# pasqal-io/Pulser

Measured on NVIDIA H100. Metric: time-steps/s (1 ns sampling intervals of the Sequence evolved per second), higher is better.
Workload: dtype f64 (complex128)

## Files before the change

### include/pulser_b200.h

```cpp
#ifndef PULSER_B200_H
#define PULSER_B200_H

#include <stdint.h>

#ifdef __cplusplus
extern "C" {
#endif

#define PB200_OK 0
#define PB200_ERR_INVALID -1
#define PB200_ERR_CUDA -2
#define PB200_ERR_UNSUPPORTED -3
#define PB200_ERR_STATE -4

#define PB200_MAX_QUDITS 40
#define PB200_MAX_DRIVES 3

typedef struct pb200_plan pb200_plan;

typedef struct pb200_drive_desc {
    int32_t state_to;
    int32_t state_from;
    int32_t uniform;
    int32_t reserved;
} pb200_drive_desc;

typedef struct pb200_plan_desc {
    int32_t n_qudits;
    int32_t dim;
    int32_t n_times;
    int32_t interp_order;
    int32_t n_drives;
    int32_t rydberg_state;
    int32_t n_traj;
    int32_t device;
    const double* sampling_times;
    pb200_drive_desc drives[PB200_MAX_DRIVES];
} pb200_plan_desc;

typedef struct pb200_run_opts {
    int32_t max_step_samples;
    int32_t refine_window;
    double cheb_tol;
    double rough_tol;
    int32_t magnus_order;
    int32_t check_every;
    double tol;
    int32_t extrapolate;
    int32_t integrator;
} pb200_run_opts;

typedef struct pb200_run_stats {
    int64_t n_steps;
    int64_t n_exponentials;
    int64_t n_applies;
    int64_t n_launches;
    double gpu_ms;
    double max_rho;
    int64_t n_checks;
    double err_estimate;
    double mean_step_samples;
    int64_t integrator;
    int64_t n_rejected;
} pb200_run_stats;

int pb200_version(void);
const char* pb200_last_error(void);
int pb200_device_count(void);

int pb200_plan_create(pb200_plan** out, const pb200_plan_desc* desc);
int pb200_plan_destroy(pb200_plan* plan);
int pb200_plan_set_stream(pb200_plan* plan, void* cuda_stream);

int pb200_plan_set_interaction(pb200_plan* plan, int32_t traj0, int32_t count,
                               const double* U, const uint8_t* bad,
                               int32_t shared);

int pb200_plan_set_xy(pb200_plan* plan, int32_t traj0, int32_t count,
                      const double* Uxy, const uint8_t* bad, int32_t shared,
                      int32_t digit_u, int32_t digit_d);

int pb200_plan_set_slm_mask(pb200_plan* plan, const uint8_t* masked, const double* coeff);

int pb200_plan_set_drive(pb200_plan* plan, int32_t drive, int32_t traj0,
                         int32_t count, const double* coef, const double* det);

int pb200_plan_set_dissipator(pb200_plan* plan, int32_t n_pairs,
                              const double* generators);

int pb200_plan_set_collapse(pb200_plan* plan, int32_t n_ops, const double* ops,
                            uint64_t seed);
int pb200_plan_jump_counts(pb200_plan* plan, int64_t* jumps);

int pb200_state_set(pb200_plan* plan, int32_t traj0, int32_t count,
                    const double* psi, int64_t basis_index, int32_t broadcast);
int pb200_state_get(pb200_plan* plan, int32_t traj0, int32_t count, double* psi);
int pb200_state_probabilities(pb200_plan* plan, int32_t traj0, int32_t count,
                              double* probs);
int pb200_state_norm2(pb200_plan* plan, int32_t traj0, int32_t count,
                      double* norms2);
int pb200_state_occupation(pb200_plan* plan, int32_t traj0, int32_t count,
                           int32_t digit, double* occ);
int pb200_state_correlation(pb200_plan* plan, int32_t traj0, int32_t count,
                            int32_t digit, double* corr);

int pb200_state_energy(pb200_plan* plan, double t_us, double* energy, double* h2);

int pb200_state_overlap(pb200_plan* plan, int32_t traj0, int32_t count,
                        const double* phi, double* out);

typedef struct pb200_op_terms {
    int32_t n_terms;
    const double*  coeff;
    const int32_t* site_start;
    const int32_t* site;
    const int32_t* shift;
    const double*  weight;
} pb200_op_terms;
int pb200_state_expect(pb200_plan* plan, int32_t traj0, int32_t count,
                       const pb200_op_terms* op, double* out);

int pb200_state_sample(pb200_plan* plan, int32_t traj, int32_t one_digit,
                       const double* uniforms, int32_t n_shots, int64_t* out);
int pb200_state_copy(pb200_plan* dst, int32_t dst_traj, pb200_plan* src, int32_t src_traj);
int pb200_state_device_ptr(pb200_plan* plan, void** dptr);

int pb200_density_trace(pb200_plan* plan, int32_t traj0, int32_t count,
                        double* trace);
int pb200_density_occupation(pb200_plan* plan, int32_t traj0, int32_t count,
                             int32_t digit, double* occ);
int pb200_density_correlation(pb200_plan* plan, int32_t traj0, int32_t count,
                              int32_t digit, double* corr);
int pb200_density_expect(pb200_plan* plan, int32_t traj0, int32_t count,
                         const pb200_op_terms* op, double* out);
int pb200_density_energy(pb200_plan* plan, pb200_plan* ham, double t_us,
                         int32_t traj0, int32_t count, double* energy,
                         double* h2);
int pb200_density_overlap(pb200_plan* plan, int32_t traj0, int32_t count,
                          const double* phi, double* out);
int pb200_density_sample(pb200_plan* plan, int32_t traj, int32_t one_digit,
                         const double* uniforms, int32_t n_shots, int64_t* out);

int pb200_propagate(pb200_plan* plan, double t_start, double t_stop,
                    const pb200_run_opts* opts, pb200_run_stats* stats);

int pb200_apply_h(pb200_plan* plan, int32_t traj, double t_us,
                  const double* in, double* out);

int pb200_coefficients_at(pb200_plan* plan, int32_t traj, int32_t drive,
                          int32_t row, double t_us, double* out3);

int pb200_bench_apply(pb200_plan* plan, double t_us, int32_t reps,
                      double* ms_out, int64_t* launches_out);

int pb200_plan_create_shard(pb200_plan** out, const pb200_plan_desc* desc,
                            int32_t shard_bits, int32_t shard_index);
int pb200_shards_link(pb200_plan** plans, int32_t count);
int pb200_shards_propagate(pb200_plan** plans, int32_t count, double t_start,
                           double t_stop, const pb200_run_opts* opts,
                           pb200_run_stats* stats);
int pb200_shards_apply_h(pb200_plan** plans, int32_t count, double t_us,
                         const double* in, double* out);
int pb200_shards_energy(pb200_plan** plans, int32_t count, double t_us,
                        double* energy, double* h2);
int pb200_shards_expect(pb200_plan** plans, int32_t count,
                        const pb200_op_terms* op, double* out);

int pb200_host_interpolate(const double* x, const double* y, int32_t n,
                           int32_t order, const double* tq, int32_t nq,
                           double* out);
int pb200_host_moments(const double* x, const double* y, int32_t n,
                       int32_t order, double a, double b, double* out4);
int pb200_host_taylor_fit(const double* x, const double* y, int32_t n,
                          int32_t order, double a, double h, int32_t p,
                          double* coeffs, double* resid);
int pb200_host_taylor_separable(const double* coef, const double* det,
                                int32_t n_traj, int32_t n_qudits,
                                int32_t n_times, int32_t* separable,
                                double* a_out, double* c_out, double* m_out);
int pb200_host_taylor_shapes(const double* coef, const double* det,
                             int32_t n_traj, int32_t n_qudits, int32_t n_times,
                             int32_t max_shapes, int32_t* n_shapes,
                             double* a_out, double* c_out, double* m_out);
int pb200_host_taylor_order(double h, const double* m, int32_t p, double tol,
                            int32_t* order_out, double* tail_out);
int pb200_host_chebyshev(double rho, double tol, double* out, int32_t cap,
                         int32_t* count);

#ifdef __cplusplus
}
#endif
#endif
```

### pulser_b200/_lib.py

```python
from __future__ import annotations

import ctypes as C
import os

_HERE = os.path.dirname(os.path.abspath(__file__))
LIB_PATH = os.path.join(_HERE, "libpulser_b200.so")

PB200_MAX_DRIVES = 3


class DriveDesc(C.Structure):
    _fields_ = [
        ("state_to", C.c_int32),
        ("state_from", C.c_int32),
        ("uniform", C.c_int32),
        ("reserved", C.c_int32),
    ]


class PlanDesc(C.Structure):
    _fields_ = [
        ("n_qudits", C.c_int32),
        ("dim", C.c_int32),
        ("n_times", C.c_int32),
        ("interp_order", C.c_int32),
        ("n_drives", C.c_int32),
        ("rydberg_state", C.c_int32),
        ("n_traj", C.c_int32),
        ("device", C.c_int32),
        ("sampling_times", C.POINTER(C.c_double)),
        ("drives", DriveDesc * PB200_MAX_DRIVES),
    ]


class RunOpts(C.Structure):
    _fields_ = [
        ("max_step_samples", C.c_int32),
        ("refine_window", C.c_int32),
        ("cheb_tol", C.c_double),
        ("rough_tol", C.c_double),
        ("magnus_order", C.c_int32),
        ("check_every", C.c_int32),
        ("tol", C.c_double),
        ("extrapolate", C.c_int32),
        ("integrator", C.c_int32),
    ]


class RunStats(C.Structure):
    _fields_ = [
        ("n_steps", C.c_int64),
        ("n_exponentials", C.c_int64),
        ("n_applies", C.c_int64),
        ("n_launches", C.c_int64),
        ("gpu_ms", C.c_double),
        ("max_rho", C.c_double),
        ("n_checks", C.c_int64),
        ("err_estimate", C.c_double),
        ("mean_step_samples", C.c_double),
        ("integrator", C.c_int64),
        ("n_rejected", C.c_int64),
    ]


class OpTermsDesc(C.Structure):

    _fields_ = [
        ("n_terms", C.c_int32),
        ("coeff", C.POINTER(C.c_double)),
        ("site_start", C.POINTER(C.c_int32)),
        ("site", C.POINTER(C.c_int32)),
        ("shift", C.POINTER(C.c_int32)),
        ("weight", C.POINTER(C.c_double)),
    ]


class LibraryMissing(ImportError):
    pass


def _load() -> C.CDLL:
    if not os.path.exists(LIB_PATH):
        raise LibraryMissing(
            f"{LIB_PATH} not found: build it with "
            "`python -m pulser_b200.build` (nvcc, sm_90a). "
            "pulser_b200 has no CPU fallback."
        )
    lib = C.CDLL(LIB_PATH)
    dp = C.POINTER(C.c_double)
    vp = C.c_void_p
    sig = {
        "pb200_version": (C.c_int, []),
        "pb200_last_error": (C.c_char_p, []),
        "pb200_device_count": (C.c_int, []),
        "pb200_plan_create": (C.c_int, [C.POINTER(vp), C.POINTER(PlanDesc)]),
        "pb200_plan_destroy": (C.c_int, [vp]),
        "pb200_plan_set_stream": (C.c_int, [vp, vp]),
        "pb200_plan_set_interaction": (
            C.c_int, [vp, C.c_int32, C.c_int32, dp, C.POINTER(C.c_uint8), C.c_int32]),
        "pb200_plan_set_xy": (
            C.c_int, [vp, C.c_int32, C.c_int32, dp, C.POINTER(C.c_uint8), C.c_int32, C.c_int32, C.c_int32]),
        "pb200_plan_set_slm_mask": (C.c_int, [vp, C.POINTER(C.c_uint8), dp]),
        "pb200_plan_set_drive": (C.c_int, [vp, C.c_int32, C.c_int32, C.c_int32, dp, dp]),
        "pb200_plan_set_dissipator": (C.c_int, [vp, C.c_int32, dp]),
        "pb200_plan_set_collapse": (C.c_int, [vp, C.c_int32, dp, C.c_uint64]),
        "pb200_plan_jump_counts": (C.c_int, [vp, C.POINTER(C.c_int64)]),
        "pb200_state_set": (C.c_int, [vp, C.c_int32, C.c_int32, dp, C.c_int64, C.c_int32]),
        "pb200_state_get": (C.c_int, [vp, C.c_int32, C.c_int32, dp]),
        "pb200_state_probabilities": (C.c_int, [vp, C.c_int32, C.c_int32, dp]),
        "pb200_state_norm2": (C.c_int, [vp, C.c_int32, C.c_int32, dp]),
        "pb200_state_occupation": (C.c_int, [vp, C.c_int32, C.c_int32, C.c_int32, dp]),
        "pb200_state_correlation": (C.c_int, [vp, C.c_int32, C.c_int32, C.c_int32, dp]),
        "pb200_state_energy": (C.c_int, [vp, C.c_double, dp, dp]),
        "pb200_state_overlap": (C.c_int, [vp, C.c_int32, C.c_int32, dp, dp]),
        "pb200_state_expect": (C.c_int, [vp, C.c_int32, C.c_int32, C.POINTER(OpTermsDesc), dp]),
        "pb200_state_sample": (
            C.c_int, [vp, C.c_int32, C.c_int32, dp, C.c_int32, C.POINTER(C.c_int64)]),
        "pb200_state_copy": (C.c_int, [vp, C.c_int32, vp, C.c_int32]),
        "pb200_state_device_ptr": (C.c_int, [vp, C.POINTER(vp)]),
        "pb200_density_trace": (C.c_int, [vp, C.c_int32, C.c_int32, dp]),
        "pb200_density_occupation": (C.c_int, [vp, C.c_int32, C.c_int32, C.c_int32, dp]),
        "pb200_density_correlation": (C.c_int, [vp, C.c_int32, C.c_int32, C.c_int32, dp]),
        "pb200_density_expect": (C.c_int, [vp, C.c_int32, C.c_int32, C.POINTER(OpTermsDesc), dp]),
        "pb200_density_energy": (C.c_int, [vp, vp, C.c_double, C.c_int32, C.c_int32, dp, dp]),
        "pb200_density_overlap": (C.c_int, [vp, C.c_int32, C.c_int32, dp, dp]),
        "pb200_density_sample": (
            C.c_int, [vp, C.c_int32, C.c_int32, dp, C.c_int32, C.POINTER(C.c_int64)]),
        "pb200_propagate": (
            C.c_int, [vp, C.c_double, C.c_double, C.POINTER(RunOpts), C.POINTER(RunStats)]),
        "pb200_apply_h": (C.c_int, [vp, C.c_int32, C.c_double, dp, dp]),
        "pb200_coefficients_at": (
            C.c_int, [vp, C.c_int32, C.c_int32, C.c_int32, C.c_double, dp]),
        "pb200_bench_apply": (
            C.c_int, [vp, C.c_double, C.c_int32, dp, C.POINTER(C.c_int64)]),
        "pb200_plan_create_shard": (C.c_int, [C.POINTER(vp), C.POINTER(PlanDesc), C.c_int32, C.c_int32]),
        "pb200_shards_link": (C.c_int, [C.POINTER(vp), C.c_int32]),
        "pb200_shards_propagate": (
            C.c_int, [C.POINTER(vp), C.c_int32, C.c_double, C.c_double, C.POINTER(RunOpts), C.POINTER(RunStats)]),
        "pb200_shards_apply_h": (C.c_int, [C.POINTER(vp), C.c_int32, C.c_double, dp, dp]),
        "pb200_shards_energy": (C.c_int, [C.POINTER(vp), C.c_int32, C.c_double, dp, dp]),
        "pb200_shards_expect": (C.c_int, [C.POINTER(vp), C.c_int32, C.POINTER(OpTermsDesc), dp]),
        "pb200_host_interpolate": (
            C.c_int, [dp, dp, C.c_int32, C.c_int32, dp, C.c_int32, dp]),
        "pb200_host_moments": (
            C.c_int, [dp, dp, C.c_int32, C.c_int32, C.c_double, C.c_double, dp]),
        "pb200_host_chebyshev": (
            C.c_int, [C.c_double, C.c_double, dp, C.c_int32, C.POINTER(C.c_int32)]),
        "pb200_host_taylor_fit": (
            C.c_int, [dp, dp, C.c_int32, C.c_int32, C.c_double, C.c_double, C.c_int32, dp, dp]),
        "pb200_host_taylor_separable": (
            C.c_int, [dp, dp, C.c_int32, C.c_int32, C.c_int32, C.POINTER(C.c_int32), dp, dp, dp]),
        "pb200_host_taylor_shapes": (
            C.c_int, [dp, dp, C.c_int32, C.c_int32, C.c_int32, C.c_int32, C.POINTER(C.c_int32), dp, dp, dp]),
        "pb200_host_taylor_order": (
            C.c_int, [C.c_double, dp, C.c_int32, C.c_double, C.POINTER(C.c_int32), dp]),
    }
    for name, (res, args) in sig.items():
        fn = getattr(lib, name)
        fn.restype = res
        fn.argtypes = args
    return lib


EXPORTED_SYMBOLS = [
    "pb200_version", "pb200_last_error", "pb200_device_count",
    "pb200_plan_create", "pb200_plan_destroy", "pb200_plan_set_stream",
    "pb200_plan_set_interaction", "pb200_plan_set_xy", "pb200_plan_set_slm_mask", "pb200_plan_set_drive", "pb200_plan_set_dissipator", "pb200_plan_set_collapse",
    "pb200_plan_jump_counts", "pb200_state_set",
    "pb200_state_get", "pb200_state_probabilities", "pb200_state_norm2",
    "pb200_state_occupation", "pb200_state_correlation", "pb200_state_energy", "pb200_state_overlap", "pb200_state_expect", "pb200_state_sample", "pb200_state_copy", "pb200_state_device_ptr", "pb200_propagate", "pb200_apply_h",
    "pb200_coefficients_at", "pb200_bench_apply", "pb200_host_interpolate",
    "pb200_host_moments", "pb200_host_chebyshev", "pb200_host_taylor_fit", "pb200_host_taylor_order", "pb200_host_taylor_separable",
    "pb200_host_taylor_shapes",
    "pb200_plan_create_shard", "pb200_shards_link", "pb200_shards_propagate", "pb200_shards_apply_h", "pb200_shards_energy",
    "pb200_shards_expect",
    "pb200_density_trace", "pb200_density_occupation", "pb200_density_correlation", "pb200_density_expect",
    "pb200_density_energy", "pb200_density_overlap", "pb200_density_sample",
]

lib = _load()


class PB200Error(RuntimeError):
    def __init__(self, code: int, msg: str):
        super().__init__(f"pulser_b200 error {code}: {msg}")
        self.code = code


def check(code: int) -> None:
    if code != 0:
        raise PB200Error(code, lib.pb200_last_error().decode("utf-8", "replace"))
```

### pulser_b200/csrc/kernels.cuh

```cuda
#pragma once
#include <cuda_runtime.h>
#include <stdint.h>
#include <type_traits>

namespace pb200 {

struct c2 { double x, y; };

__host__ __device__ inline c2 cmul(c2 a, c2 b) { return {a.x * b.x - a.y * b.y, a.x * b.y + a.y * b.x}; }
__host__ __device__ inline c2 cadd(c2 a, c2 b) { return {a.x + b.x, a.y + b.y}; }

struct PassGeom {
    int n_bits;
    int lo_bits;
    int hi_shift;
    int hi_bits;
    uint32_t tile_flip_mask;
    unsigned long long extra_mask;
    int first_pass;
};

struct StageCoef {
    c2 c_psi, c_b2, c_g;
};

struct UniformDrive {
    c2 g;
    double theta;
    double w;
    double gamma;
    int to_bit;
    int from_count_is_popc;
};

__host__ __device__ inline int d2_table_stride(int n) { return 3 * n + 2; }

__device__ __forceinline__ uint32_t smem_u32(const void* p) {
    return static_cast<uint32_t>(__cvta_generic_to_shared(p));
}
__device__ __forceinline__ void mbar_init(uint64_t* bar, uint32_t count) {
    asm volatile("mbarrier.init.shared::cta.b64 [%0], %1;" ::"r"(smem_u32(bar)), "r"(count));
    asm volatile("fence.mbarrier_init.release.cluster;" ::: "memory");
    asm volatile("fence.proxy.async.shared::cta;" ::: "memory");
}
__device__ __forceinline__ void mbar_arrive_expect_tx(uint64_t* bar, uint32_t bytes) {
    asm volatile("mbarrier.arrive.expect_tx.shared::cta.b64 _, [%0], %1;" ::"r"(smem_u32(bar)), "r"(bytes)
                 : "memory");
}
__device__ __forceinline__ void mbar_wait(uint64_t* bar, uint32_t parity) {
    asm volatile(
        "{\n\t"
        ".reg .pred p;\n\t"
        "WAIT_%=:\n\t"
        "mbarrier.try_wait.parity.shared::cta.b64 p, [%0], %1;\n\t"
        "@p bra DONE_%=;\n\t"
        "bra WAIT_%=;\n\t"
        "DONE_%=:\n\t"
        "}\n" ::"r"(smem_u32(bar)),
        "r"(parity)
        : "memory");
}
__device__ __forceinline__ void tma_load_1d(void* smem_dst, const void* gmem_src, uint32_t bytes, uint64_t* bar) {
    asm volatile(
        "cp.async.bulk.shared::cluster.global.mbarrier::complete_tx::bytes [%0], [%1], %2, [%3];" ::"r"(
            smem_u32(smem_dst)),
        "l"(gmem_src), "r"(bytes), "r"(smem_u32(bar))
        : "memory");
}

__device__ __forceinline__ c2 ld_stream(const c2* p) {
    double2 r = __ldcs(reinterpret_cast<const double2*>(p));
    return {r.x, r.y};
}
__device__ __forceinline__ void st_c2(c2* p, c2 v) {
    *reinterpret_cast<double2*>(p) = make_double2(v.x, v.y);
}
__device__ __forceinline__ void st_c2_evict_last(c2* p, c2 v) {
    uint64_t pol;
    asm("createpolicy.fractional.L2::evict_last.b64 %0, 1.0;" : "=l"(pol));
    asm volatile("st.global.L2::cache_hint.v2.f64 [%0], {%1, %2}, %3;" ::"l"(p), "d"(v.x), "d"(v.y), "l"(pol) : "memory");
}

struct LanczosFuse {
    const c2* vj;
    const c2* vjm1;
    c2* vout;
    const double* acc_prev;
    const double* beta_prev;
    double* alpha_out;
    double* beta_out;
    double* acc_clear;
};

struct LanczosCoef { double alpha, beta, inv, beta_prev; };

__device__ __forceinline__ LanczosCoef lanczos_coef(const LanczosFuse& lz, long long traj) {
    LanczosCoef c;
    c.alpha = lz.acc_prev[2 * traj];
    const double ww = lz.acc_prev[2 * traj + 1];
    const double b2 = ww - c.alpha * c.alpha;
    c.beta = (b2 > 1e-28 * fmax(ww, 1e-300)) ? sqrt(b2) : 0.0;
    c.inv = c.beta > 0.0 ? 1.0 / c.beta : 0.0;
    c.beta_prev = lz.beta_prev ? lz.beta_prev[traj] : 0.0;
    return c;
}

struct StageArgs {
    const c2* v;
    const c2* psi;
    const c2* b2;
    c2* out;
    const double* dint;
    long long dint_stride;
    long long D;
    PassGeom geo;
    StageCoef coef;
    UniformDrive u;
    const double* table;
    int to_bit;
    int from_is_one;
    const double* beta_dev;
    double* dot_acc;
    LanczosFuse lz;
    const c2* w_in;
    c2* w_out;
    long long w_plane;
};

struct StageArgs2 {
    StageArgs a[2];
    int n_traj;
};

template <bool UNIFORM, bool REAL_G>
__global__ void __launch_bounds__(256) stage_d2_kernel(StageArgs a) {
    extern __shared__ __align__(128) unsigned char smem_raw[];
    c2* tile = reinterpret_cast<c2*>(smem_raw);
    __shared__ __align__(8) uint64_t mbar;

    const PassGeom g = a.geo;
    const int tbits = g.lo_bits + g.hi_bits;
    const int tsize = 1 << tbits;
    const long long traj = blockIdx.y;
    const long long tile_id = blockIdx.x;
    const int mid_bits = g.hi_shift - g.lo_bits;
    const long long mid = tile_id & ((1LL << mid_bits) - 1);
    const long long top = tile_id >> mid_bits;
    const long long base = (mid << g.lo_bits) | (top << (g.hi_shift + g.hi_bits));
    const long long voff = traj * a.D;
    const c2* vsrc = a.v + voff;

    double* tab = reinterpret_cast<double*>(tile + tsize);
    if (!UNIFORM) {
        const int stride = d2_table_stride(g.n_bits);
        const double* src = a.table + traj * stride;
        for (int i = threadIdx.x; i < stride; i += blockDim.x) tab[i] = src[i];
    }

    if (threadIdx.x == 0) mbar_init(&mbar, 1);
    __syncthreads();
    if (threadIdx.x == 0) mbar_arrive_expect_tx(&mbar, (uint32_t)tsize * 16u);
    {
        const int rows = 1 << g.hi_bits;
        const uint32_t row_bytes = (uint32_t)(16u << g.lo_bits);
        for (int r = threadIdx.x; r < rows; r += blockDim.x)
            tma_load_1d(tile + ((size_t)r << g.lo_bits), vsrc + base + ((long long)r << g.hi_shift), row_bytes, &mbar);
    }
    mbar_wait(&mbar, 0);

    const long long lomask = (1LL << g.lo_bits) - 1;
    double w, gamma, theta_u;
    c2 gu;
    if (UNIFORM) {
        w = a.u.w; gamma = a.u.gamma; theta_u = a.u.theta; gu = a.u.g;
    } else {
        w = tab[3 * g.n_bits]; gamma = tab[3 * g.n_bits + 1]; theta_u = 0.0; gu = {0.0, 0.0};
    }
    const int to_bit = a.to_bit;

    for (int t = threadIdx.x; t < tsize; t += blockDim.x) {
        const long long idx = base | (t & lomask) | ((long long)(t >> g.lo_bits) << g.hi_shift);
        const c2 vo = tile[t];
        double pr = 0.0, pi = 0.0, qr = 0.0, qi = 0.0;
#pragma unroll 1
        for (uint32_t m = g.tile_flip_mask; m; m &= m - 1) {
            const int j = __ffs(m) - 1;
            const c2 pv = tile[t ^ (1 << j)];
            const int bit = (t >> j) & 1;
            if (UNIFORM) {
                pr += pv.x; pi += pv.y;
                if (!REAL_G) {
                    const double s = (bit == to_bit) ? 1.0 : -1.0;
                    qr = fma(s, pv.x, qr); qi = fma(s, pv.y, qi);
                }
            } else {
                const int p = (j < g.lo_bits) ? j : (j - g.lo_bits + g.hi_shift);
                const double gx = tab[2 * p];
                const double gy = (bit == to_bit) ? tab[2 * p + 1] : -tab[2 * p + 1];
                pr = fma(gx, pv.x, pr); pr = fma(-gy, pv.y, pr);
                pi = fma(gx, pv.y, pi); pi = fma(gy, pv.x, pi);
            }
        }
#pragma unroll 1
        for (unsigned long long m = g.extra_mask; m; m &= m - 1) {
            const int p = __ffsll((long long)m) - 1;
            const double2 raw = __ldg(reinterpret_cast<const double2*>(vsrc + (idx ^ (1LL << p))));
            const c2 pv = {raw.x, raw.y};
            const int bit = (int)((idx >> p) & 1);
            if (UNIFORM) {
                pr += pv.x; pi += pv.y;
                if (!REAL_G) {
                    const double s = (bit == to_bit) ? 1.0 : -1.0;
                    qr = fma(s, pv.x, qr); qi = fma(s, pv.y, qi);
                }
            } else {
                const double gx = tab[2 * p];
                const double gy = (bit == to_bit) ? tab[2 * p + 1] : -tab[2 * p + 1];
                pr = fma(gx, pv.x, pr); pr = fma(-gy, pv.y, pr);
                pi = fma(gx, pv.y, pi); pi = fma(gy, pv.x, pi);
            }
        }
        c2 drive;
        if (UNIFORM) {
            drive.x = gu.x * pr; drive.y = gu.x * pi;
            if (!REAL_G) { drive.x = fma(-gu.y, qi, drive.x); drive.y = fma(gu.y, qr, drive.y); }
        } else {
            drive = {pr, pi};
        }
        c2 res;
        if (g.first_pass) {
            double diag = -gamma;
            if (a.dint) diag = fma(w, __ldcs(a.dint + traj * a.dint_stride + idx), diag);
            if (UNIFORM) {
                const int ones = __popcll((unsigned long long)idx);
                const int cnt = a.from_is_one ? ones : (g.n_bits - ones);
                diag = fma(-theta_u, (double)cnt, diag);
            } else {
                double acc = 0.0;
                for (int p = 0; p < g.n_bits; ++p) {
                    const int bit = (int)((idx >> p) & 1);
                    acc += (bit == a.from_is_one) ? tab[2 * g.n_bits + p] : 0.0;
                }
                diag -= acc;
            }
            c2 gv = {fma(diag, vo.x, drive.x), fma(diag, vo.y, drive.y)};
            res = cmul(a.coef.c_g, gv);
            if (a.psi) res = cadd(res, cmul(a.coef.c_psi, ld_stream(a.psi + voff + idx)));
            if (a.b2) res = cadd(res, cmul(a.beta_dev ? c2{-a.beta_dev[traj], 0.0} : a.coef.c_b2, ld_stream(a.b2 + voff + idx)));
        } else {
            res = cadd(ld_stream(a.out + voff + idx), cmul(a.coef.c_g, drive));
        }
        st_c2(a.out + voff + idx, res);
    }
}

__device__ __forceinline__ c2 ld_own(const c2* p) {
    double2 r = __ldcs(reinterpret_cast<const double2*>(p));
    return {r.x, r.y};
}

__device__ __forceinline__ void taylor_signed_add(double gx, double gy, double sg, double x, double y, double& pr, double& pi,
                                                  double& qr, double& qi) {
    const double zx = fma(gx, x, -gy * y), zy = fma(gx, y, gy * x);
    pr += zx; pi += zy;
    qr = fma(sg, zx, qr); qi = fma(sg, zy, qi);
}

template <bool UNIFORM, bool REAL_G, int TBITS, int RB, bool SIGNED = false>
__device__ __forceinline__ void rb_tile_gather(const PassGeom& g, const c2* tile, const double* __restrict__ tab, int tid,
                                               int to_bit, int jstart, bool skip_smem, const c2 (&v)[1 << RB],
                                               double (&pr)[1 << RB], double (&pi)[1 << RB], double (&qr)[1 << RB],
                                               double (&qi)[1 << RB]) {
    static_assert(!SIGNED || !UNIFORM, "signed sums of the per-bit table gather");
    constexpr int R = 1 << RB;
    constexpr int NT = 1 << (TBITS - RB);
#pragma unroll
    for (int q = 0; q < RB; ++q) {
        const int j = TBITS - RB + q;
        double gx = 0.0, gyt = 0.0;
        if (!UNIFORM) {
            const int p = (j < g.lo_bits) ? j : (j - g.lo_bits + g.hi_shift);
            gx = tab[2 * p]; gyt = tab[2 * p + 1];
        }
#pragma unroll
        for (int r = 0; r < R; ++r) {
            const c2 pv = v[r ^ (1 << q)];
            const int bit = (r >> q) & 1;
            if (UNIFORM) {
                pr[r] += pv.x; pi[r] += pv.y;
                if (!REAL_G) {
                    if (bit == to_bit) { qr[r] += pv.x; qi[r] += pv.y; } else { qr[r] -= pv.x; qi[r] -= pv.y; }
                }
            } else if constexpr (SIGNED) {
                const double gy = (bit == to_bit) ? gyt : -gyt;
                taylor_signed_add(gx, gy, bit == to_bit ? 1.0 : -1.0, pv.x, pv.y, pr[r], pi[r], qr[r], qi[r]);
            } else {
                const double gy = (bit == to_bit) ? gyt : -gyt;
                pr[r] = fma(gx, pv.x, pr[r]); pr[r] = fma(-gy, pv.y, pr[r]);
                pi[r] = fma(gx, pv.y, pi[r]); pi[r] = fma(gy, pv.x, pi[r]);
            }
        }
    }
#pragma unroll
    for (int j = 0; j < TBITS - RB; ++j) {
        if (j >= jstart && !skip_smem) {
            const int bit = (tid >> j) & 1;
            const int ptid = tid ^ (1 << j);
            double gx = 0.0, gy = 0.0;
            if (!UNIFORM) {
                const int p = (j < g.lo_bits) ? j : (j - g.lo_bits + g.hi_shift);
                gx = tab[2 * p];
                gy = (bit == to_bit) ? tab[2 * p + 1] : -tab[2 * p + 1];
            }
            const double sg = (bit == to_bit) ? 1.0 : -1.0;
#pragma unroll
            for (int r = 0; r < R; ++r) {
                const c2 pv = tile[ptid + r * NT];
                if (UNIFORM) {
                    pr[r] += pv.x; pi[r] += pv.y;
                    if (!REAL_G) { qr[r] = fma(sg, pv.x, qr[r]); qi[r] = fma(sg, pv.y, qi[r]); }
                } else if constexpr (SIGNED) {
                    taylor_signed_add(gx, gy, sg, pv.x, pv.y, pr[r], pi[r], qr[r], qi[r]);
                } else {
                    pr[r] = fma(gx, pv.x, pr[r]); pr[r] = fma(-gy, pv.y, pr[r]);
                    pi[r] = fma(gx, pv.y, pi[r]); pi[r] = fma(gy, pv.x, pi[r]);
                }
            }
        }
    }
}

template <bool UNIFORM, bool REAL_G, int TBITS, int RB>
__device__ __forceinline__ void rb_tile_compute(const StageArgs& a, const PassGeom& g, const c2* tile,
                                                const double* __restrict__ tab, long long base, long long traj,
                                                int tid, uint64_t* tile_bar) {
    constexpr int R = 1 << RB;
    constexpr int NT = 1 << (TBITS - RB);
    const long long voff = traj * a.D;
    const c2* vsrc = a.v + voff;
    const long long lomask = (1LL << g.lo_bits) - 1;
    const int to_bit = a.to_bit;
    const int jstart = __ffs(g.tile_flip_mask) - 1;

    c2 v[R];
    double pr[R], pi[R], qr[R], qi[R];
    long long idx[R];
#pragma unroll
    for (int r = 0; r < R; ++r) {
        const int t = tid + r * NT;
        idx[r] = base | (t & lomask) | ((long long)(t >> g.lo_bits) << g.hi_shift);
        pr[r] = 0.0; pi[r] = 0.0; qr[r] = 0.0; qi[r] = 0.0;
    }
    for (unsigned long long m = g.extra_mask; m; m &= m - 1) {
        const int p = __ffsll((long long)m) - 1;
        double gx = 0.0, gyt = 0.0;
        if (!UNIFORM) { gx = tab[2 * p]; gyt = tab[2 * p + 1]; }
        const int bit = (int)((base >> p) & 1);
        const double sg = (bit == to_bit) ? 1.0 : -1.0;
        const double gy = (bit == to_bit) ? gyt : -gyt;
        double2 raw[R];
#pragma unroll
        for (int r = 0; r < R; ++r) raw[r] = __ldg(reinterpret_cast<const double2*>(vsrc + (idx[r] ^ (1LL << p))));
#pragma unroll
        for (int r = 0; r < R; ++r) {
            if (UNIFORM) {
                pr[r] += raw[r].x; pi[r] += raw[r].y;
                if (!REAL_G) { qr[r] = fma(sg, raw[r].x, qr[r]); qi[r] = fma(sg, raw[r].y, qi[r]); }
            } else {
                pr[r] = fma(gx, raw[r].x, pr[r]); pr[r] = fma(-gy, raw[r].y, pr[r]);
                pi[r] = fma(gx, raw[r].y, pi[r]); pi[r] = fma(gy, raw[r].x, pi[r]);
            }
        }
    }
    if (tile_bar) mbar_wait(tile_bar, 0);
#pragma unroll
    for (int r = 0; r < R; ++r) v[r] = tile[tid + r * NT];
    rb_tile_gather<UNIFORM, REAL_G, TBITS, RB>(g, tile, tab, tid, to_bit, jstart, false, v, pr, pi, qr, qi);
    double w = 0.0, gamma = 0.0, th_common = 0.0;
    double th_r[R];
    if (g.first_pass) {
        if (UNIFORM) { w = a.u.w; gamma = a.u.gamma; }
        else {
            w = tab[3 * g.n_bits]; gamma = tab[3 * g.n_bits + 1];
            const long long fixed = base | (tid & lomask) | ((long long)(tid >> g.lo_bits) << g.hi_shift);
            for (int p = 0; p < g.n_bits; ++p) {
                const int bit = (int)((fixed >> p) & 1);
                th_common += (bit == a.from_is_one) ? tab[2 * g.n_bits + p] : 0.0;
            }
#pragma unroll
            for (int r = 0; r < R; ++r) {
                double acc = 0.0;
#pragma unroll
                for (int q = 0; q < RB; ++q) {
                    const int j = TBITS - RB + q;
                    const int p = (j < g.lo_bits) ? j : (j - g.lo_bits + g.hi_shift);
                    const double th = tab[2 * g.n_bits + p];
                    const int bit = (r >> q) & 1;
                    acc += ((bit == a.from_is_one) ? th : 0.0) - ((0 == a.from_is_one) ? th : 0.0);
                }
                th_r[r] = acc;
            }
        }
    }
#pragma unroll
    for (int r = 0; r < R; ++r) {
        if (UNIFORM) {
            const double dx = a.u.g.x * pr[r], dy = a.u.g.x * pi[r];
            if (!REAL_G) { pr[r] = fma(-a.u.g.y, qi[r], dx); pi[r] = fma(a.u.g.y, qr[r], dy); }
            else { pr[r] = dx; pi[r] = dy; }
        }
    }
    constexpr int H = (R >= 4) ? R / 2 : R;
    const c2 cb2 = a.beta_dev ? c2{-a.beta_dev[traj], 0.0} : a.coef.c_b2;
    const bool fuse = a.lz.vj != nullptr;
    LanczosCoef lc{0.0, 0.0, 0.0, 0.0};
    if (fuse) lc = lanczos_coef(a.lz, traj);
    double dot0 = 0.0, dot1 = 0.0;
    if (g.first_pass) {
        const double* dsrc = a.dint ? a.dint + traj * a.dint_stride : nullptr;
#pragma unroll
        for (int h0 = 0; h0 < R; h0 += H) {
            double dv[H];
            c2 pv[H], bv[H];
#pragma unroll
            for (int r = 0; r < H; ++r) {
                dv[r] = dsrc ? __ldcs(dsrc + idx[h0 + r]) : 0.0;
                if (fuse) {
                    pv[r] = ld_own(a.lz.vj + voff + idx[h0 + r]);
                    bv[r] = (a.lz.vjm1 && lc.beta_prev != 0.0) ? ld_own(a.lz.vjm1 + voff + idx[h0 + r]) : c2{0.0, 0.0};
                } else {
                    pv[r] = a.psi ? ld_own(a.psi + voff + idx[h0 + r]) : c2{0.0, 0.0};
                    bv[r] = a.b2 ? ld_own(a.b2 + voff + idx[h0 + r]) : c2{0.0, 0.0};
                }
            }
#pragma unroll
            for (int r = 0; r < H; ++r) {
                const int rr = h0 + r;
                double diag = fma(w, dv[r], -gamma);
                if (UNIFORM) {
                    const int ones = __popcll((unsigned long long)idx[rr]);
                    const int cnt = a.from_is_one ? ones : (g.n_bits - ones);
                    diag = fma(-a.u.theta, (double)cnt, diag);
                } else {
                    diag -= th_common + th_r[rr];
                }
                const c2 gv = {fma(diag, v[rr].x, pr[rr]), fma(diag, v[rr].y, pi[rr])};
                c2 res, lhs;
                if (fuse) {
                    const c2 vn = {(v[rr].x - lc.alpha * pv[r].x) * lc.inv, (v[rr].y - lc.alpha * pv[r].y) * lc.inv};
                    const double ai = lc.alpha * lc.inv, abi = ai * lc.beta_prev;
                    res.x = fma(lc.inv, gv.x, -fma(ai, v[rr].x, fma(abi, bv[r].x, lc.beta * pv[r].x)));
                    res.y = fma(lc.inv, gv.y, -fma(ai, v[rr].y, fma(abi, bv[r].y, lc.beta * pv[r].y)));
                    st_c2(a.lz.vout + voff + idx[rr], vn);
                    lhs = vn;
                } else {
                    res = cmul(a.coef.c_g, gv);
                    res = cadd(res, cmul(a.coef.c_psi, pv[r]));
                    res = cadd(res, cmul(cb2, bv[r]));
                    lhs = v[rr];
                }
                dot0 = fma(lhs.x, res.x, dot0); dot0 = fma(lhs.y, res.y, dot0);
                dot1 = fma(res.x, res.x, dot1); dot1 = fma(res.y, res.y, dot1);
                st_c2(a.out + voff + idx[rr], res);
            }
        }
    } else {
#pragma unroll
        for (int h0 = 0; h0 < R; h0 += H) {
            c2 ov[H];
#pragma unroll
            for (int r = 0; r < H; ++r) ov[r] = ld_own(a.out + voff + idx[h0 + r]);
#pragma unroll
            for (int r = 0; r < H; ++r) {
                const int rr = h0 + r;
                const c2 res = cadd(ov[r], cmul(a.coef.c_g, c2{pr[rr], pi[rr]}));
                dot0 = fma(v[rr].x, res.x, dot0); dot0 = fma(v[rr].y, res.y, dot0);
                dot1 = fma(res.x, res.x, dot1); dot1 = fma(res.y, res.y, dot1);
                st_c2(a.out + voff + idx[rr], res);
            }
        }
    }
    if (a.dot_acc) {
        for (int o = 16; o > 0; o >>= 1) {
            dot0 += __shfl_xor_sync(0xffffffffu, dot0, o);
            dot1 += __shfl_xor_sync(0xffffffffu, dot1, o);
        }
        __shared__ double dred[2][NT / 32 > 0 ? NT / 32 : 1];
        if ((tid & 31) == 0) { dred[0][tid >> 5] = dot0; dred[1][tid >> 5] = dot1; }
        __syncthreads();
        if (tid == 0) {
            double s0 = 0.0, s1 = 0.0;
#pragma unroll
            for (int i = 0; i < NT / 32; ++i) { s0 += dred[0][i]; s1 += dred[1][i]; }
            atomicAdd(a.dot_acc + 2 * traj, s0);
            atomicAdd(a.dot_acc + 2 * traj + 1, s1);
        }
    }
    if (fuse && blockIdx.x == 0 && tid == 0) {
        a.lz.alpha_out[traj] = lc.alpha;
        a.lz.beta_out[traj] = lc.beta;
        a.lz.acc_clear[2 * traj] = 0.0;
        a.lz.acc_clear[2 * traj + 1] = 0.0;
    }
}

__device__ __forceinline__ long long tile_base_of(const PassGeom& g, long long tile_id) {
    const int mid_bits = g.hi_shift - g.lo_bits;
    const long long mid = tile_id & ((1LL << mid_bits) - 1);
    const long long top = tile_id >> mid_bits;
    return (mid << g.lo_bits) | (top << (g.hi_shift + g.hi_bits));
}

__device__ __forceinline__ void pdl_wait() { asm volatile("griddepcontrol.wait;" ::: "memory"); }
__device__ __forceinline__ void pdl_launch_dependents() { asm volatile("griddepcontrol.launch_dependents;" ::: "memory"); }

template <bool UNIFORM, bool REAL_G, int TBITS, int RB>
__global__ void __launch_bounds__(1 << (TBITS - RB), (65536 / ((1 << (TBITS - RB)) * (RB >= 3 ? 128 : 64))))
stage_d2_rb_kernel(const __grid_constant__ StageArgs2 m) {
    constexpr int NT = 1 << (TBITS - RB);
    constexpr int TSIZE = 1 << TBITS;
    extern __shared__ __align__(128) unsigned char smem_raw[];
    c2* tile = reinterpret_cast<c2*>(smem_raw);
    __shared__ __align__(8) uint64_t mbar;

    const int chain = blockIdx.y / m.n_traj;
    const StageArgs& a = m.a[chain];
    const PassGeom g = a.geo;
    const int tid = threadIdx.x;
    const long long traj = blockIdx.y - chain * m.n_traj;
    const long long base = tile_base_of(g, blockIdx.x);
    const c2* vsrc = a.v + traj * a.D;

    if (tid == 0) mbar_init(&mbar, 1);
    __syncthreads();
    pdl_wait();
    pdl_launch_dependents();
    if (tid == 0) mbar_arrive_expect_tx(&mbar, (uint32_t)TSIZE * 16u);
    const int rows = 1 << g.hi_bits;
    const uint32_t row_bytes = (uint32_t)(16u << g.lo_bits);
    for (int r = tid; r < rows; r += NT)
        tma_load_1d(tile + ((size_t)r << g.lo_bits), vsrc + base + ((long long)r << g.hi_shift), row_bytes, &mbar);
    double* tab = reinterpret_cast<double*>(tile + TSIZE);
    if (!UNIFORM) {
        const int stride = d2_table_stride(g.n_bits);
        const double* src = a.table + traj * stride;
        for (int i = tid; i < stride; i += NT) tab[i] = src[i];
        __syncthreads();
    }
    rb_tile_compute<UNIFORM, REAL_G, TBITS, RB>(a, g, tile, tab, base, traj, tid, &mbar);
}

template <bool REAL_G, int TBITS, int RB>
__global__ void __launch_bounds__(1 << (TBITS - RB), 2) stage_d2_fwd_kernel(const __grid_constant__ StageArgs2 m) {
    constexpr int R = 1 << RB;
    constexpr int NT = 1 << (TBITS - RB);
    constexpr int TSIZE = 1 << TBITS;
    extern __shared__ __align__(128) unsigned char smem_raw[];
    c2* tile = reinterpret_cast<c2*>(smem_raw);
    c2* rtile = tile + TSIZE;
    __shared__ __align__(8) uint64_t mbar;

    const int chain = blockIdx.y / m.n_traj;
    const StageArgs& a = m.a[chain];
    const PassGeom g = a.geo;
    const int tid = threadIdx.x;
    const long long traj = blockIdx.y - chain * m.n_traj;
    const long long base = tile_base_of(g, blockIdx.x);
    const long long voff = traj * a.D;
    const c2* vsrc = a.v + voff;

    if (tid == 0) mbar_init(&mbar, 1);
    __syncthreads();
    pdl_wait();
    pdl_launch_dependents();
    if (tid == 0) mbar_arrive_expect_tx(&mbar, (uint32_t)TSIZE * 16u);
    {
        const int rows = 1 << g.hi_bits;
        const uint32_t row_bytes = (uint32_t)(16u << g.lo_bits);
        for (int r = tid; r < rows; r += NT)
            tma_load_1d(tile + ((size_t)r << g.lo_bits), vsrc + base + ((long long)r << g.hi_shift), row_bytes, &mbar);
    }
    const long long lomask = (1LL << g.lo_bits) - 1;
    const long long fixed = base | (tid & lomask) | ((long long)(tid >> g.lo_bits) << g.hi_shift);
    int pq[RB];
#pragma unroll
    for (int q = 0; q < RB; ++q) {
        const int j = TBITS - RB + q;
        pq[q] = (j < g.lo_bits) ? j : (j - g.lo_bits + g.hi_shift);
    }
    auto idx_of = [&](int r) {
        long long o = fixed;
#pragma unroll
        for (int q = 0; q < RB; ++q) o |= (long long)((r >> q) & 1) << pq[q];
        return o;
    };
    double pr[R], pi[R], qr[R], qi[R];
    c2 part[R];
    double dg[R];
    {
        const double* dsrc = a.dint ? a.dint + traj * a.dint_stride : nullptr;
#pragma unroll
        for (int r = 0; r < R; ++r) {
            const long long ix = idx_of(r);
            c2 w0 = {0.0, 0.0}, w1 = {0.0, 0.0}, ps = {0.0, 0.0}, bb = {0.0, 0.0};
            if (a.w_in) { w0 = ld_own(a.w_in + voff + ix); if (!REAL_G) w1 = ld_own(a.w_in + a.w_plane + voff + ix); }
            if (a.psi) ps = ld_own(a.psi + voff + ix);
            if (a.b2) bb = ld_own(a.b2 + voff + ix);
            const double dv = dsrc ? __ldcs(dsrc + ix) : 0.0;
            pr[r] = w0.x; pi[r] = w0.y; qr[r] = w1.x; qi[r] = w1.y;
            part[r] = cadd(cmul(a.coef.c_psi, ps), cmul(a.coef.c_b2, bb));
            const int ones = __popcll((unsigned long long)ix);
            const int cnt = a.from_is_one ? ones : (g.n_bits - ones);
            dg[r] = fma(-a.u.theta, (double)cnt, fma(a.u.w, dv, -a.u.gamma));
        }
    }
    const int to_bit = a.to_bit;
    for (unsigned long long em = g.extra_mask; em; em &= em - 1) {
        const int p = __ffsll((long long)em) - 1;
        const double sg = (((base >> p) & 1) == to_bit) ? 1.0 : -1.0;
        double2 raw[R];
#pragma unroll
        for (int r = 0; r < R; ++r) raw[r] = __ldg(reinterpret_cast<const double2*>(vsrc + (idx_of(r) ^ (1LL << p))));
#pragma unroll
        for (int r = 0; r < R; ++r) {
            pr[r] += raw[r].x; pi[r] += raw[r].y;
            if (!REAL_G) { qr[r] = fma(sg, raw[r].x, qr[r]); qi[r] = fma(sg, raw[r].y, qi[r]); }
        }
    }
    mbar_wait(&mbar, 0);
    const int jstart = __ffs(g.tile_flip_mask) - 1;
    c2 v[R];
#pragma unroll
    for (int r = 0; r < R; ++r) v[r] = tile[tid + r * NT];
    rb_tile_gather<true, REAL_G, TBITS, RB>(g, tile, nullptr, tid, to_bit, jstart, false, v, pr, pi, qr, qi);
#pragma unroll
    for (int r = 0; r < R; ++r) {
        double dx = a.u.g.x * pr[r], dy = a.u.g.x * pi[r];
        if (!REAL_G) { dx = fma(-a.u.g.y, qi[r], dx); dy = fma(a.u.g.y, qr[r], dy); }
        const c2 gv = {fma(dg[r], v[r].x, dx), fma(dg[r], v[r].y, dy)};
        const c2 res = cadd(part[r], cmul(a.coef.c_g, gv));
        st_c2(a.out + voff + idx_of(r), res);
        v[r] = res;
    }
    if (a.w_out) {
#pragma unroll
        for (int r = 0; r < R; ++r) {
            rtile[tid + r * NT] = v[r];
            pr[r] = 0.0; pi[r] = 0.0; qr[r] = 0.0; qi[r] = 0.0;
        }
        __syncthreads();
        rb_tile_gather<true, REAL_G, TBITS, RB>(g, rtile, nullptr, tid, to_bit, jstart, false, v, pr, pi, qr, qi);
#pragma unroll
        for (int r = 0; r < R; ++r) {
            const long long ix = idx_of(r);
            st_c2(a.w_out + voff + ix, c2{pr[r], pi[r]});
            if (!REAL_G) st_c2(a.w_out + a.w_plane + voff + ix, c2{qr[r], qi[r]});
        }
    }
}

#define PB200_TAYLOR_PMAX 8
#define PB200_MAX_SHARD_BITS 3
#define PB200_TAYLOR_SMAX 4
__host__ __device__ inline int taylor_table_stride(int n, int s) { return 2 * n + s * n; }
struct TaylorArgs {
    const c2* v;
    c2* out;
    c2* g_out;
    c2* acc;
    const double* dint;
    long long dint_stride;
    const double* cpl;
    long long cpl_stride;
    int ryd_bit;
    long long D;
    PassGeom geo;
    c2 unit;
    const double* table;
    int tab_shapes;
    int to_bit, from_is_one;
    double th0, gam0, om0;
    double m0[PB200_TAYLOR_SMAX];
    c2 scale;
    int nh;
    const c2* hchi[PB200_TAYLOR_PMAX];
    const c2* hg[PB200_TAYLOR_PMAX];
    double hth[PB200_TAYLOR_PMAX], hgam[PB200_TAYLOR_PMAX], hom[PB200_TAYLOR_PMAX];
    double hm[PB200_TAYLOR_SMAX][PB200_TAYLOR_PMAX];
    int acc_read;
    int acc_add_v;
    int acc_add_h;
    int acc_on;
    c2 acc_mul;
    const c2* peer[PB200_MAX_SHARD_BITS];
    int shard_bits, shard;
    c2* g2_out;
    double om0i;
    const c2* hg2[PB200_TAYLOR_PMAX];
    double homi[PB200_TAYLOR_PMAX];
    c2 dw[4], df[4];
    int n_pair;
    int diss_flip;
};

template <int R, int H = (R >= 4) ? R / 2 : R, bool SHARD = false, bool CPLX = false, bool DISS = false, class Off,
          class Dint>
__device__ __forceinline__ void taylor_epilogue(const TaylorArgs& a, const long long (&idx)[R], c2 (&v)[R],
                                                const double (&gx)[R], const double (&gy)[R], const Off& off,
                                                long long voff, const Dint& dint,
                                                const double* qx = nullptr, const double* qy = nullptr,
                                                const double* ex = nullptr, const double* ey = nullptr) {
    constexpr bool SHAPES = !std::is_array<Off>::value;
    const int nb = a.geo.n_bits;
    const int ones_hi = SHARD ? __popc(a.shard) : 0;
#pragma unroll
    for (int h0 = 0; h0 < R; h0 += H) {
        double sx[H], sy[H], cn[H];
        {
            double dv[H];
#pragma unroll
            for (int r = 0; r < H; ++r) dv[r] = dint(h0 + r);
#pragma unroll
            for (int r = 0; r < H; ++r) {
                const int ones = __popcll((unsigned long long)idx[h0 + r]) + ones_hi;
                cn[r] = (double)(a.from_is_one ? ones : (nb - ones));
                double diag;
                if constexpr (SHAPES) diag = fma(-a.th0, cn[r], dv[r] - a.gam0 - off(h0 + r, 0));
                else diag = fma(-a.th0, cn[r], fma(-a.m0[0], off[h0 + r], dv[r] - a.gam0));
                sx[r] = fma(diag, v[h0 + r].x, a.om0 * gx[h0 + r]);
                sy[r] = fma(diag, v[h0 + r].y, a.om0 * gy[h0 + r]);
                if constexpr (CPLX) { sx[r] = fma(a.om0i, qx[h0 + r], sx[r]); sy[r] = fma(a.om0i, qy[h0 + r], sy[r]); }
                if constexpr (DISS) { sx[r] += ex[h0 + r]; sy[r] += ey[h0 + r]; }
            }
        }
        for (int j = 0; j < a.nh; ++j) {
            if (a.hchi[j]) {
                c2 c[H];
#pragma unroll
                for (int r = 0; r < H; ++r) c[r] = ld_own(a.hchi[j] + voff + idx[h0 + r]);
#pragma unroll
                for (int r = 0; r < H; ++r) {
                    double d;
                    if constexpr (SHAPES) d = -fma(a.hth[j], cn[r], a.hgam[j] + off(h0 + r, j + 1));
                    else d = -fma(a.hth[j], cn[r], fma(a.hm[0][j], off[h0 + r], a.hgam[j]));
                    sx[r] = fma(d, c[r].x, sx[r]); sy[r] = fma(d, c[r].y, sy[r]);
                    if (j == 0 && a.acc_add_h) v[h0 + r] = cadd(v[h0 + r], c[r]);
                }
            }
            if (a.hg[j]) {
                c2 c[H];
#pragma unroll
                for (int r = 0; r < H; ++r) c[r] = ld_own(a.hg[j] + voff + idx[h0 + r]);
#pragma unroll
                for (int r = 0; r < H; ++r) { sx[r] = fma(a.hom[j], c[r].x, sx[r]); sy[r] = fma(a.hom[j], c[r].y, sy[r]); }
            }
            if constexpr (CPLX) {
                if (a.hg2[j]) {
                    c2 c[H];
#pragma unroll
                    for (int r = 0; r < H; ++r) c[r] = ld_own(a.hg2[j] + voff + idx[h0 + r]);
#pragma unroll
                    for (int r = 0; r < H; ++r) { sx[r] = fma(a.homi[j], c[r].x, sx[r]); sy[r] = fma(a.homi[j], c[r].y, sy[r]); }
                }
            }
        }
        c2 res[H];
#pragma unroll
        for (int r = 0; r < H; ++r) {
            res[r] = {a.scale.x * sx[r] - a.scale.y * sy[r], a.scale.x * sy[r] + a.scale.y * sx[r]};
            st_c2_evict_last(a.out + voff + idx[h0 + r], res[r]);
            if (a.g_out) st_c2(a.g_out + voff + idx[h0 + r], c2{gx[h0 + r], gy[h0 + r]});
            if constexpr (CPLX) { if (a.g2_out) st_c2(a.g2_out + voff + idx[h0 + r], c2{qx[h0 + r], qy[h0 + r]}); }
        }
        if (a.acc_on) {
            c2 ac[H];
#pragma unroll
            for (int r = 0; r < H; ++r) ac[r] = a.acc_read ? ld_own(a.acc + voff + idx[h0 + r]) : c2{0.0, 0.0};
#pragma unroll
            for (int r = 0; r < H; ++r) {
                c2 s = cadd(ac[r], res[r]);
                if (a.acc_add_v) s = cadd(s, v[h0 + r]);
                st_c2(a.acc + voff + idx[h0 + r], cmul(a.acc_mul, s));
            }
        }
    }
}

__device__ __forceinline__ c2 taylor_diss_diag(const TaylorArgs& a, long long s, c2 v) {
    const unsigned long long c = (unsigned long long)s & ((1ULL << a.n_pair) - 1), r = (unsigned long long)s >> a.n_pair;
    const double nr = (double)__popcll(r), nc = (double)__popcll(c), nrc = (double)__popcll(r & c);
    const double wx = fma(a.dw[3].x, nrc, fma(a.dw[2].x, nc, fma(a.dw[1].x, nr, a.dw[0].x)));
    const double wy = fma(a.dw[3].y, nrc, fma(a.dw[2].y, nc, fma(a.dw[1].y, nr, a.dw[0].y)));
    return {wx * v.x - wy * v.y, wx * v.y + wy * v.x};
}

__device__ __forceinline__ void taylor_diss_flip(const TaylorArgs& a, long long s, int pr, int pc, double2 pv, double& dx,
                                                 double& dy) {
    const c2 f = a.df[(int)((((s >> pr) & 1) << 1) | ((s >> pc) & 1))];
    dx = fma(f.x, pv.x, dx); dx = fma(-f.y, pv.y, dx);
    dy = fma(f.x, pv.y, dy); dy = fma(f.y, pv.x, dy);
}

__host__ __device__ constexpr int taylor_dint_doubles(int tbits, int rb) {
    return tbits * tbits + tbits + 1 + (1 << rb) + (rb + 1) * (1 << (tbits - rb));
}

template <int TBITS, int RB>
__device__ __forceinline__ void taylor_dint_setup(const TaylorArgs& a, long long traj, unsigned long long hi, int tid,
                                                  double* dsm) {
    constexpr int NT = 1 << (TBITS - RB), L0 = TBITS - RB;
    const int nb = a.geo.n_bits;
    double* Ws = dsm + taylor_dint_doubles(TBITS, RB);
    const double* Wq = a.cpl + traj * a.cpl_stride;
    for (int i = tid; i < nb * nb; i += NT) Ws[i] = __ldg(Wq + i);
    __syncthreads();
    auto W = [&](int p, int q) { return Ws[(nb - 1 - p) * nb + (nb - 1 - q)]; };
    const unsigned long long flip = a.ryd_bit ? 0ULL : ~0ULL;
    const unsigned long long nmask = nb >= 64 ? ~0ULL : (1ULL << nb) - 1;
    const unsigned long long hs = (hi ^ flip) & nmask & ~((1ULL << TBITS) - 1);
    double* wt = dsm;
    double* wj = wt + TBITS * TBITS;
    double* hh = wj + TBITS;
    double* ts = hh + 1;
    double* xt = ts + (1 << RB);
    for (int i = tid; i < TBITS * TBITS; i += NT) wt[i] = W(i / TBITS, i % TBITS);
    if (tid < TBITS) {
        double s = 0.0;
        for (unsigned long long m = hs; m; m &= m - 1) s += W(__ffsll((long long)m) - 1, tid);
        wj[tid] = s;
    } else if (tid >= 32 && tid < 32 + (1 << RB)) {
        const int m = tid - 32;
        const unsigned ms = ((unsigned)m ^ (unsigned)flip) & ((1u << RB) - 1);
        double s = 0.0;
        for (int q = 0; q < RB; ++q) {
            if (!((ms >> q) & 1)) continue;
            for (unsigned long long h = hs; h; h &= h - 1) s += W(L0 + q, __ffsll((long long)h) - 1);
            for (int q2 = q + 1; q2 < RB; ++q2) if ((ms >> q2) & 1) s += W(L0 + q, L0 + q2);
        }
        ts[m] = s;
    } else if (tid >= 64 && tid < 96) {
        double s = 0.0;
        for (int p = TBITS + (tid - 64); p < nb; p += 32) {
            if (!((hs >> p) & 1)) continue;
            for (unsigned long long h = hs & ~((2ULL << p) - 1); h; h &= h - 1) s += W(p, __ffsll((long long)h) - 1);
        }
#pragma unroll
        for (int o = 16; o; o >>= 1) s += __shfl_xor_sync(0xffffffffu, s, o);
        if (tid == 64) hh[0] = s;
    }
    __syncthreads();
    const unsigned tb = ((unsigned)tid ^ (unsigned)flip) & (NT - 1);
    double ct = hh[0];
    double y[RB];
#pragma unroll
    for (int q = 0; q < RB; ++q) y[q] = 0.0;
#pragma unroll 1
    for (int i = 0; i < L0; ++i) {
        const bool bi = (tb >> i) & 1;
        ct += bi ? wj[i] : 0.0;
        for (int j = i + 1; j < L0; ++j) ct += (bi && ((tb >> j) & 1)) ? wt[i * TBITS + j] : 0.0;
#pragma unroll
        for (int q = 0; q < RB; ++q) y[q] += bi ? wt[i * TBITS + L0 + q] : 0.0;
    }
#pragma unroll
    for (int q = 0; q < RB; ++q) {
        if (!a.ryd_bit) { ct += y[q]; y[q] = -y[q]; }
        xt[(q + 1) * NT + tid] = y[q];
    }
    xt[tid] = ct;
}

template <bool UNIFORM, bool REAL_G, int TBITS, int RB, bool SHARD = false, int NS = (UNIFORM ? 0 : 1), bool CPLX = false,
          bool DISS = false>
__global__ void __launch_bounds__(1 << (TBITS - RB),
                                  (CPLX || DISS) ? 1 : (65536 / ((1 << (TBITS - RB)) * (RB >= 3 ? 128 : 64))))
stage_d2_taylor_kernel(const __grid_constant__ TaylorArgs a) {
    static_assert(RB >= 3, "chunks of 8 amplitudes per thread");
    static_assert(UNIFORM || !SHARD, "shards carry one state with a uniform drive");
    static_assert(NS == (UNIFORM ? 0 : 1) || NS == PB200_TAYLOR_SMAX, "one-shape table, or PB200_TAYLOR_SMAX shapes");
    static_assert(!CPLX || !REAL_G, "a complex drive gathers through the per-bit table");
    static_assert(!DISS || (!UNIFORM && !SHARD && !CPLX), "a density matrix runs the batch gather, one device, one phase");
    constexpr bool SHAPES = NS == PB200_TAYLOR_SMAX;
    constexpr int NT = 1 << (TBITS - RB);
    constexpr int TSIZE = 1 << TBITS;
    constexpr int RC = 8;
    constexpr int CB = RB - 3;
    constexpr int STB = TBITS - CB;
    constexpr bool TAB = !(UNIFORM && REAL_G);
    extern __shared__ __align__(128) unsigned char smem_raw[];
    c2* tile = reinterpret_cast<c2*>(smem_raw);
    __shared__ __align__(8) uint64_t mbar;
    const PassGeom& g = a.geo;
    const int tid = threadIdx.x;
    const long long traj = UNIFORM ? 0 : (long long)blockIdx.y;
    const long long voff = traj * a.D;
    const long long base = (long long)blockIdx.x << TBITS;
    const c2* vsrc = a.v + voff;

    if (tid == 0) mbar_init(&mbar, 1);
    __syncthreads();
    double* dsm = reinterpret_cast<double*>(tile + TSIZE);
    const double* ts = dsm + TBITS * TBITS + TBITS + 1;
    const double* xt = ts + (1 << RB);
    double* tab = dsm + taylor_dint_doubles(TBITS, RB) + g.n_bits * g.n_bits;
    if (a.cpl)
        taylor_dint_setup<TBITS, RB>(
            a, traj, (unsigned long long)base | (SHARD ? (unsigned long long)a.shard << (g.n_bits - a.shard_bits) : 0ULL),
            tid, dsm);
    pdl_wait();
    pdl_launch_dependents();
    if (tid == 0) {
        mbar_arrive_expect_tx(&mbar, (uint32_t)TSIZE * 16u);
        tma_load_1d(tile, vsrc + base, (uint32_t)TSIZE * 16u, &mbar);
    }
    double* bl = tab + (SHAPES ? taylor_table_stride(g.n_bits, NS) : 0);
    double* at = bl + ((PB200_TAYLOR_PMAX + 1) << RB);
    auto shape_coef = [&](int J, int s) { return J == 0 ? a.m0[s] : a.hm[s][J - 1]; };
    if (TAB || SHAPES) {
        if (UNIFORM && !SHAPES) {
            for (int i = tid; i < 2 * g.n_bits; i += NT) tab[i] = (i & 1) ? a.unit.y : a.unit.x;
        } else {
            const int stride = SHAPES ? taylor_table_stride(g.n_bits, NS) : d2_table_stride(g.n_bits);
            const double* src = a.table + traj * stride;
            for (int i = tid; i < stride; i += NT) tab[i] = src[i];
            if (SHAPES) {
                for (int i = tid; i < ((a.nh + 1) << RB); i += NT) {
                    const int J = i >> RB;
                    double acc = 0.0;
                    for (int s = 0; s < NS; ++s) {
                        const double* w = src + 2 * g.n_bits + s * g.n_bits + (TBITS - RB);
                        double l = 0.0;
                        for (int q = 0; q < RB; ++q) {
                            const int bit = (i >> q) & 1;
                            l += ((bit == a.from_is_one) ? w[q] : 0.0) - ((0 == a.from_is_one) ? w[q] : 0.0);
                        }
                        acc = fma(shape_coef(J, s), l, acc);
                    }
                    bl[i] = acc;
                }
            }
        }
        __syncthreads();
    }
    const int to_bit = a.to_bit;
    const int nb = g.n_bits;
    double common = 0.0;
    if (!UNIFORM && !SHAPES) {
        for (int p = 0; p < nb; ++p) {
            const int bit = (int)(((base + tid) >> p) & 1);
            common += (bit == a.from_is_one) ? tab[2 * nb + p] : 0.0;
        }
    }
    if (SHAPES) {
        double cs[NS > 0 ? NS : 1];
#pragma unroll
        for (int s = 0; s < NS; ++s) cs[s] = 0.0;
        for (int p = 0; p < nb; ++p) {
            int bit = (int)(((base + tid) >> p) & 1);
            if (SHARD && p >= nb - a.shard_bits) bit = (a.shard >> (p - (nb - a.shard_bits))) & 1;
            if (bit == a.from_is_one) {
#pragma unroll
                for (int s = 0; s < NS; ++s) cs[s] += tab[2 * nb + s * nb + p];
            }
        }
        for (int J = 0; J <= a.nh; ++J) {
            double acc = 0.0;
#pragma unroll
            for (int s = 0; s < NS; ++s) acc = fma(shape_coef(J, s), cs[s], acc);
            at[J * NT + tid] = acc;
        }
    }
#pragma unroll 1
    for (int c = 0; c < (1 << CB); ++c) {
        const long long i0 = base + tid + c * RC * NT;
        double pr[RC], pi[RC];
        double dr[RC], di[RC];
#pragma unroll
        for (int r = 0; r < RC; ++r) { pr[r] = 0.0; pi[r] = 0.0; dr[r] = 0.0; di[r] = 0.0; }
        for (unsigned long long m = g.extra_mask; m; m &= m - 1) {
            const int p = __ffsll((long long)m) - 1;
            const int bit = (int)((base >> p) & 1);
            double gx = 0.0, gy = 0.0;
            if (TAB) { gx = tab[2 * p]; gy = (bit == to_bit) ? tab[2 * p + 1] : -tab[2 * p + 1]; }
            const c2* src = vsrc + (i0 ^ (1LL << p));
            double2 raw[RC];
#pragma unroll
            for (int r = 0; r < RC; ++r) raw[r] = __ldg(reinterpret_cast<const double2*>(src + r * NT));
#pragma unroll
            for (int r = 0; r < RC; ++r) {
                if constexpr (CPLX) {
                    taylor_signed_add(gx, gy, bit == to_bit ? 1.0 : -1.0, raw[r].x, raw[r].y, pr[r], pi[r], dr[r], di[r]);
                } else if (!TAB) {
                    pr[r] += raw[r].x; pi[r] += raw[r].y;
                } else {
                    pr[r] = fma(gx, raw[r].x, pr[r]); pr[r] = fma(-gy, raw[r].y, pr[r]);
                    pi[r] = fma(gx, raw[r].y, pi[r]); pi[r] = fma(gy, raw[r].x, pi[r]);
                }
            }
        }
        if (SHARD) {
            for (int q = 0; q < a.shard_bits; ++q) {
                const int bit = (a.shard >> q) & 1;
                double gx = 0.0, gy = 0.0;
                if (TAB) {
                    const int p = nb - a.shard_bits + q;
                    gx = tab[2 * p]; gy = (bit == to_bit) ? tab[2 * p + 1] : -tab[2 * p + 1];
                }
                const c2* src = a.peer[q] + i0;
                double2 raw[RC];
#pragma unroll
                for (int r = 0; r < RC; ++r) raw[r] = *reinterpret_cast<const double2*>(src + r * NT);
#pragma unroll
                for (int r = 0; r < RC; ++r) {
                    if constexpr (CPLX) {
                        taylor_signed_add(gx, gy, bit == to_bit ? 1.0 : -1.0, raw[r].x, raw[r].y, pr[r], pi[r], dr[r], di[r]);
                    } else if (!TAB) {
                        pr[r] += raw[r].x; pi[r] += raw[r].y;
                    } else {
                        pr[r] = fma(gx, raw[r].x, pr[r]); pr[r] = fma(-gy, raw[r].y, pr[r]);
                        pi[r] = fma(gx, raw[r].y, pi[r]); pi[r] = fma(gy, raw[r].x, pi[r]);
                    }
                }
            }
        }
        if (c == 0) mbar_wait(&mbar, 0);
        auto dint = [&](int r) {
            if (!a.cpl) return 0.0;
            const int m = c * RC + r;
            double d = ts[m] + xt[tid];
#pragma unroll
            for (int q = 0; q < RB; ++q)
                if ((m >> q) & 1) d += xt[(q + 1) * NT + tid];
            return d;
        };
        const c2* sub = tile + (c << STB);
        c2 v[RC];
        double qd[RC];
#pragma unroll
        for (int r = 0; r < RC; ++r) v[r] = sub[tid + r * NT];
        if constexpr (CPLX) rb_tile_gather<false, false, STB, 3, true>(g, sub, tab, tid, to_bit, 0, false, v, pr, pi, dr, di);
        else rb_tile_gather<!TAB, !TAB, STB, 3>(g, sub, tab, tid, to_bit, 0, false, v, pr, pi, qd, qd);
#pragma unroll
        for (int q = 0; q < CB; ++q) {
            const int p = STB + q;
            const int bit = (c >> q) & 1;
            double gx = 0.0, gy = 0.0;
            if (TAB) { gx = tab[2 * p]; gy = (bit == to_bit) ? tab[2 * p + 1] : -tab[2 * p + 1]; }
            const c2* other = tile + ((c ^ (1 << q)) << STB);
#pragma unroll
            for (int r = 0; r < RC; ++r) {
                const c2 pv = other[tid + r * NT];
                if constexpr (CPLX) {
                    taylor_signed_add(gx, gy, bit == to_bit ? 1.0 : -1.0, pv.x, pv.y, pr[r], pi[r], dr[r], di[r]);
                } else if (!TAB) {
                    pr[r] += pv.x; pi[r] += pv.y;
                } else {
                    pr[r] = fma(gx, pv.x, pr[r]); pr[r] = fma(-gy, pv.y, pr[r]);
                    pi[r] = fma(gx, pv.y, pi[r]); pi[r] = fma(gy, pv.x, pi[r]);
                }
            }
        }
        double off[RC];
        long long idx[RC];
#pragma unroll
        for (int r = 0; r < RC; ++r) {
            idx[r] = i0 + r * NT;
            if (!TAB) { pr[r] *= a.unit.x; pi[r] *= a.unit.x; }
            double acc = common;
            if (!UNIFORM && !SHAPES) {
#pragma unroll
                for (int q = 0; q < RB; ++q) {
                    const double th = tab[2 * nb + TBITS - RB + q];
                    const int bit = ((c * RC + r) >> q) & 1;
                    acc += ((bit == a.from_is_one) ? th : 0.0) - ((0 == a.from_is_one) ? th : 0.0);
                }
            }
            off[r] = acc;
        }
        double ex[RC], ey[RC];
        if constexpr (DISS) {
            double dx[RC], dy[RC];
#pragma unroll
            for (int r = 0; r < RC; ++r) {
                const c2 w = taylor_diss_diag(a, idx[r], v[r]);
                dx[r] = w.x; dy[r] = w.y;
            }
            if (a.diss_flip) {
                const int tpos = tid + (c << STB);
                for (int pc = 0; pc < a.n_pair; ++pc) {
                    const int pr = pc + a.n_pair;
                    const long long mask = (1LL << pr) | (1LL << pc);
                    double2 pv[RC];
                    if (pr < TBITS) {
#pragma unroll
                        for (int r = 0; r < RC; ++r) {
                            const c2 t = tile[(tpos + r * NT) ^ (int)mask];
                            pv[r] = make_double2(t.x, t.y);
                        }
                    } else {
#pragma unroll
                        for (int r = 0; r < RC; ++r) pv[r] = __ldg(reinterpret_cast<const double2*>(vsrc + (idx[r] ^ mask)));
                    }
#pragma unroll
                    for (int r = 0; r < RC; ++r) taylor_diss_flip(a, idx[r], pr, pc, pv[r], dx[r], dy[r]);
                }
            }
#pragma unroll
            for (int r = 0; r < RC; ++r) { ex[r] = -dy[r]; ey[r] = dx[r]; }
        }
        if constexpr (CPLX) {
            double qx[RC], qy[RC];
#pragma unroll
            for (int r = 0; r < RC; ++r) { qx[r] = -di[r]; qy[r] = dr[r]; }
            if constexpr (SHAPES) {
                const double* lc = bl + c * RC;
                const double* lt = at + tid;
                taylor_epilogue<RC, RC / 4, SHARD, true>(
                    a, idx, v, pr, pi, [&](int r, int J) { return lt[J * NT] + lc[(J << RB) + r]; }, voff, dint, qx, qy);
            } else {
                taylor_epilogue<RC, RC / 4, SHARD, true>(a, idx, v, pr, pi, off, voff, dint, qx, qy);
            }
        } else if constexpr (SHAPES) {
            const double* lc = bl + c * RC;
            const double* lt = at + tid;
            taylor_epilogue<RC, RC / 4, SHARD, false, DISS>(
                a, idx, v, pr, pi, [&](int r, int J) { return lt[J * NT] + lc[(J << RB) + r]; }, voff, dint, nullptr,
                nullptr, ex, ey);
        } else {
            taylor_epilogue<RC, UNIFORM ? RC / 2 : RC / 4, SHARD, false, DISS>(a, idx, v, pr, pi, off, voff, dint, nullptr,
                                                                             nullptr, ex, ey);
        }
    }
}

template <bool CPLX = false, bool DISS = false>
__global__ void __launch_bounds__(256) stage_d2_taylor_small_kernel(const __grid_constant__ TaylorArgs a) {
    const long long s = (long long)blockIdx.x * blockDim.x + threadIdx.x;
    if (s >= a.D) return;
    const int nb = a.geo.n_bits;
    const long long traj = blockIdx.y;
    const long long voff = traj * a.D;
    const int ns = a.tab_shapes ? a.tab_shapes : 1;
    const double* tab = a.table ? a.table + traj * (a.tab_shapes ? taylor_table_stride(nb, ns) : d2_table_stride(nb)) : nullptr;
    double gxs = 0.0, gys = 0.0, offv[PB200_TAYLOR_SMAX];
    double q2x = 0.0, q2y = 0.0;
#pragma unroll
    for (int q = 0; q < PB200_TAYLOR_SMAX; ++q) offv[q] = 0.0;
    if (tab) {
        double dx = 0.0, dy = 0.0;
        for (int p = 0; p < nb; ++p) {
            const double2 raw = __ldg(reinterpret_cast<const double2*>(a.v + voff + (s ^ (1LL << p))));
            const int bit = (int)((s >> p) & 1);
            const double gx = tab[2 * p], gy = (bit == a.to_bit) ? tab[2 * p + 1] : -tab[2 * p + 1];
            if constexpr (CPLX) {
                taylor_signed_add(gx, gy, bit == a.to_bit ? 1.0 : -1.0, raw.x, raw.y, gxs, gys, dx, dy);
            } else {
                gxs = fma(gx, raw.x, gxs); gxs = fma(-gy, raw.y, gxs);
                gys = fma(gx, raw.y, gys); gys = fma(gy, raw.x, gys);
            }
            if (bit == a.from_is_one) {
#pragma unroll
                for (int q = 0; q < PB200_TAYLOR_SMAX; ++q)
                    if (q < ns) offv[q] += tab[2 * nb + q * nb + p];
            }
        }
        q2x = -dy; q2y = dx;
    } else {
        double pr = 0.0, pi = 0.0, qr = 0.0, qi = 0.0;
        for (int p = 0; p < nb; ++p) {
            const double2 raw = __ldg(reinterpret_cast<const double2*>(a.v + voff + (s ^ (1LL << p))));
            const double sg = ((int)((s >> p) & 1) == a.to_bit) ? 1.0 : -1.0;
            pr += raw.x; pi += raw.y; qr = fma(sg, raw.x, qr); qi = fma(sg, raw.y, qi);
        }
        gxs = fma(-a.unit.y, qi, a.unit.x * pr);
        gys = fma(a.unit.y, qr, a.unit.x * pi);
        q2x = -fma(a.unit.x, qi, a.unit.y * pr);
        q2y = fma(a.unit.x, qr, -a.unit.y * pi);
    }
    const long long idx[1] = {s};
    const double2 own = __ldg(reinterpret_cast<const double2*>(a.v + voff + s));
    c2 v[1] = {{own.x, own.y}};
    const double gx[1] = {gxs}, gy[1] = {gys}, offv1[1] = {offv[0]};
    const double qx[1] = {q2x}, qy[1] = {q2y};
    double ex[1] = {0.0}, ey[1] = {0.0};
    if constexpr (DISS) {
        const c2 w = taylor_diss_diag(a, s, v[0]);
        double dx = w.x, dy = w.y;
        if (a.diss_flip) {
            for (int pc = 0; pc < a.n_pair; ++pc) {
                const int pr = pc + a.n_pair;
                const double2 pv = __ldg(reinterpret_cast<const double2*>(a.v + voff + (s ^ (1LL << pr) ^ (1LL << pc))));
                taylor_diss_flip(a, s, pr, pc, pv, dx, dy);
            }
        }
        ex[0] = -dy; ey[0] = dx;
    }
    auto local = [&](int, int J) {
        double acc = 0.0;
#pragma unroll
        for (int q = 0; q < PB200_TAYLOR_SMAX; ++q) acc = fma(J == 0 ? a.m0[q] : a.hm[q][J - 1], offv[q], acc);
        return acc;
    };
    const double* dsrc = a.dint ? a.dint + traj * a.dint_stride : nullptr;
    auto dint = [&](int) { return dsrc ? __ldcs(dsrc + s) : 0.0; };
    if (a.tab_shapes) taylor_epilogue<1, 1, false, CPLX, DISS>(a, idx, v, gx, gy, local, voff, dint, qx, qy, ex, ey);
    else taylor_epilogue<1, 1, false, CPLX, DISS>(a, idx, v, gx, gy, offv1, voff, dint, qx, qy, ex, ey);
}

__host__ __device__ inline int gen_table_stride(int n, int n_drives) { return n_drives * 3 * n + 3; }

#define PB200_TILED_MAX_HIGH 40
#define PB200_MAX_DRIVES_K 3
struct GenArgs {
    const c2* v; const c2* psi; const c2* b2; c2* out;
    const double* dint; long long dint_stride; long long D;
    int n, dim, n_drives;
    int to[3], from[3];
    StageCoef coef;
    const double* table;
    const double* beta_dev;
    const double* xy; long long xy_stride; int xy_u, xy_d;
    unsigned long long slm_mask; const double* dint2;
    double* dot_acc;
    LanczosFuse lz;
};

__global__ void __launch_bounds__(256) stage_generic_kernel(GenArgs a) {
    extern __shared__ __align__(16) unsigned char smem_raw[];
    double* tab = reinterpret_cast<double*>(smem_raw);
    const int stride = gen_table_stride(a.n, a.n_drives);
    const long long traj = blockIdx.y;
    for (int i = threadIdx.x; i < stride; i += blockDim.x) tab[i] = a.table[traj * stride + i];
    __syncthreads();
    double* xys = tab + stride;
    if (a.xy) {
        const double wx = tab[stride - 2], wxc = tab[stride - 3];
        for (int i = threadIdx.x; i < a.n * a.n; i += blockDim.x) {
            const int qi = i / a.n, qj = i - qi * a.n;
            const bool touched = ((a.slm_mask >> qi) | (a.slm_mask >> qj)) & 1ULL;
            xys[i] = a.xy[traj * a.xy_stride + i] * (touched ? wxc : wx);
        }
        __syncthreads();
    }
    const double w = tab[stride - 2], gamma = tab[stride - 1];
    const long long voff = traj * a.D;
    for (long long idx = blockIdx.x * (long long)blockDim.x + threadIdx.x; idx < a.D;
         idx += (long long)gridDim.x * blockDim.x) {
        const c2 vo = a.v[voff + idx];
        double diag = -gamma;
        if (a.dint) diag = fma(w, a.dint[traj * a.dint_stride + idx], diag);
        if (a.dint2) diag = fma(tab[stride - 3], a.dint2[traj * a.dint_stride + idx], diag);
        double rr = 0.0, ri = 0.0;
        long long rem = idx, st = 1;
        for (int k = a.n - 1; k >= 0; --k) {
            const int digit = (int)(rem % a.dim);
            rem /= a.dim;
            for (int q = 0; q < a.n_drives; ++q) {
                const double* gq = tab + q * 3 * a.n;
                if (digit == a.to[q]) {
                    const c2 pv = a.v[voff + idx + (long long)(a.from[q] - a.to[q]) * st];
                    const double gx = gq[2 * k], gy = gq[2 * k + 1];
                    rr = fma(gx, pv.x, rr); rr = fma(-gy, pv.y, rr);
                    ri = fma(gx, pv.y, ri); ri = fma(gy, pv.x, ri);
                } else if (digit == a.from[q]) {
                    const c2 pv = a.v[voff + idx + (long long)(a.to[q] - a.from[q]) * st];
                    const double gx = gq[2 * k], gy = -gq[2 * k + 1];
                    rr = fma(gx, pv.x, rr); rr = fma(-gy, pv.y, rr);
                    ri = fma(gx, pv.y, ri); ri = fma(gy, pv.x, ri);
                    diag -= gq[2 * a.n + k];
                }
            }
            st *= a.dim;
        }
        if (a.xy) {
            signed char dg[40];
            long long sts[40];
            long long r2 = idx, s2 = 1;
            for (int k = a.n - 1; k >= 0; --k) { dg[k] = (signed char)(r2 % a.dim); r2 /= a.dim; sts[k] = s2; s2 *= a.dim; }
            for (int i = 0; i < a.n; ++i) {
                if (dg[i] != a.xy_u && dg[i] != a.xy_d) continue;
                for (int j = i + 1; j < a.n; ++j) {
                    if ((dg[i] == a.xy_u && dg[j] == a.xy_d) || (dg[i] == a.xy_d && dg[j] == a.xy_u)) {
                        const double u = xys[i * a.n + j];
                        if (u == 0.0) continue;
                        const long long pidx2 = idx + (long long)(dg[j] - dg[i]) * sts[i] + (long long)(dg[i] - dg[j]) * sts[j];
                        const c2 pv = a.v[voff + pidx2];
                        rr = fma(u, pv.x, rr); ri = fma(u, pv.y, ri);
                    }
                }
            }
        }
        c2 gv = {fma(diag, vo.x, rr), fma(diag, vo.y, ri)};
        c2 res = cmul(a.coef.c_g, gv);
        if (a.psi) res = cadd(res, cmul(a.coef.c_psi, a.psi[voff + idx]));
        if (a.b2) res = cadd(res, cmul(a.beta_dev ? c2{-a.beta_dev[traj], 0.0} : a.coef.c_b2, a.b2[voff + idx]));
        st_c2(a.out + voff + idx, res);
    }
}

struct TileExtra { long long off; double gx, gy; };

__host__ __device__ constexpr int ipow_c(int b, int e) { return e <= 0 ? 1 : b * ipow_c(b, e - 1); }

template <int DIM, int K, int RBD>
__global__ void __launch_bounds__(256, 2) stage_multilevel_rb_kernel(GenArgs a) {
    constexpr int R = ipow_c(DIM, RBD);
    extern __shared__ __align__(128) unsigned char smem_raw[];
    __shared__ __align__(8) uint64_t mbar;
    __shared__ TileExtra extra[PB200_MAX_DRIVES_K * PB200_TILED_MAX_HIGH];
    __shared__ int n_extra;
    __shared__ double diag_high;

    const int tid = threadIdx.x;
    const long long traj = blockIdx.y;
    const int n = a.n;
    const int kk = n < K ? n : K;
    int nt_act = 1;
    for (int j = 0; j < kk - RBD; ++j) nt_act *= DIM;
    const int tsz = nt_act * R;
    c2* tile = reinterpret_cast<c2*>(smem_raw);
    double* tab = reinterpret_cast<double*>(smem_raw + (((size_t)tsz * 16 + 127) / 128) * 128);
    const int stride = gen_table_stride(n, a.n_drives);
    const long long base = (long long)blockIdx.x * tsz;
    const long long voff = traj * a.D;

    if (tid == 0) mbar_init(&mbar, 1);
    for (int i = tid; i < stride; i += blockDim.x) tab[i] = a.table[traj * stride + i];
    __syncthreads();
    if (tid == 0) {
        mbar_arrive_expect_tx(&mbar, (uint32_t)tsz * 16u);
        tma_load_1d(tile, a.v + voff + base, (uint32_t)tsz * 16u, &mbar);
    }
    if (tid < 32) {
        int cnt = 0;
        double dh = 0.0;
        const int total = (n - kk) * a.n_drives;
        for (int e0 = 0; e0 < total; e0 += 32) {
            const int e = e0 + tid;
            bool valid = false;
            TileExtra te = {0, 0.0, 0.0};
            if (e < total) {
                const int j = kk + e / a.n_drives, q = e % a.n_drives;
                long long rem = blockIdx.x, st = tsz;
                for (int jj = kk; jj < j; ++jj) { rem /= DIM; st *= DIM; }
                const int digit = (int)(rem % DIM);
                const int k = n - 1 - j;
                const double* gq = tab + q * 3 * n;
                if (digit == a.to[q]) {
                    valid = true;
                    te = {(long long)(a.from[q] - a.to[q]) * st, gq[2 * k], gq[2 * k + 1]};
                } else if (digit == a.from[q]) {
                    valid = true;
                    te = {(long long)(a.to[q] - a.from[q]) * st, gq[2 * k], -gq[2 * k + 1]};
                    dh -= gq[2 * n + k];
                }
            }
            const unsigned m = __ballot_sync(0xffffffffu, valid);
            if (valid) extra[cnt + __popc(m & ((1u << tid) - 1u))] = te;
            cnt += __popc(m);
        }
        for (int o = 16; o > 0; o >>= 1) dh += __shfl_xor_sync(0xffffffffu, dh, o);
        if (tid == 0) { n_extra = cnt; diag_high = dh; }
    }
    __syncthreads();
    mbar_wait(&mbar, 0);
    double dot0 = 0.0, dot1 = 0.0;
    const bool fuse = a.lz.vj != nullptr;
    LanczosCoef lc{0.0, 0.0, 0.0, 0.0};
    if (fuse) lc = lanczos_coef(a.lz, traj);
    if (tid < nt_act) {

    double rr[R], ri[R], dd[R];
#pragma unroll
    for (int i = 0; i < R; ++i) { rr[i] = 0.0; ri[i] = 0.0; dd[i] = 0.0; }
    double diag_low = 0.0;
    {
        int rem = tid, st = 1;
#pragma unroll
        for (int j = 0; j < K - RBD; ++j) {
            if (j < kk - RBD) {
                const int digit = rem % DIM;
                rem /= DIM;
                const int k = n - 1 - j;
                for (int q = 0; q < a.n_drives; ++q) {
                    const double* gq = tab + q * 3 * n;
                    const bool is_to = digit == a.to[q], is_from = digit == a.from[q];
                    if (is_to || is_from) {
                        const int off = tid + (is_to ? (a.from[q] - a.to[q]) : (a.to[q] - a.from[q])) * st;
                        const double gx = gq[2 * k];
                        const double gy = is_to ? gq[2 * k + 1] : -gq[2 * k + 1];
                        diag_low -= is_from ? gq[2 * n + k] : 0.0;
#pragma unroll
                        for (int i = 0; i < R; ++i) {
                            const c2 pv = tile[off + i * nt_act];
                            rr[i] = fma(gx, pv.x, rr[i]); rr[i] = fma(-gy, pv.y, rr[i]);
                            ri[i] = fma(gx, pv.y, ri[i]); ri[i] = fma(gy, pv.x, ri[i]);
                        }
                    }
                }
                st *= DIM;
            }
        }
    }
#pragma unroll
    for (int jj = 0; jj < RBD; ++jj) {
        const int j = kk - RBD + jj;
        const int k = n - 1 - j;
        const int stj = nt_act * ipow_c(DIM, jj);
        for (int q = 0; q < a.n_drives; ++q) {
            const double* gq = tab + q * 3 * n;
            const double gx0 = gq[2 * k], gy0 = gq[2 * k + 1], th = gq[2 * n + k];
            const int to = a.to[q], from = a.from[q];
#pragma unroll
            for (int i = 0; i < R; ++i) {
                const int digit = (i / ipow_c(DIM, jj)) % DIM;
                const bool is_to = digit == to, is_from = digit == from;
                if (is_to || is_from) {
                    const c2 pv = tile[tid + i * nt_act + (is_to ? (from - to) : (to - from)) * stj];
                    const double gy = is_to ? gy0 : -gy0;
                    rr[i] = fma(gx0, pv.x, rr[i]); rr[i] = fma(-gy, pv.y, rr[i]);
                    ri[i] = fma(gx0, pv.y, ri[i]); ri[i] = fma(gy, pv.x, ri[i]);
                    dd[i] -= is_from ? th : 0.0;
                }
            }
        }
    }
    const c2* vbase = a.v + voff + base + tid;
    const int nex = n_extra;
    for (int e = 0; e < nex; ++e) {
        const long long off = extra[e].off;
        const double gx = extra[e].gx, gy = extra[e].gy;
#pragma unroll
        for (int i = 0; i < R; ++i) {
// ... 707 lines not shown
```

### pulser_b200/csrc/plan.cu

```cuda
#include <cuda_runtime.h>

#include <algorithm>
#include <deque>
#include <map>
#include <memory>
#include <mutex>
#include <unordered_map>
#include <cmath>
#include <complex>
#include <cstdarg>
#include <cstdio>
#include <cstdlib>
#include <cstring>
#include <stdexcept>
#include <string>
#include <vector>

#include "../../include/pulser_b200.h"
#include "kernels.cuh"
#include "spline.hpp"
#include <cub/device/device_scan.cuh>
#include <nvtx3/nvToolsExt.h>
#include <random>

namespace pb200 {

static thread_local std::string g_last_error;

struct Error : std::runtime_error {
    int code;
    Error(int c, const std::string& m) : std::runtime_error(m), code(c) {}
};

[[noreturn]] static void fail(int code, const char* fmt, ...) {
    char buf[1024];
    va_list ap;
    va_start(ap, fmt);
    vsnprintf(buf, sizeof buf, fmt, ap);
    va_end(ap);
    throw Error(code, buf);
}

#define CUDA_CHECK(expr)                                                                        \
    do {                                                                                        \
        cudaError_t e__ = (expr);                                                               \
        if (e__ != cudaSuccess)                                                                 \
            fail(PB200_ERR_CUDA, "CUDA error %s at %s:%d: %s", #expr, __FILE__, __LINE__,       \
                 cudaGetErrorString(e__));                                                      \
    } while (0)

struct EventPair {
    cudaEvent_t a = nullptr, b = nullptr;
    EventPair() {
        CUDA_CHECK(cudaEventCreate(&a));
        if (cudaEventCreate(&b) != cudaSuccess) { cudaEventDestroy(a); a = nullptr; fail(PB200_ERR_CUDA, "cudaEventCreate failed"); }
    }
    ~EventPair() { if (a) cudaEventDestroy(a); if (b) cudaEventDestroy(b); }
    void start(cudaStream_t s) { CUDA_CHECK(cudaEventRecord(a, s)); }
    float stop_ms(cudaStream_t s) {
        CUDA_CHECK(cudaEventRecord(b, s));
        CUDA_CHECK(cudaEventSynchronize(b));
        float ms = 0.f;
        CUDA_CHECK(cudaEventElapsedTime(&ms, a, b));
        return ms;
    }
    EventPair(const EventPair&) = delete;
    EventPair& operator=(const EventPair&) = delete;
};

#define PB200_MAX_DEVICES 64

struct NvtxRange {
    explicit NvtxRange(const char* name) { nvtxRangePushA(name); }
    ~NvtxRange() { nvtxRangePop(); }
    NvtxRange(const NvtxRange&) = delete;
    NvtxRange& operator=(const NvtxRange&) = delete;
};

static int env_int(const char* name, int dflt) {
    const char* s = getenv(name);
    return s ? atoi(s) : dflt;
}

struct DevicePool {
    std::mutex mu;
    std::multimap<size_t, void*> free_list[PB200_MAX_DEVICES];
    std::unordered_map<void*, size_t> size_of;
    size_t held[PB200_MAX_DEVICES] = {0};
};
static DevicePool& pool() { static DevicePool* p = new DevicePool(); return *p; }

static void* pool_alloc(int dev, size_t bytes) {
    if (bytes == 0) bytes = 16;
    bytes = (bytes + 255) & ~(size_t)255;
    DevicePool& pl = pool();
    if (dev >= 0 && dev < PB200_MAX_DEVICES) {
        std::lock_guard<std::mutex> lk(pl.mu);
        auto it = pl.free_list[dev].lower_bound(bytes);
        if (it != pl.free_list[dev].end() && it->first <= bytes + bytes / 4) {
            void* p = it->second;
            pl.held[dev] -= it->first;
            pl.free_list[dev].erase(it);
            return p;
        }
    }
    void* p = nullptr;
    cudaError_t e = cudaMalloc(&p, bytes);
    if (e != cudaSuccess) {
        cudaGetLastError();
        {
            std::lock_guard<std::mutex> lk(pl.mu);
            if (dev >= 0 && dev < PB200_MAX_DEVICES) {
                for (auto& kv : pl.free_list[dev]) { pl.size_of.erase(kv.second); cudaFree(kv.second); }
                pl.free_list[dev].clear(); pl.held[dev] = 0;
            }
        }
        CUDA_CHECK(cudaMalloc(&p, bytes));
    }
    std::lock_guard<std::mutex> lk(pl.mu);
    pl.size_of[p] = bytes;
    return p;
}

static void pool_free(int dev, void* p) {
    if (!p) return;
    DevicePool& pl = pool();
    static const size_t cap = (size_t)std::max(0, env_int("PB200_POOL_MIB", 16384)) << 20;
    {
        std::lock_guard<std::mutex> lk(pl.mu);
        auto it = pl.size_of.find(p);
        if (it != pl.size_of.end() && dev >= 0 && dev < PB200_MAX_DEVICES && pl.held[dev] + it->second <= cap) {
            pl.free_list[dev].emplace(it->second, p);
            pl.held[dev] += it->second;
            return;
        }
        if (it != pl.size_of.end()) pl.size_of.erase(it);
    }
    cudaFree(p);
}

struct Plan;

template <typename T>
class DevBuf {
  public:
    DevBuf() = default;
    DevBuf(const Plan& P, size_t n) { reset(P, n); }
    DevBuf(DevBuf&& o) noexcept : dev_(o.dev_), stream_(o.stream_), n_(o.n_), p_(o.p_) { o.p_ = nullptr; o.n_ = 0; }
    DevBuf& operator=(DevBuf&& o) noexcept {
        if (this != &o) {
            release();
            dev_ = o.dev_; stream_ = o.stream_; n_ = o.n_; p_ = o.p_;
            o.p_ = nullptr; o.n_ = 0;
        }
        return *this;
    }
    DevBuf(const DevBuf&) = delete;
    DevBuf& operator=(const DevBuf&) = delete;
    ~DevBuf() { release(); }

    void reset(const Plan& P, size_t n);
    void release() noexcept {
        if (!p_) return;
        if (cudaStreamSynchronize(*stream_) != cudaSuccess) cudaGetLastError();
        pool_free(dev_, p_);
        p_ = nullptr; n_ = 0;
    }
    T* get() const { return p_; }
    size_t size() const { return n_; }
    explicit operator bool() const { return p_ != nullptr; }

  private:
    int dev_ = -1;
    const cudaStream_t* stream_ = nullptr;
    size_t n_ = 0;
    T* p_ = nullptr;
};

constexpr int kTaylorTileBits = 13;
constexpr int kTaylorRegBits = 4;
constexpr int kTaylorCplxRegBits = 5;
static size_t taylor_shapes_smem(int n) {
    return ((size_t)16 << kTaylorTileBits) +
           (size_t)(taylor_table_stride(n, PB200_TAYLOR_SMAX) +
                    (PB200_TAYLOR_PMAX + 1) * ((1 << kTaylorRegBits) + (1 << (kTaylorTileBits - kTaylorRegBits)))) * 8;
}
constexpr int kStageTileBits = 11;
constexpr int kStageRegBits = 3;
constexpr int kMaxExtraBits = 16;
constexpr int kShardMaxLocalBits = 29;
static_assert(kShardMaxLocalBits - kTaylorTileBits <= kMaxExtraBits, "a shard's local bits fit the single-pass geometry");

enum class TaylorSmem { Tile, TileTable, Shapes };
struct TaylorVariant {
    bool uniform, real_g, shard;
    int ns;
    bool cplx;
    void (*kernel)(TaylorArgs);
    int rb;
    TaylorSmem smem;
    bool pdl;
    bool diss = false;
};

static const std::vector<TaylorVariant>& taylor_variants() {
    constexpr int TB = kTaylorTileBits, RB = kTaylorRegBits, RBC = kTaylorCplxRegBits, SM = PB200_TAYLOR_SMAX;
    using S = TaylorSmem;
    static const std::vector<TaylorVariant> v = {
        {true,  true,  false, 0,  false, stage_d2_taylor_kernel<true, true, TB, RB, false, 0, false>,     RB,  S::Tile,      true},
        {true,  false, false, 0,  false, stage_d2_taylor_kernel<true, false, TB, RB, false, 0, false>,    RB,  S::TileTable, true},
        {false, false, false, 1,  false, stage_d2_taylor_kernel<false, false, TB, RB, false, 1, false>,   RB,  S::TileTable, true},
        {true,  true,  false, SM, false, stage_d2_taylor_kernel<true, true, TB, RB, false, SM, false>,    RB,  S::Shapes,    true},
        {true,  false, false, SM, false, stage_d2_taylor_kernel<true, false, TB, RB, false, SM, false>,   RB,  S::Shapes,    true},
        {false, false, false, SM, false, stage_d2_taylor_kernel<false, false, TB, RB, false, SM, false>,  RB,  S::Shapes,    true},
        {true,  true,  true,  0,  false, stage_d2_taylor_kernel<true, true, TB, RB, true, 0, false>,      RB,  S::Tile,      false},
        {true,  false, true,  0,  false, stage_d2_taylor_kernel<true, false, TB, RB, true, 0, false>,     RB,  S::TileTable, false},
        {true,  true,  true,  SM, false, stage_d2_taylor_kernel<true, true, TB, RB, true, SM, false>,     RB,  S::Shapes,    false},
        {true,  false, true,  SM, false, stage_d2_taylor_kernel<true, false, TB, RB, true, SM, false>,    RB,  S::Shapes,    false},
        {true,  false, false, 0,  true,  stage_d2_taylor_kernel<true, false, TB, RBC, false, 0, true>,    RBC, S::TileTable, true},
        {false, false, false, 1,  true,  stage_d2_taylor_kernel<false, false, TB, RBC, false, 1, true>,   RBC, S::TileTable, true},
        {true,  false, false, SM, true,  stage_d2_taylor_kernel<true, false, TB, RBC, false, SM, true>,   RBC, S::Shapes,    true},
        {false, false, false, SM, true,  stage_d2_taylor_kernel<false, false, TB, RBC, false, SM, true>,  RBC, S::Shapes,    true},
        {true,  false, true,  0,  true,  stage_d2_taylor_kernel<true, false, TB, RBC, true, 0, true>,     RBC, S::TileTable, false},
        {true,  false, true,  SM, true,  stage_d2_taylor_kernel<true, false, TB, RBC, true, SM, true>,    RBC, S::Shapes,    false},
        {false, false, false, 1,  false, stage_d2_taylor_kernel<false, false, TB, RBC, false, 1, false, true>,  RBC, S::TileTable, true, true},
        {false, false, false, SM, false, stage_d2_taylor_kernel<false, false, TB, RBC, false, SM, false, true>, RBC, S::Shapes,    true, true},
    };
    return v;
}

static size_t taylor_variant_smem(const TaylorVariant& v, int n) {
    const size_t tile = (size_t)16 << kTaylorTileBits;
    const size_t rest = v.smem == TaylorSmem::Shapes      ? taylor_shapes_smem(n) - tile
                        : v.smem == TaylorSmem::TileTable ? (size_t)d2_table_stride(n) * 8
                                                          : 0;
    return tile + (size_t)(taylor_dint_doubles(kTaylorTileBits, v.rb) + n * n) * 8 + rest;
}

static int device_setup(int dev) {
    static std::mutex mu;
    static int sm_count[PB200_MAX_DEVICES] = {0};
    std::lock_guard<std::mutex> lk(mu);
    if (dev >= 0 && dev < PB200_MAX_DEVICES && sm_count[dev] > 0) return sm_count[dev];
    int sms = 0;
    CUDA_CHECK(cudaDeviceGetAttribute(&sms, cudaDevAttrMultiProcessorCount, dev));
    const int max_smem = (1 << 13) * 16 + 1024;
    CUDA_CHECK(cudaFuncSetAttribute(stage_d2_kernel<true, true>, cudaFuncAttributeMaxDynamicSharedMemorySize, max_smem));
    CUDA_CHECK(cudaFuncSetAttribute(stage_d2_kernel<true, false>, cudaFuncAttributeMaxDynamicSharedMemorySize, max_smem));
    CUDA_CHECK(cudaFuncSetAttribute(stage_d2_kernel<false, false>, cudaFuncAttributeMaxDynamicSharedMemorySize, max_smem));
    constexpr int TB = kStageTileBits, RB = kStageRegBits;
    CUDA_CHECK(cudaFuncSetAttribute(stage_d2_rb_kernel<true, true, TB, RB>, cudaFuncAttributeMaxDynamicSharedMemorySize, max_smem));
    CUDA_CHECK(cudaFuncSetAttribute(stage_d2_rb_kernel<true, false, TB, RB>, cudaFuncAttributeMaxDynamicSharedMemorySize, max_smem));
    CUDA_CHECK(cudaFuncSetAttribute(stage_d2_rb_kernel<false, false, TB, RB>, cudaFuncAttributeMaxDynamicSharedMemorySize, max_smem));
    for (const TaylorVariant& v : taylor_variants())
        CUDA_CHECK(cudaFuncSetAttribute(v.kernel, cudaFuncAttributeMaxDynamicSharedMemorySize,
                                        (int)taylor_variant_smem(v, 64)));
    CUDA_CHECK(cudaFuncSetAttribute(stage_d2_fwd_kernel<true, TB, RB>, cudaFuncAttributeMaxDynamicSharedMemorySize, 2 * 2048 * 16 + 256));
    CUDA_CHECK(cudaFuncSetAttribute(stage_d2_fwd_kernel<false, TB, RB>, cudaFuncAttributeMaxDynamicSharedMemorySize, 2 * 2048 * 16 + 256));
    if (dev >= 0 && dev < PB200_MAX_DEVICES) sm_count[dev] = sms;
    return sms;
}

struct DriveTables {
    std::vector<PiecewiseCubic<cplx>> coef;
    std::vector<PiecewiseCubic<double>> det;
    std::vector<double> coef_scale, det_scale;
};

struct Plan {
    pb200_plan_desc desc;
    std::vector<double> times;
    int n = 0, dim = 0, B = 1;
    long long D = 0;
    int n_drives = 0;
    cudaStream_t stream = nullptr;
    struct OwnedStream {
        cudaStream_t s = nullptr;
        OwnedStream() = default;
        OwnedStream(const OwnedStream&) = delete;
        OwnedStream& operator=(const OwnedStream&) = delete;
        ~OwnedStream() { reset(); }
        void reset() {
            if (s) { cudaStreamSynchronize(s); cudaStreamDestroy(s); s = nullptr; }
        }
    } owned_stream;
    DevBuf<c2> buf[3];
    DevBuf<c2> aux[6];
    int cur = 0;
    DevBuf<double> dint;
    DevBuf<double> cpl;
    bool dint_shared = true;
    bool has_interaction = false;
    DevBuf<double> d_table;
    DevBuf<double> d_scratch;
    std::vector<std::vector<DriveTables>> tabs;
    std::vector<std::vector<bool>> tabs_set;
    std::vector<double> dmin_cnt, dmax_cnt;
    std::vector<double> dmin_traj, dmax_traj;
    bool state_set = false;
    int sm_count = 132;
    std::vector<std::vector<cplx>> diss_gen;
    DevBuf<c2> kry; int kry_cap = 0;
    DevBuf<double> d_kry;
    int m_last = 8;
    bool has_diss = false;
    struct DissTaylor {
        bool ok = false;
        const char* why = "";
        c2 dw[4] = {}, df[4] = {};
        bool flip = false;
        double norm = 0.0;
    } diss_tay;
    std::vector<std::vector<cplx>> jump_ops;
    std::vector<std::vector<double>> jump_ldl;
    std::vector<std::vector<cplx>> jump_ldl_full;
    bool jump_diag = true;
    bool has_collapse = false;
    DevBuf<double> d_xy; bool xy_shared = true; bool has_xy = false; int xy_u = 0, xy_d = 1;
    std::vector<double> xy_norm;
    bool has_slm = false; unsigned long long slm_bits = 0; PiecewiseCubic<double> slm_coef;
    DevBuf<double> dint2;
    std::vector<double> xy_norm2, dmin2_traj, dmax2_traj;
    std::mt19937_64 rng;
    std::vector<double> thresholds;
    std::vector<long long> jump_count;
    struct FineCache { bool valid = false; int window = -1; double rtol = -1.0; std::vector<char> fine, jump; std::vector<int> dist; } fine_cache;
    struct CtrlOptions {
        double gtol = 0.0; bool extrap = false; int order = 0, Kmax = 0;
        bool operator==(const CtrlOptions& o) const {
            return gtol == o.gtol && extrap == o.extrap && order == o.order && Kmax == o.Kmax;
        }
    };
    double ctrl_Kc = -1.0; CtrlOptions ctrl_opts; double ctrl_t_end = -1e300;
    DevBuf<c2> wbuf[2];
    struct TaylorCache {
        bool valid = false, ok = false;
        const char* why = "";
        c2 unit{1.0, 0.0};
        PiecewiseCubic<double> om;
        PiecewiseCubic<double> om_im;
        bool phase_moves = false;
        std::vector<double> w_knot;
        bool uniform = true;
        bool drive_uniform = true;
        int ns = 0;
        PiecewiseCubic<double> shape[PB200_TAYLOR_SMAX];
        std::vector<cplx> a;
        std::vector<double> c;
        double a_sum_max = 0.0;
        double c_sum_max[PB200_TAYLOR_SMAX] = {};
        int tab_shapes = 0;
        std::vector<double> tab_host;
        DevBuf<double> d_tab;
        c2 tab_unit{1.0, 0.0};
    } tay;
    std::vector<DevBuf<c2>> tay_ws;
    int shard_bits = 0, shard = 0;
    std::vector<Plan*> group;
    long long shard_offset() const { return (long long)shard << (n - shard_bits); }
    bool all_uniform() const {
        for (int q = 0; q < n_drives; ++q)
            if (!desc.drives[q].uniform) return false;
        return true;
    }
};

template <typename T>
void DevBuf<T>::reset(const Plan& P, size_t n) {
    release();
    dev_ = P.desc.device;
    stream_ = &P.stream;
    p_ = static_cast<T*>(pool_alloc(dev_, sizeof(T) * n));
    n_ = n;
}

template <typename F>
static void sum_launch(const Plan& P, double* acc, size_t n, F&& launch) {
    CUDA_CHECK(cudaMemsetAsync(acc, 0, sizeof(double) * n, P.stream));
    launch();
    CUDA_CHECK(cudaGetLastError());
}

static void sum_fetch(const Plan& P, const double* acc, size_t n, double* host) {
    CUDA_CHECK(cudaMemcpyAsync(host, acc, sizeof(double) * n, cudaMemcpyDeviceToHost, P.stream));
    CUDA_CHECK(cudaStreamSynchronize(P.stream));
}

template <typename F>
static void device_sum(const Plan& P, double* acc, size_t n, double* host, F&& launch) {
    sum_launch(P, acc, n, launch);
    sum_fetch(P, acc, n, host);
}

static void check_traj_range(const Plan& P, int traj0, int count, const char* who) {
    if (traj0 < 0 || count < 1 || traj0 + count > P.B)
        fail(PB200_ERR_INVALID, "%s: trajectory range [%d, %d) outside [0, %d)", who, traj0, traj0 + count, P.B);
}

static void check_drives_set(const Plan& P, const char* who) {
    for (int tr = 0; tr < P.B; ++tr)
        for (int q = 0; q < P.n_drives; ++q)
            if (!P.tabs_set[tr][q]) fail(PB200_ERR_STATE, "%s: drive %d of trajectory %d not set", who, q, tr);
}

template <typename... KArgs, typename... Args>
static void launch_k(void (*kernel)(KArgs...), dim3 grid, dim3 block, size_t smem, cudaStream_t st, bool pdl,
                     Args... args) {
    cudaLaunchConfig_t cfg = {};
    cfg.gridDim = grid; cfg.blockDim = block; cfg.dynamicSmemBytes = smem; cfg.stream = st;
    cudaLaunchAttribute attr[1];
    attr[0].id = cudaLaunchAttributeProgrammaticStreamSerialization;
    attr[0].val.programmaticStreamSerializationAllowed = 1;
    cfg.attrs = attr; cfg.numAttrs = pdl ? 1 : 0;
    CUDA_CHECK(cudaLaunchKernelEx(&cfg, kernel, KArgs(args)...));
}

static std::vector<PassGeom> plan_passes(int N, int TB, int EX) {
    std::vector<PassGeom> passes;
    PassGeom g{};
    g.n_bits = N;
    if (N <= TB) {
        g.lo_bits = N; g.hi_shift = N; g.hi_bits = 0;
        g.tile_flip_mask = (N >= 32) ? 0xffffffffu : ((1u << N) - 1u);
        g.extra_mask = 0; g.first_pass = 1;
        passes.push_back(g);
        return passes;
    }
    if (N - TB <= EX) {
        g.lo_bits = TB; g.hi_shift = TB; g.hi_bits = 0;
        g.tile_flip_mask = (1u << TB) - 1u;
        g.extra_mask = ((1ULL << N) - 1ULL) & ~((1ULL << TB) - 1ULL);
        g.first_pass = 1;
        passes.push_back(g);
        return passes;
    }
    g.lo_bits = TB; g.hi_shift = TB; g.hi_bits = 0;
    g.tile_flip_mask = (1u << TB) - 1u; g.extra_mask = 0; g.first_pass = 1;
    passes.push_back(g);
    int next = TB;
    const int min_row_bits = 2;
    while (next < N) {
        int rem = N - next;
        PassGeom p{};
        p.n_bits = N; p.first_pass = 0;
        int hb = std::min(rem, TB - min_row_bits);
        int left = rem - hb;
        p.hi_bits = hb; p.hi_shift = next; p.lo_bits = TB - hb;
        p.tile_flip_mask = ((1u << hb) - 1u) << p.lo_bits;
        p.extra_mask = 0;
        if (left > 0 && left <= EX) {
            p.extra_mask = ((1ULL << N) - 1ULL) & ~((1ULL << (next + hb)) - 1ULL);
            left = 0;
            next = N;
        } else {
            next += hb;
        }
        passes.push_back(p);
    }
    return passes;
}

struct ExpParams {
    std::vector<cplx> g;
    std::vector<double> th;
    double w = 0.0;
    double wc = 0.0;
};

static inline bool is_d2path(const Plan& P) { return P.dim == 2 && P.n_drives == 1 && !P.has_xy; }

static inline bool one_uniform_state(const Plan& P) { return is_d2path(P) && P.all_uniform() && P.B == 1; }

struct ExpChoice {
    bool krylov = false;
    bool fwd = false;
    PassGeom fwd_passes[3];
    std::vector<PassGeom> passes;
    bool dual_ok = false;
};

static inline size_t pidx(const Plan& P, int traj, int q, int row) {
    return ((size_t)traj * P.n_drives + q) * P.n + row;
}

struct StageIO {
    const c2* v; const c2* psi; const c2* b2; c2* out;
    StageCoef coef; UniformDrive ud; const double* table; bool real_g;
    const double* beta_dev = nullptr;
    double* dot_acc = nullptr;
    const LanczosFuse* lz = nullptr;
    int fwd_role = 0; bool fwd_emit = false; c2* wbuf = nullptr;
};

static StageArgs make_stage_args(const Plan& P, const PassGeom& geo, const StageIO& io, bool geo_is_last = true) {
    StageArgs a{};
    a.v = io.v; a.psi = io.psi; a.b2 = io.b2; a.out = io.out;
    a.dint = P.has_interaction ? P.dint.get() : nullptr;
    a.dint_stride = P.dint_shared ? 0 : P.D;
    a.D = P.D; a.geo = geo; a.coef = io.coef; a.u = io.ud; a.table = io.table;
    a.to_bit = P.desc.drives[0].state_to;
    a.from_is_one = P.desc.drives[0].state_from;
    a.beta_dev = io.beta_dev;
    a.dot_acc = (geo_is_last ? io.dot_acc : nullptr);
    if (geo_is_last && io.lz) a.lz = *io.lz;
    return a;
}

static bool multilevel_eligible(const Plan& P) {
    return !P.has_xy && (P.dim == 3 || P.dim == 4) && P.n <= PB200_TILED_MAX_HIGH &&
           P.n >= (P.dim == 3 ? 2 : 1) && !(P.dim == 2);
}

static bool rb_eligible(const PassGeom& geo) {
    return geo.lo_bits + geo.hi_bits == kStageTileBits && (geo.first_pass || geo.hi_bits >= kStageRegBits);
}

static bool dual_chain_ok(const Plan& P, const std::vector<PassGeom>& passes) {
    if (!is_d2path(P)) return false;
    for (const PassGeom& g : passes)
// ... 1356 lines not shown
    for (int b = 0; b < B; ++b) {
        double* t = tab.data() + (size_t)b * stride;
        for (int k = 0; k < N; ++k) {
            const int p = N - 1 - k;
            const cplx g = C.a[(size_t)b * N + k] * unit;
            t[2 * p] = g.real(); t[2 * p + 1] = g.imag();
            for (int s = 0; s < C.ns; ++s) t[2 * N + s * N + p] = C.c[((size_t)b * N + k) * C.ns + s];
        }
    }
    return tab;
}

static Plan::DissTaylor diss_taylor_analyse(const std::vector<std::vector<cplx>>& gen, int dim) {
    Plan::DissTaylor T;
    if (dim != 2) { T.why = "a master equation of d = 3 levels: the Taylor propagator takes d = 2 only"; return T; }
    const std::vector<cplx>& G = gen[0];
    double scale = 0.0;
    for (const std::vector<cplx>& g : gen)
        for (const cplx& z : g) scale = std::max(scale, std::abs(z));
    const double tiny = 1e-15 * scale;
    for (const std::vector<cplx>& g : gen)
        for (int i = 0; i < 16; ++i)
            if (std::abs(g[i] - G[i]) > tiny) { T.why = "the atoms carry different dissipator generators"; return T; }
    for (int i = 0; i < 4; ++i)
        for (int j = 0; j < 4; ++j)
            if (((i ^ j) == 1 || (i ^ j) == 2) && std::abs(G[i * 4 + j]) > tiny) {
                T.why = "the dissipator has single-bit-flip entries (a collapse operator mixes diagonal and off-diagonal "
                        "elements; each one diagonal or each one off-diagonal qualifies)";
                return T;
            }
    auto c = [](cplx z) { return c2{z.real(), z.imag()}; };
    const cplx g0 = G[0], g1 = G[5], g2 = G[10], g3 = G[15];
    T.dw[0] = c(g0 * (double)gen.size()); T.dw[1] = c(g2 - g0); T.dw[2] = c(g1 - g0); T.dw[3] = c(g0 - g1 - g2 + g3);
    double row = 0.0, col = 0.0;
    for (int i = 0; i < 4; ++i) {
        T.df[i] = c(G[i * 4 + (3 - i)]);
        T.flip = T.flip || G[i * 4 + (3 - i)] != 0.0;
        row = std::max(row, std::abs(G[i * 5]) + std::abs(G[i * 4 + (3 - i)]));
        col = std::max(col, std::abs(G[i * 5]) + std::abs(G[(3 - i) * 4 + i]));
    }
    T.norm = (double)gen.size() * std::max(row, col);
    T.ok = true;
    return T;
}

static const char* const kWhyMovingPhaseRho =
    "the drive phase moves: on a density matrix the column drive -conj(omega(t)) is not a multiple of omega(t)";

static bool taylor_prepare(Plan& P) {
    Plan::TaylorCache& C = P.tay;
    g_taylor_why = "structure (d, drives, collapse / mask, interpolation order)";
    if (P.has_diss && !P.diss_tay.ok) { g_taylor_why = P.diss_tay.why; return false; }
    if (!is_d2path(P)) return false;
    if (P.has_collapse || P.has_slm) return false;
    if (P.desc.interp_order != 3 && P.desc.interp_order != 1) return false;
    if (C.valid) { g_taylor_why = C.ok ? "" : C.why; return C.ok; }
    C.valid = true; C.ok = false;
    const int N = P.n, B = P.B, nt = (int)P.times.size();
    auto rows_of = [&](int b) { return (int)P.tabs[b][0].coef.size(); };
    auto coef_pc = [&](int b, int k) -> const PiecewiseCubic<cplx>& { return P.tabs[b][0].coef[rows_of(b) == 1 ? 0 : k]; };
    auto det_pc = [&](int b, int k) -> const PiecewiseCubic<double>& { return P.tabs[b][0].det[rows_of(b) == 1 ? 0 : k]; };
    std::vector<const PiecewiseCubic<cplx>*> crow((size_t)B * N);
    std::vector<const PiecewiseCubic<double>*> drow((size_t)B * N);
    for (int b = 0; b < B; ++b)
        for (int k = 0; k < N; ++k) { crow[(size_t)b * N + k] = &coef_pc(b, k); drow[(size_t)b * N + k] = &det_pc(b, k); }
    const int npc = nt - 1;
    const SeparableFit F = taylor_separable(
        B, N, nt,
        [&](int b, int k, int i) { const PiecewiseCubic<cplx>* pc = crow[(size_t)b * N + k]; return i < npc ? pc->c0[i] : pc->y_last; },
        [&](int b, int k, int i) { const PiecewiseCubic<double>* pc = drow[(size_t)b * N + k]; return i < npc ? pc->c0[i] : pc->y_last; },
        PB200_TAYLOR_SMAX);
    if (!F.ok) {
        g_taylor_why = C.why = (P.has_diss && F.why == kWhyDriveRows) ? kWhyMovingPhaseRho : F.why;
        return false;
    }
    const double scale = F.scale;
    const cplx unit = scale > 0.0 ? F.big / scale : cplx(1.0, 0.0);
    const cplx cu = std::conj(unit);
    const PiecewiseCubic<cplx>& ref = coef_pc(F.ref_b, F.ref_k);
    const int np = ref.pieces();
    C.om = PiecewiseCubic<double>();
    C.om.c0.resize(np); C.om.c1.resize(np); C.om.c2.resize(np); C.om.c3.resize(np);
    C.om_im = C.om;
    C.phase_moves = false;
    for (int i = 0; i < np; ++i) {
        const double hi = P.times[i + 1] - P.times[i];
        const cplx v0 = ref.c0[i] * cu, v1 = ref.c1[i] * cu, v2 = ref.c2[i] * cu, v3 = ref.c3[i] * cu;
        const double im = std::max(std::max(std::fabs(v0.imag()), std::fabs(v1.imag()) * hi),
                                   std::max(std::fabs(v2.imag()) * hi * hi, std::fabs(v3.imag()) * hi * hi * hi));
        if (im > 1e-13 * scale) C.phase_moves = true;
        C.om.c0[i] = v0.real(); C.om.c1[i] = v1.real(); C.om.c2[i] = v2.real(); C.om.c3[i] = v3.real();
        C.om_im.c0[i] = v0.imag(); C.om_im.c1[i] = v1.imag(); C.om_im.c2[i] = v2.imag(); C.om_im.c3[i] = v3.imag();
    }
    C.om.y_last = (ref.y_last * cu).real();
    C.om_im.y_last = (ref.y_last * cu).imag();
    if (!C.phase_moves) C.om_im = PiecewiseCubic<double>();
    else if (P.has_diss) { g_taylor_why = C.why = kWhyMovingPhaseRho; return false; }
    C.unit = {unit.real(), unit.imag()};
    C.a = F.a; C.c = F.c; C.ns = F.ns;
    for (int s = 0; s < C.ns; ++s) C.shape[s] = make_interpolant<double>(P.times.data(), F.m[s].data(), nt, P.desc.interp_order);
    C.drive_uniform = B == 1 && !P.has_diss;
    C.a_sum_max = 0.0;
    for (int s = 0; s < PB200_TAYLOR_SMAX; ++s) C.c_sum_max[s] = 0.0;
    for (int b = 0; b < B; ++b) {
        double sa = 0.0, sc[PB200_TAYLOR_SMAX] = {};
        for (int k = 0; k < N; ++k) {
            sa += std::abs(C.a[(size_t)b * N + k]);
            for (int s = 0; s < C.ns; ++s) sc[s] += std::fabs(C.c[((size_t)b * N + k) * C.ns + s]);
            if (std::abs(C.a[(size_t)b * N + k] - cplx(1.0, 0.0)) > 0.0) C.drive_uniform = false;
        }
        C.a_sum_max = std::max(C.a_sum_max, sa);
        for (int s = 0; s < C.ns; ++s) C.c_sum_max[s] = std::max(C.c_sum_max[s], sc[s]);
    }
    C.uniform = C.drive_uniform && C.ns == 0;
    C.tab_shapes = (C.ns > 1 || (C.drive_uniform && C.ns == 1)) ? PB200_TAYLOR_SMAX : 0;
    if (!C.uniform) {
        C.tab_host = taylor_table(P, unit);
        C.d_tab.reset(P, C.tab_host.size());
        CUDA_CHECK(cudaMemcpyAsync(C.d_tab.get(), C.tab_host.data(), C.tab_host.size() * sizeof(double), cudaMemcpyHostToDevice,
                                   P.stream));
        C.tab_unit = C.unit;
    }
    C.w_knot.clear();
    C.ok = true;
    return true;
}

static void taylor_table_unit(Plan& P, c2 unit, std::deque<std::vector<double>>& keep) {
    Plan::TaylorCache& C = P.tay;
    if (C.uniform || (unit.x == C.tab_unit.x && unit.y == C.tab_unit.y)) return;
    keep.push_back(taylor_table(P, cplx(unit.x, unit.y)));
    CUDA_CHECK(cudaMemcpyAsync(C.d_tab.get(), keep.back().data(), keep.back().size() * sizeof(double), cudaMemcpyHostToDevice,
                               P.stream));
    C.tab_unit = unit;
}

static void taylor_bounds(const Plan& P, double om, double th, const double* mv, double& centre, double& half) {
    const int N = P.n;
    const Plan::TaylorCache& C = P.tay;
    double lo = 1e300, hi = -1e300;
    const bool caseA = C.drive_uniform && P.has_interaction && P.dint_shared &&
                       P.desc.drives[0].state_from == P.desc.rydberg_state && !P.dmin_cnt.empty();
    if (caseA) {
        const double dr = std::fabs(om) * N;
        std::vector<double> small(N + 1, 0.0), large(N + 1, 0.0);
        if (C.ns) {
            std::vector<double> e(N, 0.0);
            for (int k = 0; k < N; ++k)
                for (int s = 0; s < C.ns; ++s) e[k] += C.c[(size_t)k * C.ns + s] * mv[s];
            std::sort(e.begin(), e.end());
            for (int c = 1; c <= N; ++c) { small[c] = small[c - 1] + e[c - 1]; large[c] = large[c - 1] + e[N - c]; }
        }
        double dlo = 1e300, dhi = -1e300;
        for (int c = 0; c <= N; ++c) {
            if (P.dmin_cnt[c] > P.dmax_cnt[c]) continue;
            dlo = std::min(dlo, P.dmin_cnt[c] - th * c - large[c]);
            dhi = std::max(dhi, P.dmax_cnt[c] - th * c - small[c]);
        }
        lo = dlo - dr; hi = dhi + dr;
    } else {
        for (int b = 0; b < P.B; ++b) {
            double dr = 0.0;
            double dlo = 0.0, dhi = 0.0;
            if (P.has_interaction) {
                dlo = P.dint_shared ? P.dmin_traj[0] : P.dmin_traj[b];
                dhi = P.dint_shared ? P.dmax_traj[0] : P.dmax_traj[b];
            }
            for (int k = 0; k < N; ++k) {
                dr += std::abs(C.a[(size_t)b * N + k]);
                double e = 0.0;
                for (int s = 0; s < C.ns; ++s) e += C.c[((size_t)b * N + k) * C.ns + s] * mv[s];
                const double val = -(th + e);
                dlo += std::min(0.0, val); dhi += std::max(0.0, val);
            }
            dr *= std::fabs(om);
            lo = std::min(lo, dlo - dr); hi = std::max(hi, dhi + dr);
        }
    }
    centre = 0.5 * (lo + hi);
    half = std::max(0.5 * (hi - lo) * (1.0 + 1e-9), 1e-9);
}

static void taylor_knot_widths(Plan& P) {
    Plan::TaylorCache& C = P.tay;
    const int nt = (int)P.times.size();
    if ((int)C.w_knot.size() == nt) return;
    const int order = P.desc.interp_order;
    const PiecewiseCubic<double>& th_pc = P.tabs[0][0].det[0];
    C.w_knot.resize(nt);
    for (int i = 0; i < nt; ++i) {
        double c, hw, mv[PB200_TAYLOR_SMAX] = {};
        for (int s = 0; s < C.ns; ++s) mv[s] = eval_at(C.shape[s], P.times, P.times[i], order);
        double om = eval_at(C.om, P.times, P.times[i], order);
        if (C.phase_moves) om = std::hypot(om, eval_at(C.om_im, P.times, P.times[i], order));
        taylor_bounds(P, om, eval_at(th_pc, P.times, P.times[i], order), mv, c, hw);
        C.w_knot[i] = hw + P.diss_tay.norm;
    }
}

static bool taylor_worthwhile(Plan& P, double gtol) {
    const int nt = (int)P.times.size();
    if (nt < 8) return false;
    const double rate = gtol / std::max(P.times.back() - P.times.front(), 1e-30);
    const double allow = 0.25 * rate / P.n;
    std::vector<const PiecewiseCubic<double>*> pcs = {&P.tay.om, &P.tabs[0][0].det[0]};
    if (P.tay.phase_moves) pcs.push_back(&P.tay.om_im);
    for (int s = 0; s < P.tay.ns; ++s) pcs.push_back(&P.tay.shape[s]);
    std::vector<char> rough(nt, 0);
    for (const PiecewiseCubic<double>* pc : pcs) {
        const int np = pc->pieces();
        auto y = [&](int i) { return i < np ? pc->c0[i] : pc->y_last; };
        for (int i = 2; i + 2 < nt; ++i) {
            const double d4 = std::fabs(y(i + 2) - 4.0 * y(i + 1) + 6.0 * y(i) - 4.0 * y(i - 1) + y(i - 2));
            if (d4 / 384.0 > allow) rough[i] = 1;
        }
    }
    int cnt = 0;
    for (char c : rough) cnt += c;
    if (4 * cnt > nt) { g_taylor_why = "splines too rough for multi-interval polynomial steps"; return false; }
    if (P.has_diss) return true;
    taylor_knot_widths(P);
    double wsum = 0.0;
    for (int i = 0; i + 1 < nt; ++i) wsum += 0.5 * (P.tay.w_knot[i] + P.tay.w_knot[i + 1]) * (P.times[i + 1] - P.times[i]);
    const double applies_per_interval = 4.1 * wsum / std::max(nt - 1, 1);
    const double hi_mean_ns = (P.times.back() - P.times.front()) / std::max(nt - 1, 1) * 1e3;
    constexpr double kTaylorMaxAppliesPerNs = 12.0;
    const bool cheap = applies_per_interval / std::max(hi_mean_ns, 1e-30) <= kTaylorMaxAppliesPerNs;
    if (!cheap) g_taylor_why = "spectrum too wide: the Krylov path is expected to be cheaper";
    return cheap;
}

struct TaylorPoly {
    std::vector<double> c;
    double resid = 0.0;
};

static TaylorPoly taylor_fit(const PiecewiseCubic<double>& pc, const std::vector<double>& x, int order, double a, double h,
                             int p) {
    typedef long double ld;
    const ld PI = 3.14159265358979323846264338327950288L;
    const int m = p + 1;
    std::vector<ld> f(m), ck(m, 0.0L);
    for (int i = 0; i < m; ++i) {
        const ld xi = cosl(PI * (2 * i + 1) / (2.0L * m));
        f[i] = (ld)eval_at(pc, x, a + h * (double)(0.5L * (xi + 1.0L)), order);
    }
    for (int k = 0; k < m; ++k) {
        ld s = 0.0L;
        for (int i = 0; i < m; ++i) s += f[i] * cosl(PI * k * (2 * i + 1) / (2.0L * m));
        ck[k] = s * (k == 0 ? 1.0L : 2.0L) / m;
    }
    std::vector<ld> mono(m, 0.0L), Tm2(m, 0.0L), Tm1(m, 0.0L), Tk(m, 0.0L);
    Tm2[0] = 1.0L;
    mono[0] += ck[0];
    if (m > 1) { Tm1[1] = 1.0L; for (int i = 0; i < m; ++i) mono[i] += ck[1] * Tm1[i]; }
    for (int k = 2; k < m; ++k) {
        for (int i = 0; i < m; ++i) Tk[i] = (i > 0 ? 2.0L * Tm1[i - 1] : 0.0L) - Tm2[i];
        for (int i = 0; i < m; ++i) mono[i] += ck[k] * Tk[i];
        Tm2 = Tm1; Tm1 = Tk;
    }
    std::vector<ld> cu(m, 0.0L), pw(m, 0.0L), nx(m, 0.0L);
    pw[0] = 1.0L;
    for (int k = 0; k < m; ++k) {
        for (int i = 0; i < m; ++i) cu[i] += mono[k] * pw[i];
        for (int i = 0; i < m; ++i) nx[i] = (i > 0 ? 2.0L * pw[i - 1] : 0.0L) - pw[i];
        pw = nx;
    }
    TaylorPoly out;
    out.c.resize(m);
    for (int i = 0; i < m; ++i) out.c[i] = (double)cu[i];
    const int ia = find_piece(x, a + 1e-15), ib = find_piece(x, a + h - 1e-15);
    const int npts = std::max(9, 4 * (ib - ia + 1) + 1);
    double r = 0.0;
    for (int q = 0; q < npts; ++q) {
        const double u = (double)q / (npts - 1);
        double pv = 0.0;
        for (int i = m - 1; i >= 0; --i) pv = pv * u + out.c[i];
        r = std::max(r, std::fabs(pv - eval_at(pc, x, a + h * u, order)));
    }
    out.resid = r;
    return out;
}

static int taylor_order(double h, const std::vector<double>& mj, double tol, double& tail_out) {
    const int p = (int)mj.size() - 1;
    std::vector<double> y(1, 1.0);
    const int kcap = 1200;
    for (int k = 0; k < kcap; ++k) {
        double s = 0.0;
        for (int j = 0; j <= std::min(p, k); ++j) s += mj[j] * y[k - j];
        y.push_back(h * s / (k + 1));
        if (k > 8 && y.back() < 1e-40 && y.back() < y[k]) break;
    }
    double tail = 0.0;
    int kk = (int)y.size() - 1;
    for (; kk >= 1; --kk) {
        if (tail + y[kk] > tol) break;
        tail += y[kk];
    }
    tail_out = tail;
    return std::max(kk, 1);
}

static void launch_taylor_order(const Plan& P, bool tiled, const TaylorArgs& a, bool cplx) {
    const bool diss = a.n_pair > 0;
    if (!tiled) {
        const dim3 grid((unsigned)((P.D + 255) / 256), (unsigned)P.B);
        if (diss && !cplx) stage_d2_taylor_small_kernel<false, true><<<grid, 256, 0, P.stream>>>(a);
        else if (diss) fail(PB200_ERR_UNSUPPORTED, "no Taylor stage kernel for a dissipator with a complex drive");
        else if (cplx) stage_d2_taylor_small_kernel<true><<<grid, 256, 0, P.stream>>>(a);
        else stage_d2_taylor_small_kernel<false><<<grid, 256, 0, P.stream>>>(a);
        return;
    }
    const bool uniform = !a.table || (a.tab_shapes && P.tay.drive_uniform);
    const bool real_g = uniform && !cplx && a.unit.y == 0.0;
    const bool shard = a.shard_bits > 0;
    const int ns = a.tab_shapes ? PB200_TAYLOR_SMAX : uniform ? 0 : 1;
    for (const TaylorVariant& v : taylor_variants()) {
        if (v.uniform != uniform || v.real_g != real_g || v.shard != shard || v.ns != ns || v.cplx != cplx ||
            v.diss != diss)
            continue;
        launch_k(v.kernel, dim3((unsigned)(P.D >> kTaylorTileBits), uniform ? 1u : (unsigned)P.B),
                 dim3(1u << (kTaylorTileBits - v.rb)), taylor_variant_smem(v, P.n), P.stream, v.pdl, a);
        return;
    }
    fail(PB200_ERR_UNSUPPORTED, "no Taylor stage kernel for UNIFORM=%d REAL_G=%d SHARD=%d NS=%d CPLX=%d DISS=%d", uniform,
         real_g, shard, ns, cplx, diss);
}

static bool taylor_geometry(const Plan& P, PassGeom& geo, bool& tiled) {
    const int L = P.n - P.shard_bits;
    const std::vector<PassGeom> passes = plan_passes(L, kTaylorTileBits, kMaxExtraBits);
    if (P.shard_bits && passes.size() != 1) fail(PB200_ERR_UNSUPPORTED, "shard of 2^%d amplitudes: no single-pass geometry", L);
    geo = passes[0];
    geo.n_bits = P.n;
    tiled = passes.size() == 1 && geo.first_pass && geo.hi_bits == 0 && geo.lo_bits == kTaylorTileBits;
    return tiled || P.n <= 16;
}

struct TaylorStep {
    double t = 0.0, h = 0.0;
    std::vector<double> om, th;
    std::vector<double> m[PB200_TAYLOR_SMAX];
    int p_om = 0, p_th = 0, p = 0;
    std::vector<double> gam;
    int K = 0;
    double phi = 0.0;
    int n_chi = 0, n_g = 0;
    int drive = 0;
    c2 unit{1.0, 0.0};
    std::vector<double> omi;
    int ring() const { return (n_chi - 1) + n_g * (drive == 2 ? 2 : 1) + 1; }
};

struct TaylorScheduler {
    Plan& P;
    double t_stop, eps = 1e-12, gtol, rate, rho_target, fit_total, fit_spent = 0.0, round2 = 0.0;
    double t, steps_len = 0.0, t_retry_len = 0.0, A_sum, C_sum[PB200_TAYLOR_SMAX], kRoundUnit = 0.05 * 1.1102230246251565e-16;
    int order, N, nt, ns;
    bool log_steps;
    pb200_run_stats st{};
    struct Fit { TaylorPoly om, omi, th, m[PB200_TAYLOR_SMAX]; double om_allow = 0.0; bool ok; };

    TaylorScheduler(Plan& P_, double t_start, double t_stop_, const pb200_run_opts* o) : P(P_), t_stop(t_stop_), t(t_start) {
        const double tlo = P.times.front(), thi = P.times.back();
        gtol = taylor_default_tol(P, o);
        rate = gtol / std::max(thi - tlo, 1e-30);
        constexpr double kTaylorRhoMax = 14.0;
        order = P.desc.interp_order;
        N = P.n;
        nt = (int)P.times.size();
        Plan::TaylorCache& C = P.tay;
        taylor_knot_widths(P);
        rho_target = kTaylorRhoMax;
        {
            double w_total = 0.0;
            for (int i = 0; i + 1 < nt; ++i) w_total += 0.5 * (C.w_knot[i] + C.w_knot[i + 1]) * (P.times[i + 1] - P.times[i]);
            for (int it = 0; it < 3; ++it) {
                const double n_est = std::max(w_total / std::max(rho_target, 1.0), 1.0);
                rho_target = std::min(kTaylorRhoMax, std::max(4.0, std::log(0.2 * gtol / (kRoundUnit * std::sqrt(n_est)))));
            }
        }
        A_sum = std::max(C.a_sum_max, 1e-300);
        ns = C.ns;
        for (int s = 0; s < PB200_TAYLOR_SMAX; ++s) C_sum[s] = std::max(C.c_sum_max[s], 1e-300);
        fit_total = 0.5 * rate * (t_stop - t_start);
        log_steps = env_int("PB200_TAYLOR_LOG", 0) != 0;
    }

    Fit fit_step(double a, double h, bool single_piece) {
        const Plan::TaylorCache& C = P.tay;
        Fit F; F.ok = false;
        const double budget = std::max(0.5 * rate * h, 0.02 * std::max(fit_total - fit_spent, 0.0));
        const double third = budget / (3.0 * h);
        auto one = [&](const PiecewiseCubic<double>& pc, TaylorPoly& out, double allow) {
            if (!single_piece) {
                out = taylor_fit(pc, P.times, order, a, h, PB200_TAYLOR_PMAX);
                if (out.resid > allow) return false;
            }
            for (int p = 0; p < PB200_TAYLOR_PMAX; ++p) {
                TaylorPoly f = taylor_fit(pc, P.times, order, a, h, p);
                if (f.resid <= allow || (single_piece && p >= 3)) { out = f; return true; }
            }
            if (single_piece) out = taylor_fit(pc, P.times, order, a, h, PB200_TAYLOR_PMAX);
            return true;
        };
        F.om_allow = third / A_sum;
        if (C.phase_moves) F.ok = one(C.om, F.om, 0.5 * F.om_allow) && one(C.om_im, F.omi, 0.5 * F.om_allow);
        else F.ok = one(C.om, F.om, F.om_allow);
        F.ok = F.ok && one(P.tabs[0][0].det[0], F.th, third / N);
        for (int s = 0; s < ns && F.ok; ++s) F.ok = one(C.shape[s], F.m[s], third / ns / C_sum[s]);
        for (int s = ns; s < PB200_TAYLOR_SMAX; ++s) { F.m[s].c.assign(1, 0.0); F.m[s].resid = 0.0; }
        return F;
    }

    double candidate_end(int i0) {
        const Plan::TaylorCache& C = P.tay;
        double b = t, acc = 0.0, cur = t;
        int i = i0;
        while (i < nt - 1) {
            const double e1 = std::min(P.times[i + 1], t_stop);
            const double w = std::max(C.w_knot[i], C.w_knot[i + 1]);
            const double need = w * (e1 - cur);
            if (acc + need > rho_target) {
                if (i == i0 || acc == 0.0) b = cur + (rho_target - acc) / std::max(w, 1e-300);
                else b = cur;
                break;
            }
            acc += need; cur = e1; b = e1; ++i;
            if (e1 >= t_stop - eps) break;
        }
        b = std::min(b, t_stop);
        if (t_retry_len > 0.0) { b = std::min(b, t + t_retry_len); t_retry_len = 0.0; }
        if (b <= t + eps) b = std::min(P.times[i0 + 1], t_stop);
        return b;
    }

    Fit longest_fit(int i0, double& b) {
        const bool single = b <= P.times[i0 + 1] + eps;
        Fit F = fit_step(t, b - t, single);
        if (F.ok || single) return F;
        int lo_keep = 0, hi_keep = find_piece(P.times, b - eps) - i0;
        Fit Flo; bool have_lo = false;
        while (hi_keep - lo_keep > 1) {
            const int mid = (lo_keep + hi_keep) / 2;
            const double bm = P.times[i0 + 1 + mid];
            Fit Fm = fit_step(t, bm - t, false);
            if (Fm.ok) { lo_keep = mid; Flo = Fm; have_lo = true; } else hi_keep = mid;
        }
        b = P.times[i0 + 1 + lo_keep];
        return have_lo ? Flo : fit_step(t, b - t, lo_keep == 0);
    }

    double classify_drive(Fit& F, int& drive, c2& unit) const {
        auto coef = [](const std::vector<double>& c, size_t j) { return j < c.size() ? c[j] : 0.0; };
        auto poly = [](const std::vector<double>& c, double u) {
            double v = 0.0;
            for (int i = (int)c.size() - 1; i >= 0; --i) v = v * u + c[i];
            return v;
        };
        double best = 0.0, cph = 1.0, sph = 0.0;
        for (double u : {0.0, 0.5, 1.0}) {
            const double x = poly(F.om.c, u), y = poly(F.omi.c, u), r = std::hypot(x, y);
            if (r > best) { best = r; cph = x / r; sph = y / r; }
        }
        const size_t nc = std::max(F.om.c.size(), F.omi.c.size());
        std::vector<double> xr(nc), yr(nc);
        double ybound = 0.0;
        for (size_t j = 0; j < nc; ++j) {
            xr[j] = cph * coef(F.om.c, j) + sph * coef(F.omi.c, j);
            yr[j] = cph * coef(F.omi.c, j) - sph * coef(F.om.c, j);
            ybound += std::fabs(yr[j]);
        }
        const double r2 = F.om.resid + F.omi.resid;
        if (r2 + ybound <= F.om_allow) {
            F.om.c = xr;
            if (cph != 1.0 || sph != 0.0) {
                const c2 u = P.tay.unit;
                drive = 1;
                unit = {u.x * cph - u.y * sph, u.x * sph + u.y * cph};
            }
            return r2 + ybound;
        }
        drive = 2;
        return r2;
    }

    static int trim(Fit& F, bool cplx) {
        auto trim1 = [](std::vector<double>& c, double scale) {
            while (c.size() > 1 && std::fabs(c.back()) <= 1e-15 * scale) c.pop_back();
        };
        double so = 0.0, sh = 0.0;
        for (double v : F.om.c) so = std::max(so, std::fabs(v));
        if (cplx) for (double v : F.omi.c) so = std::max(so, std::fabs(v));
        for (double v : F.th.c) sh = std::max(sh, std::fabs(v));
        trim1(F.om.c, std::max(so, 1e-300)); trim1(F.th.c, std::max(sh, 1e-300));
        if (cplx) trim1(F.omi.c, std::max(so, 1e-300));
        int p_m = 0;
        for (int q = 0; q < PB200_TAYLOR_SMAX; ++q) {
            double sm = 0.0;
            for (double v : F.m[q].c) sm = std::max(sm, std::fabs(v));
            trim1(F.m[q].c, std::max(sm, 1e-300));
            p_m = std::max(p_m, (int)F.m[q].c.size() - 1);
        }
        return p_m;
    }

    void centres_and_bounds(const Fit& F, bool cplx, int p_om, int p, std::vector<double>& gam, std::vector<double>& mj) const {
        auto th_c = [&](int j) { return j < (int)F.th.c.size() ? F.th.c[j] : 0.0; };
        auto m_c = [&](int q, int j) { return j < (int)F.m[q].c.size() ? F.m[q].c[j] : 0.0; };
        auto om_abs = [&](int j) {
            const double x = j < (int)F.om.c.size() ? F.om.c[j] : 0.0;
            if (!cplx) return std::fabs(x);
            return std::hypot(x, j < (int)F.omi.c.size() ? F.omi.c[j] : 0.0);
        };
        gam.assign(p + 1, 0.0); mj.assign(p + 1, 0.0);
        double c0, hw0, mv[PB200_TAYLOR_SMAX];
        for (int q = 0; q < PB200_TAYLOR_SMAX; ++q) mv[q] = m_c(q, 0);
        taylor_bounds(P, cplx ? om_abs(0) : F.om.c[0], F.th.c[0], mv, c0, hw0);
        gam[0] = c0; mj[0] = hw0 + P.diss_tay.norm;
        for (int j = 1; j <= p; ++j) {
            const double thj = th_c(j), omj = j <= p_om ? om_abs(j) : 0.0;
            gam[j] = -thj * 0.5 * N;
            double mm = 0.0;
            for (int q = 0; q < ns; ++q) mm += std::fabs(m_c(q, j)) * C_sum[q];
            mj[j] = std::fabs(thj) * 0.5 * N + mm + std::fabs(omj) * A_sum;
        }
    }

    void record(TaylorStep& s, const Fit& F, const std::vector<double>& mj, int p_m, double om_resid, double rho) {
        double trunc_bound = 0.0;
        s.K = taylor_order(s.h, mj, std::max(1e-15, 0.1 * rate * s.h), trunc_bound);
        st.n_applies += s.K; st.n_exponentials += 1; ++st.n_steps;
        if (log_steps)
            fprintf(stderr, "taylor step t=%.6f h_ns=%.3f p_om=%d p_th=%d p_m=%d K=%d ring=%d rho=%.3f resid=%.2e/%.2e/%.2e drive=%s\n",
                    s.t, s.h * 1e3, s.p_om, s.p_th, p_m, s.K, s.ring() + 1, mj[0] * s.h, om_resid, F.th.resid, F.m[0].resid,
                    s.drive == 2 ? "cplx" : s.drive == 1 ? "rot" : "real");
        st.max_rho = std::max(st.max_rho, rho);
        double fit_m = 0.0;
        for (int q = 0; q < ns; ++q) fit_m += C_sum[q] * F.m[q].resid;
        const double fit_err = s.h * (A_sum * om_resid + N * F.th.resid + fit_m);
        st.err_estimate += trunc_bound + fit_err;
        fit_spent += fit_err;
        { const double r = kRoundUnit * std::exp(std::min(rho, 40.0)); round2 += r * r; }
        steps_len += s.h;
    }

    bool next(TaylorStep& s) {
        while (t < t_stop - eps) {
            const int i0 = find_piece(P.times, t + eps);
            double b = candidate_end(i0);
            Fit F = longest_fit(i0, b);
            const double h = b - t;
            int drive = 0;
            c2 unit = P.tay.unit;
            const double om_resid = P.tay.phase_moves ? classify_drive(F, drive, unit) : F.om.resid;
            const int p_m = trim(F, drive == 2);
            const int p_om = std::max((int)F.om.c.size(), drive == 2 ? (int)F.omi.c.size() : 0) - 1;
            const int p_th = std::max((int)F.th.c.size() - 1, p_m);
            const int p = std::max(p_om, p_th);
            std::vector<double> gam, mj;
            centres_and_bounds(F, drive == 2, p_om, p, gam, mj);
            double rho = 0.0;
            for (int j = 0; j <= p; ++j) rho += mj[j] / (j + 1);
            rho *= h;
            if (rho > 1.12 * rho_target && h > 1e-9) {
                t_retry_len = h * rho_target / rho;
                continue;
            }
            s.t = t; s.h = h;
            s.om = F.om.c; s.th = F.th.c;
            for (int q = 0; q < PB200_TAYLOR_SMAX; ++q) s.m[q] = F.m[q].c;
            s.p_om = p_om; s.p_th = p_th; s.p = p;
            s.gam = gam;
            s.n_chi = p_th + 2;
            s.n_g = p_om >= 1 ? p_om + 1 : 0;
            s.drive = drive; s.unit = unit;
            s.omi = drive == 2 ? F.omi.c : std::vector<double>();
            double phi = 0.0;
            for (int j = 0; j <= p; ++j) phi += gam[j] / (j + 1);
            s.phi = phi * h;
            record(s, F, mj, p_m, om_resid, rho);
            t = b;
            return true;
        }
        return false;
    }

    pb200_run_stats finish(double gpu_ms, long long launches) const {
        pb200_run_stats out = st;
        out.gpu_ms = gpu_ms;
        out.n_launches = launches;
        const double hi_mean = (P.times.back() - P.times.front()) / std::max(nt - 1, 1);
        out.mean_step_samples = out.n_steps ? steps_len / out.n_steps / hi_mean : 0.0;
        out.err_estimate += std::sqrt(round2);
        out.integrator = 3;
        return out;
    }
};

struct TaylorRing {
    std::vector<c2*> chi, gr, gr2;
    DevBuf<c2>* acc_slot = nullptr;
};

static void taylor_grow_ring(Plan& P, int need) {
    int have = 2 + (P.aux[0] ? 6 : 0) + (int)P.tay_ws.size();
    while (have < need) {
        P.tay_ws.emplace_back(P, (size_t)P.D * P.B);
        ++have;
    }
}

static TaylorRing taylor_ring(Plan& P, const TaylorStep& s) {
    std::vector<DevBuf<c2>*> free_slots;
    for (int i = 0; i < 3; ++i) if (i != P.cur) free_slots.push_back(&P.buf[i]);
    if (P.aux[0]) for (int i = 0; i < 6; ++i) free_slots.push_back(&P.aux[i]);
    taylor_grow_ring(P, s.ring());
    for (size_t i = 0; i < P.tay_ws.size(); ++i) free_slots.push_back(&P.tay_ws[i]);
    TaylorRing R;
    R.chi.resize(s.n_chi); R.gr.resize(s.n_g); R.gr2.resize(s.drive == 2 ? s.n_g : 0);
    int fs = 0;
    R.chi[0] = P.buf[P.cur].get();
    for (int i = 1; i < s.n_chi; ++i) R.chi[i] = free_slots[fs++]->get();
    for (int i = 0; i < s.n_g; ++i) R.gr[i] = free_slots[fs++]->get();
    for (size_t i = 0; i < R.gr2.size(); ++i) R.gr2[i] = free_slots[fs++]->get();
    R.acc_slot = free_slots[fs++];
    return R;
}

static TaylorArgs taylor_plan_args(const Plan& P, const PassGeom& geo, const c2* v, c2* out, c2 unit) {
    TaylorArgs a{};
    a.v = v; a.out = out;
    a.dint = P.has_interaction ? P.dint.get() : nullptr;
    a.dint_stride = P.dint_shared ? 0 : P.D;
    a.cpl = P.has_interaction ? P.cpl.get() : nullptr;
    a.cpl_stride = P.dint_shared ? 0 : (long long)P.n * P.n;
    a.ryd_bit = P.desc.rydberg_state;
    a.D = P.D;
    a.geo = geo;
    a.unit = unit;
    a.table = P.tay.uniform ? nullptr : P.tay.d_tab.get();
    a.tab_shapes = P.tay.tab_shapes;
    a.to_bit = P.desc.drives[0].state_to; a.from_is_one = P.desc.drives[0].state_from;
    a.shard_bits = P.shard_bits; a.shard = P.shard;
    if (P.has_diss) {
        for (int i = 0; i < 4; ++i) { a.dw[i] = P.diss_tay.dw[i]; a.df[i] = P.diss_tay.df[i]; }
        a.n_pair = P.n / 2;
        a.diss_flip = P.diss_tay.flip ? 1 : 0;
    }
    return a;
}

static TaylorArgs taylor_args(const Plan& P, const PassGeom& geo, const TaylorStep& s, const TaylorRing& R, int k) {
    auto th_c = [&](int j) { return j < (int)s.th.size() ? s.th[j] : 0.0; };
    auto m_c = [&](int q, int j) { return j < (int)s.m[q].size() ? s.m[q][j] : 0.0; };
    TaylorArgs a = taylor_plan_args(P, geo, R.chi[k % s.n_chi], R.chi[(k + 1) % s.n_chi], s.unit);
    a.g_out = (s.n_g && k + 1 < s.K) ? R.gr[k % s.n_g] : nullptr;
    a.acc = R.acc_slot->get();
    a.th0 = s.th[0]; a.gam0 = s.gam[0]; a.om0 = s.om[0];
    for (int q = 0; q < PB200_TAYLOR_SMAX; ++q) a.m0[q] = m_c(q, 0);
    a.scale = {0.0, -s.h / (k + 1)};
    a.nh = std::min(s.p, k);
    for (int j = 1; j <= a.nh; ++j) {
        const double thj = th_c(j), omj = j < (int)s.om.size() ? s.om[j] : 0.0;
        bool any_m = false;
        for (int q = 0; q < PB200_TAYLOR_SMAX; ++q) { a.hm[q][j - 1] = m_c(q, j); any_m = any_m || a.hm[q][j - 1] != 0.0; }
        a.hth[j - 1] = thj; a.hgam[j - 1] = s.gam[j]; a.hom[j - 1] = omj;
        a.hchi[j - 1] = (thj != 0.0 || any_m || s.gam[j] != 0.0) ? R.chi[(k - j) % s.n_chi] : nullptr;
        a.hg[j - 1] = (omj != 0.0) ? R.gr[(k - j) % s.n_g] : nullptr;
        if (s.drive == 2) {
            const double omij = j < (int)s.omi.size() ? s.omi[j] : 0.0;
            a.homi[j - 1] = omij;
            a.hg2[j - 1] = (omij != 0.0) ? R.gr2[(k - j) % s.n_g] : nullptr;
        }
    }
    if (s.drive == 2) {
        a.om0i = s.omi[0];
        a.g2_out = (s.n_g && k + 1 < s.K) ? R.gr2[k % s.n_g] : nullptr;
    }
    const bool last = (k + 1 == s.K);
    bool chi_hist = false;
    if (s.p >= 1) {
        chi_hist = th_c(1) != 0.0 || s.gam[1] != 0.0;
        for (int q = 0; q < PB200_TAYLOR_SMAX; ++q) chi_hist = chi_hist || m_c(q, 1) != 0.0;
    }
    const int period = chi_hist ? 3 : 2;
    a.acc_read = k > 0;
    if (k % period == 0) { a.acc_on = 1; a.acc_add_v = 1; a.acc_add_h = k > 0 && chi_hist; }
    else { a.acc_on = last ? 1 : 0; a.acc_add_v = k % period == 2; a.acc_add_h = 0; }
    a.acc_mul = last ? c2{std::cos(s.phi), -std::sin(s.phi)} : c2{1.0, 0.0};
    return a;
}

struct ShardEvents {
    std::vector<cudaEvent_t> ev;
    ShardEvents(const std::vector<Plan*>& G, unsigned flags) : ev(G.size(), nullptr) {
        for (size_t r = 0; r < G.size(); ++r) {
            CUDA_CHECK(cudaSetDevice(G[r]->desc.device));
            CUDA_CHECK(cudaEventCreateWithFlags(&ev[r], flags));
        }
    }
    ~ShardEvents() { for (cudaEvent_t e : ev) if (e) cudaEventDestroy(e); }
    ShardEvents(const ShardEvents&) = delete;
    ShardEvents& operator=(const ShardEvents&) = delete;
};

template <class Next>
static float taylor_launch_steps(const std::vector<Plan*>& G, const PassGeom& geo, bool tiled, Next&& next,
                                 long long& launches) {
    const int count = (int)G.size(), sb = count > 1 ? G[0]->shard_bits : 0;
    auto use = [&](int r) -> Plan& {
        if (count > 1) CUDA_CHECK(cudaSetDevice(G[r]->desc.device));
        return *G[r];
    };
    ShardEvents order_ev(sb ? G : std::vector<Plan*>(), cudaEventDisableTiming), t0(G, cudaEventDefault),
        t1(G, cudaEventDefault);
    for (int r = 0; r < count; ++r) CUDA_CHECK(cudaEventRecord(t0.ev[r], use(r).stream));
    bool first = true;
    std::vector<TaylorRing> R(count);
    std::deque<std::vector<double>> tables;
    for (TaylorStep s; next(s);) {
        for (int r = 0; r < count; ++r) {
            Plan& P = use(r);
            R[r] = taylor_ring(P, s);
            taylor_table_unit(P, s.drive == 1 ? s.unit : P.tay.unit, tables);
        }
        for (int k = 0; k < s.K; ++k) {
            for (int r = 0; r < count; ++r) {
                Plan& P = use(r);
                TaylorArgs a = taylor_args(P, geo, s, R[r], k);
                for (int q = 0; q < sb; ++q) {
                    const int peer = r ^ (1 << q);
                    a.peer[q] = R[peer].chi[k % s.n_chi];
                    if (!first) CUDA_CHECK(cudaStreamWaitEvent(P.stream, order_ev.ev[peer], 0));
                }
                launch_taylor_order(P, tiled, a, s.drive == 2);
                ++launches;
            }
            for (int r = 0; r < count && sb; ++r) CUDA_CHECK(cudaEventRecord(order_ev.ev[r], use(r).stream));
            first = false;
        }
        CUDA_CHECK(cudaGetLastError());
        for (int r = 0; r < count; ++r) std::swap(G[r]->buf[G[r]->cur], *R[r].acc_slot);
    }
    float ms_max = 0.f;
    for (int r = 0; r < count; ++r) CUDA_CHECK(cudaEventRecord(t1.ev[r], use(r).stream));
    for (int r = 0; r < count; ++r) {
        CUDA_CHECK(cudaEventSynchronize(t1.ev[r]));
        float ms = 0.f;
        CUDA_CHECK(cudaEventElapsedTime(&ms, t0.ev[r], t1.ev[r]));
        ms_max = std::max(ms_max, ms);
    }
    return ms_max;
}

static void propagate_taylor(Plan& P, double t_start, double t_stop, const pb200_run_opts* o, pb200_run_stats* stats) {
    PassGeom geo;
    bool tiled = false;
    if (!taylor_geometry(P, geo, tiled)) fail(PB200_ERR_UNSUPPORTED, "Taylor propagator: unsupported register size");
    ensure_aux_buffers(P);
    TaylorScheduler S(P, t_start, t_stop, o);
    long long launches = 0;
    const float ms = taylor_launch_steps({&P}, geo, tiled, [&S](TaylorStep& s) { return S.next(s); }, launches);
    if (stats) *stats = S.finish(ms, launches);
}

static ExpParams params_at(const Plan& P, double t) {
    ExpParams E;
    const int N = P.n, B = P.B, nd = P.n_drives;
    E.g.assign((size_t)B * nd * N, cplx(0)); E.th.assign((size_t)B * nd * N, 0.0); E.w = 1.0;
    if (P.has_slm) E.wc = eval_at(P.slm_coef, P.times, t, P.desc.interp_order);
    for (int tr = 0; tr < B; ++tr)
        for (int q = 0; q < nd; ++q) {
            const DriveTables& T = P.tabs[tr][q];
            const int rows = (int)T.coef.size();
            for (int k = 0; k < N; ++k) {
                const int r = rows == 1 ? 0 : k;
                E.g[pidx(P, tr, q, k)] = eval_at(T.coef[r], P.times, t, P.desc.interp_order);
                E.th[pidx(P, tr, q, k)] = eval_at(T.det[r], P.times, t, P.desc.interp_order);
            }
        }
    return E;
}

struct ApplyH {
    bool uniform, real_g;
    UniformDrive ud{};
    std::vector<PassGeom> passes;

    void launch(Plan& P, const c2* in, c2* out, long long& launches) const {
        launch_stage(P, passes, in, nullptr, nullptr, out, StageCoef{{0, 0}, {0, 0}, {1, 0}}, uniform, real_g, ud,
                     P.d_table.get(), launches);
    }
};

static ApplyH apply_h_device(Plan& P, double t, const c2* in, c2* out, long long& launches) {
    const ExpParams E = params_at(P, t);
    double gamma0, rho; std::vector<double> host;
    build_tables(P, E, gamma0, rho, host, is_d2path(P), false);
    ensure_table_capacity(P, host.size());
    CUDA_CHECK(cudaMemcpyAsync(P.d_table.get(), host.data(), host.size() * sizeof(double), cudaMemcpyHostToDevice, P.stream));
    CUDA_CHECK(cudaStreamSynchronize(P.stream));
    ApplyH A;
    A.uniform = one_uniform_state(P);
    A.real_g = E.g[0].imag() == 0.0;
    A.ud.g = {E.g[0].real(), E.g[0].imag()}; A.ud.theta = E.th[0]; A.ud.w = 1.0; A.ud.gamma = 0.0;
    A.passes = plan_passes(P.n, kStageTileBits, kMaxExtraBits);
    A.launch(P, in, out, launches);
    CUDA_CHECK(cudaGetLastError());
    return A;
}

}

using namespace pb200;

struct pb200_plan {
    Plan p;
};

static void refuse_shard(const Plan& P, const char* who, const char* instead) {
    if (P.shard_bits)
        fail(PB200_ERR_STATE, "%s: the plan is shard %d of %d of a state; use %s on the linked shards", who, P.shard,
             1 << P.shard_bits, instead);
}


static std::vector<Plan*> shard_group(pb200_plan** plans, int count, const char* who) {
    if (!plans || count < 2) fail(PB200_ERR_INVALID, "%s: pass the plans of every shard", who);
    std::vector<Plan*> G(count);
    for (int i = 0; i < count; ++i) {
        if (!plans[i]) fail(PB200_ERR_INVALID, "%s: null plan", who);
        G[i] = &plans[i]->p;
    }
    for (int i = 0; i < count; ++i)
        if (G[i]->group != G)
            fail(PB200_ERR_STATE, "%s: plans[] is not a linked shard group in shard order (pb200_shards_link)", who);
    return G;
}

static void shards_sync(const std::vector<Plan*>& G) {
    for (Plan* P : G) {
        CUDA_CHECK(cudaSetDevice(P->desc.device));
        CUDA_CHECK(cudaStreamSynchronize(P->stream));
    }
}

static void shards_apply_h(const std::vector<Plan*>& G, double t, const std::vector<c2*>& in, const std::vector<c2*>& out) {
    const Plan& P0 = *G[0];
    PassGeom geo;
    bool tiled = false;
    taylor_geometry(P0, geo, tiled);
    const int order = P0.desc.interp_order;
    const double om = eval_at(P0.tay.om, P0.times, t, order), th = eval_at(P0.tabs[0][0].det[0], P0.times, t, order);
    const bool cplx = P0.tay.phase_moves;
    shards_sync(G);
    const int count = (int)G.size();
    std::deque<std::vector<double>> tables;
    for (int r = 0; r < count; ++r) {
        Plan& P = *G[r];
        CUDA_CHECK(cudaSetDevice(P.desc.device));
        taylor_table_unit(P, P.tay.unit, tables);
        TaylorArgs a = taylor_plan_args(P, geo, in[r], out[r], P.tay.unit);
        if (cplx) a.om0i = eval_at(P0.tay.om_im, P0.times, t, order);
        for (int s = 0; s < P.tay.ns; ++s) a.m0[s] = eval_at(P.tay.shape[s], P.times, t, order);
        a.th0 = th; a.om0 = om;
        a.scale = {1.0, 0.0};
        a.acc_mul = {1.0, 0.0};
        for (int q = 0; q < P.shard_bits; ++q) a.peer[q] = in[r ^ (1 << q)];
        launch_taylor_order(P, tiled, a, cplx);
    }
    CUDA_CHECK(cudaGetLastError());
    shards_sync(G);
}

static void check_op_terms(const pb200_op_terms* op, int n, int dim, const char* who) {
    if (!op) fail(PB200_ERR_INVALID, "%s: null operator", who);
    if (op->n_terms < 0) fail(PB200_ERR_INVALID, "%s: n_terms = %d", who, op->n_terms);
    if (op->n_terms == 0) return;
    if (!op->coeff || !op->site_start) fail(PB200_ERR_INVALID, "%s: null coeff or site_start", who);
    if (op->site_start[0] != 0) fail(PB200_ERR_INVALID, "%s: site_start[0] = %d, must be 0", who, op->site_start[0]);
    for (int t = 0; t < op->n_terms; ++t)
        if (op->site_start[t + 1] < op->site_start[t]) fail(PB200_ERR_INVALID, "%s: site_start decreases at term %d", who, t);
    if (op->site_start[op->n_terms] > 0 && (!op->site || !op->shift || !op->weight))
        fail(PB200_ERR_INVALID, "%s: null site, shift or weight", who);
    for (int t = 0; t < op->n_terms; ++t) {
        unsigned long long seen = 0;
        for (int e = op->site_start[t]; e < op->site_start[t + 1]; ++e) {
            const int k = op->site[e], m = op->shift[e];
            if (k < 0 || k >= n) fail(PB200_ERR_INVALID, "%s: term %d names qudit %d of a %d-qudit register", who, t, k, n);
            if ((seen >> k) & 1ull) fail(PB200_ERR_INVALID, "%s: term %d names qudit %d twice", who, t, k);
            seen |= 1ull << k;
            if (m < 0 || m >= dim) fail(PB200_ERR_INVALID, "%s: term %d: shift %d outside [0, %d)", who, t, m, dim);
        }
    }
}

struct ExpHost {
    bool d2 = true;
    std::vector<char> img;
    size_t off_sites = 0, off_ct = 0, off_cs = 0;
    int n_chunks = 0;
    unsigned used_shard_bits = 0;
};

template <typename TermT, typename SiteT>
static void exp_pack(std::vector<std::pair<TermT, std::vector<SiteT>>>& B, ExpHost& H) {
    std::vector<TermT> T;
    std::vector<SiteT> S;
    std::vector<int> ct{0}, cs{0};
    int nt = 0, ns = 0;
    for (auto& b : B) {
        if (nt == kExpChunkTerms || ns + (int)b.second.size() > kExpChunkSites) {
            ct.push_back((int)T.size()); cs.push_back((int)S.size());
            nt = ns = 0;
        }
        b.first.s0 = ns; b.first.sn = (int)b.second.size();
        T.push_back(b.first);
        S.insert(S.end(), b.second.begin(), b.second.end());
        ++nt; ns += (int)b.second.size();
    }
    if (nt) { ct.push_back((int)T.size()); cs.push_back((int)S.size()); }
    H.n_chunks = (int)ct.size() - 1;
    auto al = [](size_t x) { return (x + 255) & ~(size_t)255; };
    H.off_sites = al(sizeof(TermT) * T.size());
    H.off_ct = H.off_sites + al(sizeof(SiteT) * S.size());
    H.off_cs = H.off_ct + al(sizeof(int) * ct.size());
    H.img.assign(H.off_cs + sizeof(int) * cs.size(), 0);
    if (!T.empty()) std::memcpy(H.img.data(), T.data(), sizeof(TermT) * T.size());
    if (!S.empty()) std::memcpy(H.img.data() + H.off_sites, S.data(), sizeof(SiteT) * S.size());
    std::memcpy(H.img.data() + H.off_ct, ct.data(), sizeof(int) * ct.size());
    std::memcpy(H.img.data() + H.off_cs, cs.data(), sizeof(int) * cs.size());
}

static ExpHost exp_host_d2(const pb200_op_terms* op, int n, int local_bits) {
    std::vector<std::pair<ExpD2Term, std::vector<ExpGenSite>>> B;
    const cplx* co = reinterpret_cast<const cplx*>(op->coeff);
    const cplx* w = reinterpret_cast<const cplx*>(op->weight);
    for (int t = 0; t < op->n_terms; ++t) {
        ExpD2Term T{};
        std::vector<ExpGenSite> gen;
        cplx c = co[t];
        for (int e = op->site_start[t]; e < op->site_start[t + 1] && c != 0.0; ++e) {
            const unsigned long long bit = 1ull << (n - 1 - op->site[e]);
            const cplx w0 = w[2 * e], w1 = w[2 * e + 1];
            if (op->shift[e]) T.f |= bit;
            if (w0 == 0.0) { T.care |= bit; T.val |= bit; c *= w1; }
            else if (w1 == 0.0) { T.care |= bit; c *= w0; }
            else {
                c *= w0;
                const cplx r = w1 / w0;
                if (r == -1.0) T.z |= bit;
                else if (r != 1.0) gen.push_back({{r.real(), r.imag()}, bit});
            }
        }
        if (c == 0.0) continue;
        T.c = {c.real(), c.imag()};
        B.emplace_back(T, std::move(gen));
    }
    std::stable_sort(B.begin(), B.end(), [](const auto& x, const auto& y) { return x.first.f < y.first.f; });
    ExpHost H;
    for (const auto& b : B) H.used_shard_bits |= 1u << (unsigned)(b.first.f >> local_bits);
    exp_pack(B, H);
    return H;
}

static ExpHost exp_host_general(const pb200_op_terms* op, int n, int dim) {
    std::vector<std::pair<ExpTerm, std::vector<ExpSite>>> B;
    const cplx* co = reinterpret_cast<const cplx*>(op->coeff);
    const cplx* w = reinterpret_cast<const cplx*>(op->weight);
    for (int t = 0; t < op->n_terms; ++t) {
        if (co[t] == 0.0) continue;
// ... 865 lines not shown
    evs.start(P.stream);
    for (int r = 0; r < reps; ++r) A.launch(P, in, outb, launches);
    *ms_out = evs.stop_ms(P.stream);
    CUDA_CHECK(cudaGetLastError());
    if (launches_out) *launches_out = launches;
    PB200_CATCH
}

int pb200_shards_link(pb200_plan** plans, int32_t count) {
    PB200_TRY
    NvtxRange nvtx_range("pb200_shards_link");
    if (!plans) fail(PB200_ERR_INVALID, "null argument");
    if (count != 2 && count != 4 && count != 8) fail(PB200_ERR_INVALID, "pb200_shards_link: count = %d, must be 2, 4 or 8", count);
    std::vector<Plan*> G(count);
    for (int i = 0; i < count; ++i) {
        if (!plans[i]) fail(PB200_ERR_INVALID, "pb200_shards_link: null plan");
        G[i] = &plans[i]->p;
    }
    for (int i = 0; i < count; ++i) {
        Plan& P = *G[i];
        if ((1 << P.shard_bits) != count) fail(PB200_ERR_INVALID, "pb200_shards_link: plans[%d] is not one of %d shards", i, count);
        if (P.shard != i) fail(PB200_ERR_INVALID, "pb200_shards_link: plans[%d] is shard %d (plans[i] must be shard i)", i, P.shard);
        if (P.n != G[0]->n || P.times != G[0]->times || P.desc.interp_order != G[0]->desc.interp_order)
            fail(PB200_ERR_INVALID, "pb200_shards_link: the shards differ in N, sampling times or interpolation order");
        if (P.has_interaction != G[0]->has_interaction || (P.has_interaction && !P.dint_shared))
            fail(PB200_ERR_INVALID, "pb200_shards_link: every shard needs the same (shared) interaction");
        if (!P.tabs_set[0][0]) fail(PB200_ERR_STATE, "pb200_shards_link: the drive of shard %d is not set", i);
        if (!taylor_prepare(P)) fail(PB200_ERR_UNSUPPORTED, "pb200_shards_link: no Taylor propagator for this sequence: %s", g_taylor_why);
        if (!P.tay.drive_uniform)
            fail(PB200_ERR_UNSUPPORTED, "pb200_shards_link: shards need one drive coefficient for every qubit (per-qubit drive "
                                        "amplitudes are not sharded; per-qubit detuning is)");
    }
    for (int i = 0; i < count; ++i)
        for (int q = 0; (1 << q) < count; ++q) {
            const int di = G[i]->desc.device, dj = G[i ^ (1 << q)]->desc.device;
            if (di == dj) continue;
            int can = 0;
            CUDA_CHECK(cudaDeviceCanAccessPeer(&can, di, dj));
            if (!can) fail(PB200_ERR_UNSUPPORTED, "pb200_shards_link: device %d cannot access the memory of device %d (no peer access)", di, dj);
            CUDA_CHECK(cudaSetDevice(di));
            const cudaError_t e = cudaDeviceEnablePeerAccess(dj, 0);
            if (e == cudaErrorPeerAccessAlreadyEnabled) cudaGetLastError();
            else CUDA_CHECK(e);
        }
    if (G[0]->has_interaction) {
        std::vector<double> mins = G[0]->dmin_cnt, maxs = G[0]->dmax_cnt;
        double mn = G[0]->dmin_traj[0], mx = G[0]->dmax_traj[0];
        for (int i = 1; i < count; ++i) {
            for (size_t c = 0; c < mins.size(); ++c) {
                mins[c] = std::min(mins[c], G[i]->dmin_cnt[c]);
                maxs[c] = std::max(maxs[c], G[i]->dmax_cnt[c]);
            }
            mn = std::min(mn, G[i]->dmin_traj[0]); mx = std::max(mx, G[i]->dmax_traj[0]);
        }
        for (Plan* P : G) { P->dmin_cnt = mins; P->dmax_cnt = maxs; P->dmin_traj[0] = mn; P->dmax_traj[0] = mx; }
    }
    for (Plan* P : G) { P->tay.w_knot.clear(); P->group = G; }
    PB200_CATCH
}

int pb200_shards_propagate(pb200_plan** plans, int32_t count, double t_start, double t_stop, const pb200_run_opts* o,
                           pb200_run_stats* stats) {
    PB200_TRY
    NvtxRange nvtx_range("pb200_shards_propagate");
    const std::vector<Plan*> G = shard_group(plans, count, "pb200_shards_propagate");
    if (o && ((o->integrator != 0 && o->integrator != 3) || o->max_step_samples > 0 || o->tol < 0.0))
        fail(PB200_ERR_UNSUPPORTED, "pb200_shards_propagate: shards run the Taylor propagator only (integrator 0 or 3, "
                                    "max_step_samples = 0, tol >= 0)");
    for (int r = 0; r < count; ++r)
        if (!G[r]->state_set) fail(PB200_ERR_STATE, "pb200_shards_propagate: no state set on shard %d", r);
    Plan& P0 = *G[0];
    const double tlo = P0.times.front(), thi = P0.times.back(), eps = 1e-12;
    if (t_start < tlo - eps || t_stop > thi + eps || t_stop < t_start)
        fail(PB200_ERR_INVALID, "pb200_shards_propagate: [%g, %g] outside sampling times [%g, %g]", t_start, t_stop, tlo, thi);
    t_start = std::max(t_start, tlo); t_stop = std::min(t_stop, thi);
    PassGeom geo;
    bool tiled = false;
    taylor_geometry(P0, geo, tiled);
    TaylorScheduler S(P0, t_start, t_stop, o);
    std::vector<TaylorStep> steps;
    for (TaylorStep s; S.next(s);) steps.push_back(s);
    int need = 0;
    for (const TaylorStep& s : steps) need = std::max(need, s.ring());
    for (Plan* P : G) {
        CUDA_CHECK(cudaSetDevice(P->desc.device));
        try {
            taylor_grow_ring(*P, need);
        } catch (const Error& e) {
            fail(PB200_ERR_CUDA, "pb200_shards_propagate: this call needs the state and %d more state-sized buffers per shard, "
                                 "%lld bytes each (%d amplitudes x 16 B) besides the 8 B/amplitude interaction diagonal: %s",
                 need, (long long)(16 * P->D), (int)P->D, e.what());
        }
    }
    long long launches = 0;
    size_t i = 0;
    auto next = [&](TaylorStep& s) {
        if (i == steps.size()) return false;
        s = steps[i++];
        return true;
    };
    const float ms = taylor_launch_steps(G, geo, tiled, next, launches);
    if (stats) *stats = S.finish(ms, launches);
    PB200_CATCH
}

int pb200_shards_apply_h(pb200_plan** plans, int32_t count, double t_us, const double* in, double* out) {
    PB200_TRY
    NvtxRange nvtx_range("pb200_shards_apply_h");
    if (!in || !out) fail(PB200_ERR_INVALID, "null argument");
    const std::vector<Plan*> G = shard_group(plans, count, "pb200_shards_apply_h");
    std::vector<c2*> bin(count), bout(count);
    for (int r = 0; r < count; ++r) {
        Plan& P = *G[r];
        bin[r] = P.buf[(P.cur + 1) % 3].get(); bout[r] = P.buf[(P.cur + 2) % 3].get();
        CUDA_CHECK(cudaSetDevice(P.desc.device));
        CUDA_CHECK(cudaMemcpyAsync(bin[r], in + (size_t)2 * P.D * r, sizeof(c2) * (size_t)P.D, cudaMemcpyHostToDevice, P.stream));
    }
    shards_apply_h(G, t_us, bin, bout);
    for (int r = 0; r < count; ++r) {
        Plan& P = *G[r];
        CUDA_CHECK(cudaSetDevice(P.desc.device));
        CUDA_CHECK(cudaMemcpyAsync(out + (size_t)2 * P.D * r, bout[r], sizeof(c2) * (size_t)P.D, cudaMemcpyDeviceToHost, P.stream));
    }
    shards_sync(G);
    PB200_CATCH
}

int pb200_shards_energy(pb200_plan** plans, int32_t count, double t_us, double* energy, double* h2) {
    PB200_TRY
    NvtxRange nvtx_range("pb200_shards_energy");
    if (!energy || !h2) fail(PB200_ERR_INVALID, "null argument");
    const std::vector<Plan*> G = shard_group(plans, count, "pb200_shards_energy");
    std::vector<c2*> psi(count), hpsi(count);
    for (int r = 0; r < count; ++r) {
        if (!G[r]->state_set) fail(PB200_ERR_STATE, "pb200_shards_energy: no state set on shard %d", r);
        psi[r] = G[r]->buf[G[r]->cur].get(); hpsi[r] = G[r]->buf[(G[r]->cur + 2) % 3].get();
    }
    shards_apply_h(G, t_us, psi, hpsi);
    double e = 0.0, e2 = 0.0;
    for (int r = 0; r < count; ++r) {
        Plan& P = *G[r];
        CUDA_CHECK(cudaSetDevice(P.desc.device));
        const long long blocks = std::min<long long>((P.D + 255) / 256, (long long)P.sm_count * 8);
        double acc[2];
        device_sum(P, P.d_scratch.get(), 2, acc, [&] {
            dot2_kernel<<<dim3((unsigned)std::max<long long>(blocks, 1), 1), 256, 0, P.stream>>>(psi[r], hpsi[r], P.D,
                                                                                                 P.d_scratch.get());
        });
        e += acc[0]; e2 += acc[1];
    }
    energy[0] = e; h2[0] = e2;
    PB200_CATCH
}

int pb200_shards_expect(pb200_plan** plans, int32_t count, const pb200_op_terms* op, double* out) {
    PB200_TRY
    NvtxRange nvtx_range("pb200_shards_expect");
    if (!out) fail(PB200_ERR_INVALID, "pb200_shards_expect: null argument");
    const std::vector<Plan*> G = shard_group(plans, count, "pb200_shards_expect");
    const Plan& P0 = *G[0];
    check_op_terms(op, P0.n, P0.dim, "pb200_shards_expect");
    for (int r = 0; r < count; ++r)
        if (!G[r]->state_set) fail(PB200_ERR_STATE, "pb200_shards_expect: no state set on shard %d", r);
    out[0] = out[1] = 0.0;
    const int L = P0.n - P0.shard_bits;
    const ExpHost H = exp_host(op, P0.n, P0.dim, L);
    if (H.n_chunks == 0) return PB200_OK;
    for (int x = 1; x < count; ++x) {
        if (!((H.used_shard_bits >> x) & 1u)) continue;
        for (int r = 0; r < count; ++r) {
            const int di = G[r]->desc.device, dj = G[r ^ x]->desc.device;
            if (di == dj) continue;
            int can = 0;
            CUDA_CHECK(cudaDeviceCanAccessPeer(&can, di, dj));
            if (!can)
                fail(PB200_ERR_UNSUPPORTED, "pb200_shards_expect: the operator pairs shards %d and %d, but device %d cannot "
                                            "access the memory of device %d (no peer access)", r, r ^ x, di, dj);
            CUDA_CHECK(cudaSetDevice(di));
            const cudaError_t e = cudaDeviceEnablePeerAccess(dj, 0);
            if (e == cudaErrorPeerAccessAlreadyEnabled) cudaGetLastError();
            else CUDA_CHECK(e);
        }
    }
    ExpSrc src{};
    src.local_bits = L;
    for (int r = 0; r < count; ++r) src.p[r] = G[r]->buf[G[r]->cur].get();
    std::vector<DevBuf<char>> X(count);
    std::vector<DevBuf<double>> acc(count);
    struct GroupIdle {
        const std::vector<Plan*>& G;
        ~GroupIdle() {
            for (Plan* P : G)
                if (cudaStreamSynchronize(P->stream) != cudaSuccess) cudaGetLastError();
        }
    } idle{G};
    shards_sync(G);
    for (int r = 0; r < count; ++r) {
        Plan& P = *G[r];
        CUDA_CHECK(cudaSetDevice(P.desc.device));
        X[r] = upload_exp(H, P);
        acc[r].reset(P, 2);
        src.shard = r;
        sum_launch(P, acc[r].get(), 2, [&] { launch_expect<false>(P, P.D, H, X[r].get(), src, nullptr, 1, acc[r].get()); });
    }
    for (int r = 0; r < count; ++r) {
        double a[2];
        CUDA_CHECK(cudaSetDevice(G[r]->desc.device));
        sum_fetch(*G[r], acc[r].get(), 2, a);
        out[0] += a[0]; out[1] += a[1];
    }
    shards_sync(G);
    PB200_CATCH
}

int pb200_host_interpolate(const double* x, const double* y, int32_t n, int32_t order, const double* tq, int32_t nq,
                           double* out) {
    PB200_TRY
    if (!x || !y || !tq || !out || n < 2) fail(PB200_ERR_INVALID, "bad argument");
    std::vector<double> xs(x, x + n);
    auto pc = make_interpolant<cplx>(x, reinterpret_cast<const cplx*>(y), n, order);
    for (int i = 0; i < nq; ++i) {
        const cplx v = eval_at(pc, xs, tq[i], order);
        out[2 * i] = v.real(); out[2 * i + 1] = v.imag();
    }
    PB200_CATCH
}

int pb200_host_moments(const double* x, const double* y, int32_t n, int32_t order, double a, double b, double* out4) {
    PB200_TRY
    if (!x || !y || !out4 || n < 2) fail(PB200_ERR_INVALID, "bad argument");
    std::vector<double> xs(x, x + n);
    auto pc = make_interpolant<cplx>(x, reinterpret_cast<const cplx*>(y), n, order);
    cplx b0, b1;
    magnus_moments(pc, xs, a, b, b0, b1);
    out4[0] = b0.real(); out4[1] = b0.imag(); out4[2] = b1.real(); out4[3] = b1.imag();
    PB200_CATCH
}

int pb200_host_taylor_fit(const double* x, const double* y, int32_t n, int32_t order, double a, double h, int32_t p,
                          double* coeffs, double* resid) {
    PB200_TRY
    if (!x || !y || !coeffs || n < 2 || p < 0 || p > PB200_TAYLOR_PMAX || !(h > 0.0)) fail(PB200_ERR_INVALID, "bad argument");
    std::vector<double> xs(x, x + n);
    auto pc = make_interpolant<double>(x, y, n, order);
    const TaylorPoly f = taylor_fit(pc, xs, order, a, h, p);
    for (int i = 0; i <= p; ++i) coeffs[i] = f.c[i];
    if (resid) *resid = f.resid;
    PB200_CATCH
}

int pb200_host_taylor_separable(const double* coef, const double* det, int32_t n_traj, int32_t n_qudits, int32_t n_times,
                                int32_t* separable, double* a_out, double* c_out, double* m_out) {
    PB200_TRY
    if (!coef || !det || !separable || n_traj < 1 || n_qudits < 1 || n_times < 2) fail(PB200_ERR_INVALID, "bad argument");
    const cplx* y = reinterpret_cast<const cplx*>(coef);
    const size_t nt = (size_t)n_times, N = (size_t)n_qudits;
    const SeparableFit F = taylor_separable(
        n_traj, n_qudits, n_times, [&](int b, int k, int i) { return y[((size_t)b * N + k) * nt + i]; },
        [&](int b, int k, int i) { return det[((size_t)b * N + k) * nt + i]; });
    *separable = F.ok ? 1 : 0;
    if (F.ok) {
        if (a_out)
            for (size_t x = 0; x < F.a.size(); ++x) { a_out[2 * x] = F.a[x].real(); a_out[2 * x + 1] = F.a[x].imag(); }
        if (c_out) for (size_t x = 0; x < (size_t)n_traj * N; ++x) c_out[x] = F.ns ? F.c[x] : 0.0;
        if (m_out) for (size_t i = 0; i < nt; ++i) m_out[i] = F.ns ? F.m[0][i] : 0.0;
    }
    PB200_CATCH
}

int pb200_host_taylor_shapes(const double* coef, const double* det, int32_t n_traj, int32_t n_qudits, int32_t n_times,
                             int32_t max_shapes, int32_t* n_shapes, double* a_out, double* c_out, double* m_out) {
    PB200_TRY
    if (!coef || !det || !n_shapes || n_traj < 1 || n_qudits < 1 || n_times < 2 || max_shapes < 0 ||
        max_shapes > PB200_TAYLOR_SMAX)
        fail(PB200_ERR_INVALID, "bad argument");
    const cplx* y = reinterpret_cast<const cplx*>(coef);
    const size_t nt = (size_t)n_times, N = (size_t)n_qudits, S = (size_t)max_shapes;
    const SeparableFit F = taylor_separable(
        n_traj, n_qudits, n_times, [&](int b, int k, int i) { return y[((size_t)b * N + k) * nt + i]; },
        [&](int b, int k, int i) { return det[((size_t)b * N + k) * nt + i]; }, max_shapes);
    *n_shapes = F.ok ? F.ns : -1;
    if (F.ok) {
        if (a_out)
            for (size_t x = 0; x < F.a.size(); ++x) { a_out[2 * x] = F.a[x].real(); a_out[2 * x + 1] = F.a[x].imag(); }
        if (c_out)
            for (size_t x = 0; x < (size_t)n_traj * N; ++x)
                for (size_t s = 0; s < S; ++s) c_out[x * S + s] = (int)s < F.ns ? F.c[x * F.ns + s] : 0.0;
        if (m_out)
            for (size_t s = 0; s < S; ++s)
                for (size_t i = 0; i < nt; ++i) m_out[s * nt + i] = (int)s < F.ns ? F.m[s][i] : 0.0;
    }
    PB200_CATCH
}

int pb200_host_taylor_order(double h, const double* m, int32_t p, double tol, int32_t* order_out, double* tail_out) {
    PB200_TRY
    if (!m || !order_out || p < 0 || p > PB200_TAYLOR_PMAX) fail(PB200_ERR_INVALID, "bad argument");
    double tail = 0.0;
    *order_out = taylor_order(h, std::vector<double>(m, m + p + 1), tol, tail);
    if (tail_out) *tail_out = tail;
    PB200_CATCH
}

int pb200_host_chebyshev(double rho, double tol, double* out, int32_t cap, int32_t* count) {
    PB200_TRY
    if (!out || !count) fail(PB200_ERR_INVALID, "bad argument");
    std::vector<cplx> a = chebyshev_exp_coeffs(rho, tol);
    *count = (int32_t)a.size();
    for (int i = 0; i < (int)a.size() && i < cap; ++i) { out[2 * i] = a[i].real(); out[2 * i + 1] = a[i].imag(); }
    PB200_CATCH
}

}
```

Before: 22510.

## Store and load late Taylor orders in single precision under a rounding-error bound

```diff
diff --git a/experiments/taylor_lowprec_cost.py b/experiments/taylor_lowprec_cost.py
--- /dev/null
+++ b/experiments/taylor_lowprec_cost.py
@@ -0,0 +1,83 @@
+from __future__ import annotations
+
+import json
+import os
+import re
+import sys
+import tempfile
+
+sys.path.insert(0, os.path.dirname(os.path.dirname(os.path.abspath(__file__))))
+from experiments.shard_scaling import gpu_info
+from pulser_b200 import engine, workloads as W
+
+STEP_RE = re.compile(r"taylor step .* K=(\d+) ring=.* k_lo=(\d+)")
+KERNEL_RE = re.compile(r"stage_d2_taylor_kernel<([^>]*)>")
+COMBOS = {(False, False): "fp64->fp64", (False, True): "fp64->fp32", (True, True): "fp32->fp32"}
+
+
+def step_log(spec):
+    os.environ["PB200_TAYLOR_LOG"] = "1"
+    with tempfile.TemporaryFile(mode="w+") as f:
+        fd = os.dup(2)
+        os.dup2(f.fileno(), 2)
+        try:
+            with engine.DevicePlan(spec) as plan:
+                plan.set_state("all-ground")
+                plan.propagate(0.0, spec.sampling_times[-1])
+        finally:
+            os.dup2(fd, 2)
+            os.close(fd)
+            del os.environ["PB200_TAYLOR_LOG"]
+        f.seek(0)
+        return [(int(m[1]), int(m[2])) for m in STEP_RE.finditer(f.read())]
+
+
+def kernel_times(spec):
+    import torch
+    from torch.profiler import ProfilerActivity, profile
+
+    with engine.DevicePlan(spec) as plan:
+        plan.set_state("all-ground")
+        plan.propagate(0.0, spec.sampling_times[-1])
+        plan.set_state("all-ground")
+        with profile(activities=[ProfilerActivity.CUDA]) as prof:
+            st = plan.propagate(0.0, spec.sampling_times[-1])
+            torch.cuda.synchronize()
+    recs = []
+    for ev in prof.events():
+        m = KERNEL_RE.search(ev.name)
+        if not m or ev.device_type != torch.autograd.DeviceType.CUDA:
+            continue
+        args = [x.strip() for x in m.group(1).split(",")]
+        key = COMBOS.get((args[8] == "true", args[9] == "true"), "other") if len(args) == 10 else "fp64->fp64"
+        recs.append((ev.time_range.start, ev.time_range.end, key))
+    recs.sort()
+    per = {}
+    for i, (t0, t1, key) in enumerate(recs):
+        n, us = per.get(key, (0, 0.0))
+        per[key] = (n + 1, us + (t1 - (recs[i - 1][1] if i else t0)))
+    total = sum(n for n, _ in per.values())
+    return {
+        "orders": int(st["n_applies"]), "kernel_records": total,
+        "per_combination": {k: {"orders": n, "us_per_order": us / n, "share": n / total} for k, (n, us) in sorted(per.items())},
+        "us_per_order_all": sum(us for _, us in per.values()) / max(total, 1),
+    }
+
+
+def main():
+    out = {"gpu": gpu_info()}
+    for name, spec in (("c2", W.config_c2(n=20)), ("c5", W.config_c5(n=24))):
+        steps = step_log(spec)
+        orders = sum(k for k, _ in steps)
+        low = sum(k - lo for k, lo in steps)
+        out[name] = {"steps": len(steps), "orders": orders, "orders_at_or_after_k_lo": low,
+                     "fraction_low": low / max(orders, 1), **kernel_times(spec)}
+    text = json.dumps(out, indent=1)
+    print(text)
+    if "--out" in sys.argv:
+        with open(sys.argv[sys.argv.index("--out") + 1], "w") as f:
+            f.write(text + "\n")
+
+
+if __name__ == "__main__":
+    main()
diff --git a/include/pulser_b200.h b/include/pulser_b200.h
--- a/include/pulser_b200.h
+++ b/include/pulser_b200.h
@@ -184,6 +184,9 @@
                              double* a_out, double* c_out, double* m_out);
 int pb200_host_taylor_order(double h, const double* m, int32_t p, double tol,
                             int32_t* order_out, double* tail_out);
+int pb200_host_taylor_lowprec(double h, const double* m, int32_t p, int32_t K,
+                              int32_t g_stored, double tol, int32_t* k_lo_out,
+                              double* bound_out);
 int pb200_host_chebyshev(double rho, double tol, double* out, int32_t cap,
                          int32_t* count);
 
diff --git a/pulser_b200/_lib.py b/pulser_b200/_lib.py
--- a/pulser_b200/_lib.py
+++ b/pulser_b200/_lib.py
@@ -154,6 +154,8 @@
             C.c_int, [dp, dp, C.c_int32, C.c_int32, C.c_int32, C.c_int32, C.POINTER(C.c_int32), dp, dp, dp]),
         "pb200_host_taylor_order": (
             C.c_int, [C.c_double, dp, C.c_int32, C.c_double, C.POINTER(C.c_int32), dp]),
+        "pb200_host_taylor_lowprec": (
+            C.c_int, [C.c_double, dp, C.c_int32, C.c_int32, C.c_int32, C.c_double, C.POINTER(C.c_int32), dp]),
     }
     for name, (res, args) in sig.items():
         fn = getattr(lib, name)
@@ -170,7 +172,8 @@
     "pb200_state_get", "pb200_state_probabilities", "pb200_state_norm2",
     "pb200_state_occupation", "pb200_state_correlation", "pb200_state_energy", "pb200_state_overlap", "pb200_state_expect", "pb200_state_sample", "pb200_state_copy", "pb200_state_device_ptr", "pb200_propagate", "pb200_apply_h",
     "pb200_coefficients_at", "pb200_bench_apply", "pb200_host_interpolate",
-    "pb200_host_moments", "pb200_host_chebyshev", "pb200_host_taylor_fit", "pb200_host_taylor_order", "pb200_host_taylor_separable",
+    "pb200_host_moments", "pb200_host_chebyshev", "pb200_host_taylor_fit", "pb200_host_taylor_order", "pb200_host_taylor_lowprec",
+    "pb200_host_taylor_separable",
     "pb200_host_taylor_shapes",
     "pb200_plan_create_shard", "pb200_shards_link", "pb200_shards_propagate", "pb200_shards_apply_h", "pb200_shards_energy",
     "pb200_shards_expect",
diff --git a/pulser_b200/csrc/kernels.cuh b/pulser_b200/csrc/kernels.cuh
--- a/pulser_b200/csrc/kernels.cuh
+++ b/pulser_b200/csrc/kernels.cuh
@@ -79,6 +79,20 @@
     uint64_t pol;
     asm("createpolicy.fractional.L2::evict_last.b64 %0, 1.0;" : "=l"(pol));
     asm volatile("st.global.L2::cache_hint.v2.f64 [%0], {%1, %2}, %3;" ::"l"(p), "d"(v.x), "d"(v.y), "l"(pol) : "memory");
+}
+__device__ __forceinline__ void st_c2(float2* p, c2 v) { *p = make_float2((float)v.x, (float)v.y); }
+__device__ __forceinline__ void st_c2_evict_last(float2* p, c2 v) {
+    uint64_t pol;
+    asm("createpolicy.fractional.L2::evict_last.b64 %0, 1.0;" : "=l"(pol));
+    asm volatile("st.global.L2::cache_hint.v2.f32 [%0], {%1, %2}, %3;" ::"l"(p), "f"((float)v.x), "f"((float)v.y), "l"(pol)
+                 : "memory");
+}
+__device__ __forceinline__ c2 tile_c2(const c2& t) { return t; }
+__device__ __forceinline__ c2 tile_c2(const float2& t) { return {(double)t.x, (double)t.y}; }
+__device__ __forceinline__ double2 ld_partner(const c2* p) { return __ldg(reinterpret_cast<const double2*>(p)); }
+__device__ __forceinline__ double2 ld_partner(const float2* p) {
+    const float2 r = __ldg(p);
+    return make_double2((double)r.x, (double)r.y);
 }
 
 struct LanczosFuse {
@@ -258,6 +272,10 @@
     double2 r = __ldcs(reinterpret_cast<const double2*>(p));
     return {r.x, r.y};
 }
+__device__ __forceinline__ c2 ld_own(const float2* p) {
+    const float2 r = __ldcs(p);
+    return {(double)r.x, (double)r.y};
+}
 
 __device__ __forceinline__ void taylor_signed_add(double gx, double gy, double sg, double x, double y, double& pr, double& pi,
                                                   double& qr, double& qi) {
@@ -266,8 +284,8 @@
     qr = fma(sg, zx, qr); qi = fma(sg, zy, qi);
 }
 
-template <bool UNIFORM, bool REAL_G, int TBITS, int RB, bool SIGNED = false>
-__device__ __forceinline__ void rb_tile_gather(const PassGeom& g, const c2* tile, const double* __restrict__ tab, int tid,
+template <bool UNIFORM, bool REAL_G, int TBITS, int RB, bool SIGNED = false, class T = c2>
+__device__ __forceinline__ void rb_tile_gather(const PassGeom& g, const T* tile, const double* __restrict__ tab, int tid,
                                                int to_bit, int jstart, bool skip_smem, const c2 (&v)[1 << RB],
                                                double (&pr)[1 << RB], double (&pi)[1 << RB], double (&qr)[1 << RB],
                                                double (&qi)[1 << RB]) {
@@ -315,7 +333,7 @@
             const double sg = (bit == to_bit) ? 1.0 : -1.0;
 #pragma unroll
             for (int r = 0; r < R; ++r) {
-                const c2 pv = tile[ptid + r * NT];
+                const c2 pv = tile_c2(tile[ptid + r * NT]);
                 if (UNIFORM) {
                     pr[r] += pv.x; pi[r] += pv.y;
                     if (!REAL_G) { qr[r] = fma(sg, pv.x, qr[r]); qi[r] = fma(sg, pv.y, qi[r]); }
@@ -692,6 +710,8 @@
     int acc_add_h;
     int acc_on;
     c2 acc_mul;
+    int src32, out32;
+    unsigned hchi32, hg32;
     const c2* peer[PB200_MAX_SHARD_BITS];
     int shard_bits, shard;
     c2* g2_out;
@@ -703,8 +723,8 @@
     int diss_flip;
 };
 
-template <int R, int H = (R >= 4) ? R / 2 : R, bool SHARD = false, bool CPLX = false, bool DISS = false, class Off,
-          class Dint>
+template <int R, int H = (R >= 4) ? R / 2 : R, bool SHARD = false, bool CPLX = false, bool DISS = false,
+          bool HIST32 = false, bool OUT32 = false, class Off, class Dint>
 __device__ __forceinline__ void taylor_epilogue(const TaylorArgs& a, const long long (&idx)[R], c2 (&v)[R],
                                                 const double (&gx)[R], const double (&gy)[R], const Off& off,
                                                 long long voff, const Dint& dint,
@@ -736,8 +756,14 @@
         for (int j = 0; j < a.nh; ++j) {
             if (a.hchi[j]) {
                 c2 c[H];
-#pragma unroll
-                for (int r = 0; r < H; ++r) c[r] = ld_own(a.hchi[j] + voff + idx[h0 + r]);
+                if (HIST32 && ((a.hchi32 >> j) & 1)) {
+                    const float2* src = reinterpret_cast<const float2*>(a.hchi[j]) + voff;
+#pragma unroll
+                    for (int r = 0; r < H; ++r) c[r] = ld_own(src + idx[h0 + r]);
+                } else {
+#pragma unroll
+                    for (int r = 0; r < H; ++r) c[r] = ld_own(a.hchi[j] + voff + idx[h0 + r]);
+                }
 #pragma unroll
                 for (int r = 0; r < H; ++r) {
                     double d;
@@ -749,8 +775,14 @@
             }
             if (a.hg[j]) {
                 c2 c[H];
-#pragma unroll
-                for (int r = 0; r < H; ++r) c[r] = ld_own(a.hg[j] + voff + idx[h0 + r]);
+                if (HIST32 && ((a.hg32 >> j) & 1)) {
+                    const float2* src = reinterpret_cast<const float2*>(a.hg[j]) + voff;
+#pragma unroll
+                    for (int r = 0; r < H; ++r) c[r] = ld_own(src + idx[h0 + r]);
+                } else {
+#pragma unroll
+                    for (int r = 0; r < H; ++r) c[r] = ld_own(a.hg[j] + voff + idx[h0 + r]);
+                }
 #pragma unroll
                 for (int r = 0; r < H; ++r) { sx[r] = fma(a.hom[j], c[r].x, sx[r]); sy[r] = fma(a.hom[j], c[r].y, sy[r]); }
             }
@@ -768,8 +800,13 @@
 #pragma unroll
         for (int r = 0; r < H; ++r) {
             res[r] = {a.scale.x * sx[r] - a.scale.y * sy[r], a.scale.x * sy[r] + a.scale.y * sx[r]};
-            st_c2_evict_last(a.out + voff + idx[h0 + r], res[r]);
-            if (a.g_out) st_c2(a.g_out + voff + idx[h0 + r], c2{gx[h0 + r], gy[h0 + r]});
+            if constexpr (OUT32) {
+                st_c2_evict_last(reinterpret_cast<float2*>(a.out) + voff + idx[h0 + r], res[r]);
+                if (a.g_out) st_c2(reinterpret_cast<float2*>(a.g_out) + voff + idx[h0 + r], c2{gx[h0 + r], gy[h0 + r]});
+            } else {
+                st_c2_evict_last(a.out + voff + idx[h0 + r], res[r]);
+                if (a.g_out) st_c2(a.g_out + voff + idx[h0 + r], c2{gx[h0 + r], gy[h0 + r]});
+            }
             if constexpr (CPLX) { if (a.g2_out) st_c2(a.g2_out + voff + idx[h0 + r], c2{qx[h0 + r], qy[h0 + r]}); }
         }
         if (a.acc_on) {
@@ -871,7 +908,7 @@
 }
 
 template <bool UNIFORM, bool REAL_G, int TBITS, int RB, bool SHARD = false, int NS = (UNIFORM ? 0 : 1), bool CPLX = false,
-          bool DISS = false>
+          bool DISS = false, bool SRC32 = false, bool OUT32 = false>
 __global__ void __launch_bounds__(1 << (TBITS - RB),
                                   (CPLX || DISS) ? 1 : (65536 / ((1 << (TBITS - RB)) * (RB >= 3 ? 128 : 64))))
 stage_d2_taylor_kernel(const __grid_constant__ TaylorArgs a) {
@@ -880,6 +917,9 @@
     static_assert(NS == (UNIFORM ? 0 : 1) || NS == PB200_TAYLOR_SMAX, "one-shape table, or PB200_TAYLOR_SMAX shapes");
     static_assert(!CPLX || !REAL_G, "a complex drive gathers through the per-bit table");
     static_assert(!DISS || (!UNIFORM && !SHARD && !CPLX), "a density matrix runs the batch gather, one device, one phase");
+    static_assert(!(SRC32 || OUT32) || (UNIFORM && NS == 0 && !CPLX && !DISS),
+                  "single-precision orders: one state, a uniform drive of one phase");
+    using TT = std::conditional_t<SRC32, float2, c2>;
     constexpr bool SHAPES = NS == PB200_TAYLOR_SMAX;
     constexpr int NT = 1 << (TBITS - RB);
     constexpr int TSIZE = 1 << TBITS;
@@ -888,18 +928,18 @@
     constexpr int STB = TBITS - CB;
     constexpr bool TAB = !(UNIFORM && REAL_G);
     extern __shared__ __align__(128) unsigned char smem_raw[];
-    c2* tile = reinterpret_cast<c2*>(smem_raw);
+    TT* tile = reinterpret_cast<TT*>(smem_raw);
     __shared__ __align__(8) uint64_t mbar;
     const PassGeom& g = a.geo;
     const int tid = threadIdx.x;
     const long long traj = UNIFORM ? 0 : (long long)blockIdx.y;
     const long long voff = traj * a.D;
     const long long base = (long long)blockIdx.x << TBITS;
-    const c2* vsrc = a.v + voff;
+    const TT* vsrc = reinterpret_cast<const TT*>(a.v) + voff;
 
     if (tid == 0) mbar_init(&mbar, 1);
     __syncthreads();
-    double* dsm = reinterpret_cast<double*>(tile + TSIZE);
+    double* dsm = reinterpret_cast<double*>(smem_raw + (size_t)TSIZE * sizeof(c2));
     const double* ts = dsm + TBITS * TBITS + TBITS + 1;
     const double* xt = ts + (1 << RB);
     double* tab = dsm + taylor_dint_doubles(TBITS, RB) + g.n_bits * g.n_bits;
@@ -910,8 +950,8 @@
     pdl_wait();
     pdl_launch_dependents();
     if (tid == 0) {
-        mbar_arrive_expect_tx(&mbar, (uint32_t)TSIZE * 16u);
-        tma_load_1d(tile, vsrc + base, (uint32_t)TSIZE * 16u, &mbar);
+        mbar_arrive_expect_tx(&mbar, (uint32_t)(TSIZE * sizeof(TT)));
+        tma_load_1d(tile, vsrc + base, (uint32_t)(TSIZE * sizeof(TT)), &mbar);
     }
     double* bl = tab + (SHAPES ? taylor_table_stride(g.n_bits, NS) : 0);
     double* at = bl + ((PB200_TAYLOR_PMAX + 1) << RB);
@@ -982,10 +1022,10 @@
             const int bit = (int)((base >> p) & 1);
             double gx = 0.0, gy = 0.0;
             if (TAB) { gx = tab[2 * p]; gy = (bit == to_bit) ? tab[2 * p + 1] : -tab[2 * p + 1]; }
-            const c2* src = vsrc + (i0 ^ (1LL << p));
+            const TT* src = vsrc + (i0 ^ (1LL << p));
             double2 raw[RC];
 #pragma unroll
-            for (int r = 0; r < RC; ++r) raw[r] = __ldg(reinterpret_cast<const double2*>(src + r * NT));
+            for (int r = 0; r < RC; ++r) raw[r] = ld_partner(src + r * NT);
 #pragma unroll
             for (int r = 0; r < RC; ++r) {
                 if constexpr (CPLX) {
@@ -1006,10 +1046,13 @@
                     const int p = nb - a.shard_bits + q;
                     gx = tab[2 * p]; gy = (bit == to_bit) ? tab[2 * p + 1] : -tab[2 * p + 1];
                 }
-                const c2* src = a.peer[q] + i0;
+                const TT* src = reinterpret_cast<const TT*>(a.peer[q]) + i0;
                 double2 raw[RC];
 #pragma unroll
-                for (int r = 0; r < RC; ++r) raw[r] = *reinterpret_cast<const double2*>(src + r * NT);
+                for (int r = 0; r < RC; ++r) {
+                    if constexpr (SRC32) raw[r] = make_double2((double)src[r * NT].x, (double)src[r * NT].y);
+                    else raw[r] = *reinterpret_cast<const double2*>(src + r * NT);
+                }
 #pragma unroll
                 for (int r = 0; r < RC; ++r) {
                     if constexpr (CPLX) {
@@ -1033,11 +1076,11 @@
                 if ((m >> q) & 1) d += xt[(q + 1) * NT + tid];
             return d;
         };
-        const c2* sub = tile + (c << STB);
+        const TT* sub = tile + (c << STB);
         c2 v[RC];
         double qd[RC];
 #pragma unroll
-        for (int r = 0; r < RC; ++r) v[r] = sub[tid + r * NT];
+        for (int r = 0; r < RC; ++r) v[r] = tile_c2(sub[tid + r * NT]);
         if constexpr (CPLX) rb_tile_gather<false, false, STB, 3, true>(g, sub, tab, tid, to_bit, 0, false, v, pr, pi, dr, di);
         else rb_tile_gather<!TAB, !TAB, STB, 3>(g, sub, tab, tid, to_bit, 0, false, v, pr, pi, qd, qd);
 #pragma unroll
@@ -1046,10 +1089,10 @@
             const int bit = (c >> q) & 1;
             double gx = 0.0, gy = 0.0;
             if (TAB) { gx = tab[2 * p]; gy = (bit == to_bit) ? tab[2 * p + 1] : -tab[2 * p + 1]; }
-            const c2* other = tile + ((c ^ (1 << q)) << STB);
+            const TT* other = tile + ((c ^ (1 << q)) << STB);
 #pragma unroll
             for (int r = 0; r < RC; ++r) {
-                const c2 pv = other[tid + r * NT];
+                const c2 pv = tile_c2(other[tid + r * NT]);
                 if constexpr (CPLX) {
                     taylor_signed_add(gx, gy, bit == to_bit ? 1.0 : -1.0, pv.x, pv.y, pr[r], pi[r], dr[r], di[r]);
                 } else if (!TAB) {
@@ -1094,12 +1137,12 @@
                     if (pr < TBITS) {
 #pragma unroll
                         for (int r = 0; r < RC; ++r) {
-                            const c2 t = tile[(tpos + r * NT) ^ (int)mask];
+                            const c2 t = tile_c2(tile[(tpos + r * NT) ^ (int)mask]);
                             pv[r] = make_double2(t.x, t.y);
                         }
                     } else {
 #pragma unroll
-                        for (int r = 0; r < RC; ++r) pv[r] = __ldg(reinterpret_cast<const double2*>(vsrc + (idx[r] ^ mask)));
+                        for (int r = 0; r < RC; ++r) pv[r] = ld_partner(vsrc + (idx[r] ^ mask));
                     }
 #pragma unroll
                     for (int r = 0; r < RC; ++r) taylor_diss_flip(a, idx[r], pr, pc, pv[r], dx[r], dy[r]);
@@ -1127,8 +1170,8 @@
                 a, idx, v, pr, pi, [&](int r, int J) { return lt[J * NT] + lc[(J << RB) + r]; }, voff, dint, nullptr,
                 nullptr, ex, ey);
         } else {
-            taylor_epilogue<RC, UNIFORM ? RC / 2 : RC / 4, SHARD, false, DISS>(a, idx, v, pr, pi, off, voff, dint, nullptr,
-                                                                             nullptr, ex, ey);
+            taylor_epilogue<RC, UNIFORM ? RC / 2 : RC / 4, SHARD, false, DISS, SRC32, OUT32>(a, idx, v, pr, pi, off, voff,
+                                                                                           dint, nullptr, nullptr, ex, ey);
         }
     }
 }
diff --git a/pulser_b200/csrc/plan.cu b/pulser_b200/csrc/plan.cu
--- a/pulser_b200/csrc/plan.cu
+++ b/pulser_b200/csrc/plan.cu
@@ -201,6 +201,7 @@
     TaylorSmem smem;
     bool pdl;
     bool diss = false;
+    bool src32 = false, out32 = false;
 };
 
 static const std::vector<TaylorVariant>& taylor_variants() {
@@ -209,12 +210,28 @@
     static const std::vector<TaylorVariant> v = {
         {true,  true,  false, 0,  false, stage_d2_taylor_kernel<true, true, TB, RB, false, 0, false>,     RB,  S::Tile,      true},
         {true,  false, false, 0,  false, stage_d2_taylor_kernel<true, false, TB, RB, false, 0, false>,    RB,  S::TileTable, true},
+        {true,  true,  false, 0,  false, stage_d2_taylor_kernel<true, true, TB, RB, false, 0, false, false, false, true>,
+         RB, S::Tile, true, false, false, true},
+        {true,  true,  false, 0,  false, stage_d2_taylor_kernel<true, true, TB, RB, false, 0, false, false, true, true>,
+         RB, S::Tile, true, false, true, true},
+        {true,  false, false, 0,  false, stage_d2_taylor_kernel<true, false, TB, RB, false, 0, false, false, false, true>,
+         RB, S::TileTable, true, false, false, true},
+        {true,  false, false, 0,  false, stage_d2_taylor_kernel<true, false, TB, RB, false, 0, false, false, true, true>,
+         RB, S::TileTable, true, false, true, true},
         {false, false, false, 1,  false, stage_d2_taylor_kernel<false, false, TB, RB, false, 1, false>,   RB,  S::TileTable, true},
         {true,  true,  false, SM, false, stage_d2_taylor_kernel<true, true, TB, RB, false, SM, false>,    RB,  S::Shapes,    true},
         {true,  false, false, SM, false, stage_d2_taylor_kernel<true, false, TB, RB, false, SM, false>,   RB,  S::Shapes,    true},
         {false, false, false, SM, false, stage_d2_taylor_kernel<false, false, TB, RB, false, SM, false>,  RB,  S::Shapes,    true},
         {true,  true,  true,  0,  false, stage_d2_taylor_kernel<true, true, TB, RB, true, 0, false>,      RB,  S::Tile,      false},
         {true,  false, true,  0,  false, stage_d2_taylor_kernel<true, false, TB, RB, true, 0, false>,     RB,  S::TileTable, false},
+        {true,  true,  true,  0,  false, stage_d2_taylor_kernel<true, true, TB, RB, true, 0, false, false, false, true>,
+         RB, S::Tile, false, false, false, true},
+        {true,  true,  true,  0,  false, stage_d2_taylor_kernel<true, true, TB, RB, true, 0, false, false, true, true>,
+         RB, S::Tile, false, false, true, true},
+        {true,  false, true,  0,  false, stage_d2_taylor_kernel<true, false, TB, RB, true, 0, false, false, false, true>,
+         RB, S::TileTable, false, false, false, true},
+        {true,  false, true,  0,  false, stage_d2_taylor_kernel<true, false, TB, RB, true, 0, false, false, true, true>,
+         RB, S::TileTable, false, false, true, true},
         {true,  true,  true,  SM, false, stage_d2_taylor_kernel<true, true, TB, RB, true, SM, false>,     RB,  S::Shapes,    false},
         {true,  false, true,  SM, false, stage_d2_taylor_kernel<true, false, TB, RB, true, SM, false>,    RB,  S::Shapes,    false},
         {true,  false, false, 0,  true,  stage_d2_taylor_kernel<true, false, TB, RBC, false, 0, true>,    RBC, S::TileTable, true},
@@ -2177,6 +2194,42 @@
     return std::max(kk, 1);
 }
 
+static int taylor_lowprec_order(double h, const std::vector<double>& mj, int K, bool g_stored, double tol,
+                                double& bound_out) {
+    constexpr double u32 = 5.9604644775390625e-08;
+    const int p = (int)mj.size() - 1;
+    std::vector<double> y(K + 1, 0.0), S(K + 1, 0.0), z(K + 1);
+    y[0] = 1.0;
+    for (int k = 0; k < K; ++k) {
+        double s = 0.0;
+        for (int j = 0; j <= std::min(p, k); ++j) s += mj[j] * y[k - j];
+        y[k + 1] = h * s / (k + 1);
+    }
+    for (int j = 1; j <= K; ++j) {
+        std::fill(z.begin(), z.end(), 0.0);
+        z[j] = 1.0;
+        double sum = 1.0;
+        for (int k = j; k < K; ++k) {
+            double s = 0.0;
+            for (int i = 0; i <= std::min(p, k - j); ++i) s += mj[i] * z[k - i];
+            z[k + 1] = h * s / (k + 1);
+            sum += z[k + 1];
+        }
+        S[j] = sum;
+    }
+    double bound = 0.0;
+    int k_lo = K;
+    for (int L = K - 1; L >= 0; --L) {
+        double add = u32 * y[L + 1] * S[L + 1];
+        if (g_stored && L <= K - 2) add += u32 * y[L] * (S[L] - 1.0);
+        if (bound + add > tol) break;
+        bound += add;
+        k_lo = L;
+    }
+    bound_out = bound;
+    return k_lo;
+}
+
 static void launch_taylor_order(const Plan& P, bool tiled, const TaylorArgs& a, bool cplx) {
     const bool diss = a.n_pair > 0;
     if (!tiled) {
@@ -2193,14 +2246,14 @@
     const int ns = a.tab_shapes ? PB200_TAYLOR_SMAX : uniform ? 0 : 1;
     for (const TaylorVariant& v : taylor_variants()) {
         if (v.uniform != uniform || v.real_g != real_g || v.shard != shard || v.ns != ns || v.cplx != cplx ||
-            v.diss != diss)
+            v.diss != diss || v.src32 != (a.src32 != 0) || v.out32 != (a.out32 != 0))
             continue;
         launch_k(v.kernel, dim3((unsigned)(P.D >> kTaylorTileBits), uniform ? 1u : (unsigned)P.B),
                  dim3(1u << (kTaylorTileBits - v.rb)), taylor_variant_smem(v, P.n), P.stream, v.pdl, a);
         return;
     }
-    fail(PB200_ERR_UNSUPPORTED, "no Taylor stage kernel for UNIFORM=%d REAL_G=%d SHARD=%d NS=%d CPLX=%d DISS=%d", uniform,
-         real_g, shard, ns, cplx, diss);
+    fail(PB200_ERR_UNSUPPORTED, "no Taylor stage kernel for UNIFORM=%d REAL_G=%d SHARD=%d NS=%d CPLX=%d DISS=%d SRC32=%d OUT32=%d",
+         uniform, real_g, shard, ns, cplx, diss, a.src32, a.out32);
 }
 
 static bool taylor_geometry(const Plan& P, PassGeom& geo, bool& tiled) {
@@ -2220,6 +2273,7 @@
     int p_om = 0, p_th = 0, p = 0;
     std::vector<double> gam;
     int K = 0;
+    int k_lo = 0;
     double phi = 0.0;
     int n_chi = 0, n_g = 0;
     int drive = 0;
@@ -2234,6 +2288,7 @@
     double t, steps_len = 0.0, t_retry_len = 0.0, A_sum, C_sum[PB200_TAYLOR_SMAX], kRoundUnit = 0.05 * 1.1102230246251565e-16;
     int order, N, nt, ns;
     bool log_steps;
+    bool lowprec;
     pb200_run_stats st{};
     struct Fit { TaylorPoly om, omi, th, m[PB200_TAYLOR_SMAX]; double om_allow = 0.0; bool ok; };
 
@@ -2261,6 +2316,9 @@
         for (int s = 0; s < PB200_TAYLOR_SMAX; ++s) C_sum[s] = std::max(C.c_sum_max[s], 1e-300);
         fit_total = 0.5 * rate * (t_stop - t_start);
         log_steps = env_int("PB200_TAYLOR_LOG", 0) != 0;
+        PassGeom geo;
+        bool tiled = false;
+        lowprec = taylor_geometry(P, geo, tiled) && tiled && C.uniform;
     }
 
     Fit fit_step(double a, double h, bool single_piece) {
@@ -2404,18 +2462,19 @@
     }
 
     void record(TaylorStep& s, const Fit& F, const std::vector<double>& mj, int p_m, double om_resid, double rho) {
-        double trunc_bound = 0.0;
+        double trunc_bound = 0.0, round32 = 0.0;
         s.K = taylor_order(s.h, mj, std::max(1e-15, 0.1 * rate * s.h), trunc_bound);
+        s.k_lo = (lowprec && s.drive != 2) ? taylor_lowprec_order(s.h, mj, s.K, s.n_g > 0, 0.1 * rate * s.h, round32) : s.K;
         st.n_applies += s.K; st.n_exponentials += 1; ++st.n_steps;
         if (log_steps)
-            fprintf(stderr, "taylor step t=%.6f h_ns=%.3f p_om=%d p_th=%d p_m=%d K=%d ring=%d rho=%.3f resid=%.2e/%.2e/%.2e drive=%s\n",
+            fprintf(stderr, "taylor step t=%.6f h_ns=%.3f p_om=%d p_th=%d p_m=%d K=%d ring=%d rho=%.3f resid=%.2e/%.2e/%.2e drive=%s k_lo=%d\n",
                     s.t, s.h * 1e3, s.p_om, s.p_th, p_m, s.K, s.ring() + 1, mj[0] * s.h, om_resid, F.th.resid, F.m[0].resid,
-                    s.drive == 2 ? "cplx" : s.drive == 1 ? "rot" : "real");
+                    s.drive == 2 ? "cplx" : s.drive == 1 ? "rot" : "real", s.k_lo);
         st.max_rho = std::max(st.max_rho, rho);
         double fit_m = 0.0;
         for (int q = 0; q < ns; ++q) fit_m += C_sum[q] * F.m[q].resid;
         const double fit_err = s.h * (A_sum * om_resid + N * F.th.resid + fit_m);
-        st.err_estimate += trunc_bound + fit_err;
+        st.err_estimate += trunc_bound + round32 + fit_err;
         fit_spent += fit_err;
         { const double r = kRoundUnit * std::exp(std::min(rho, 40.0)); round2 += r * r; }
         steps_len += s.h;
@@ -2536,6 +2595,8 @@
     a.th0 = s.th[0]; a.gam0 = s.gam[0]; a.om0 = s.om[0];
     for (int q = 0; q < PB200_TAYLOR_SMAX; ++q) a.m0[q] = m_c(q, 0);
     a.scale = {0.0, -s.h / (k + 1)};
+    a.src32 = k > s.k_lo;
+    a.out32 = k >= s.k_lo;
     a.nh = std::min(s.p, k);
     for (int j = 1; j <= a.nh; ++j) {
         const double thj = th_c(j), omj = j < (int)s.om.size() ? s.om[j] : 0.0;
@@ -2544,6 +2605,8 @@
         a.hth[j - 1] = thj; a.hgam[j - 1] = s.gam[j]; a.hom[j - 1] = omj;
         a.hchi[j - 1] = (thj != 0.0 || any_m || s.gam[j] != 0.0) ? R.chi[(k - j) % s.n_chi] : nullptr;
         a.hg[j - 1] = (omj != 0.0) ? R.gr[(k - j) % s.n_g] : nullptr;
+        if (k - j - 1 >= s.k_lo) a.hchi32 |= 1u << (j - 1);
+        if (k - j >= s.k_lo) a.hg32 |= 1u << (j - 1);
         if (s.drive == 2) {
             const double omij = j < (int)s.omi.size() ? s.omi[j] : 0.0;
             a.homi[j - 1] = omij;
@@ -4015,6 +4078,16 @@
     PB200_CATCH
 }
 
+int pb200_host_taylor_lowprec(double h, const double* m, int32_t p, int32_t K, int32_t g_stored, double tol,
+                              int32_t* k_lo_out, double* bound_out) {
+    PB200_TRY
+    if (!m || !k_lo_out || p < 0 || p > PB200_TAYLOR_PMAX || K < 1) fail(PB200_ERR_INVALID, "bad argument");
+    double bound = 0.0;
+    *k_lo_out = taylor_lowprec_order(h, std::vector<double>(m, m + p + 1), K, g_stored != 0, tol, bound);
+    if (bound_out) *bound_out = bound;
+    PB200_CATCH
+}
+
 int pb200_host_chebyshev(double rho, double tol, double* out, int32_t cap, int32_t* count) {
     PB200_TRY
     if (!out || !count) fail(PB200_ERR_INVALID, "bad argument");
```

Result: faster. 24450, median of 6 (+8.6%).
